# dohyeon-Lee/IsaacgymEnv

Measured on AMD Instinct MI355X. Metric: env-steps/sec AnymalTerrain 4096 envs/GPU, higher is better.
Workload: dtype f32; 1 GPU; AnymalTerrain VecTask.step, terrainType plane (AnymalTerrain.yaml default), 5 physics substeps/step, obs noise on; num_envs_per_gpu=4096, global_num_envs=4096, parallelism=dp1, solver=TGS (physx.solver_type 1, cfg/config.yaml:31)

## Files before the change

include/gymsim.h:

```cpp
#ifndef GYMSIM_H
#define GYMSIM_H

#include <stdint.h>

#include "gymtask.h"

#ifdef __cplusplus
extern "C" {
#endif

#define GS_ABI_VERSION 9

typedef struct gs_sim gs_sim;

typedef struct gs_model_desc {
    int32_t num_bodies, num_dofs, num_candidates, num_shapes, fixed_base;
    const int32_t *parent;
    const int32_t *joint_kind;
    const int32_t *body_dof;
    const double *joint_origin;
    const double *joint_axis;
    const double *mass;
    const double *com;
    const double *inertia;
    const int32_t *cand_body;
    const double *cand_point;
    const double *cand_radius;
    const int32_t *cand_shape;
    const double *dof_effort;
    const double *dof_velocity;
    const double *dof_armature;
    const double *dof_lower;
    const double *dof_upper;
    const int32_t *dof_has_limits;
    int32_t num_links;
    const int32_t *cand_link;
    const int32_t *link_body;
    const double *link_pose;
    const double *link_com;
    const int32_t *cand_dyn;
    const int32_t *shape_kind;
    const int32_t *shape_body;
    const int32_t *shape_link;
    const double *shape_pose;
    const double *shape_size;
    const double *shape_margin;
    const double *shape_sphere;
    int32_t num_hull_verts;
    const double *hull_verts;
    const int32_t *shape_hv0;
    const int32_t *shape_hv1;
    int32_t num_pairs;
    const int32_t *pair_a;
    const int32_t *pair_b;
    const int32_t *pair_kind;
    int32_t pair_pool;
    int32_t num_pair_verts;
    const double *pair_verts;
    const int32_t *shape_pv0;
    const int32_t *shape_pv1;
} gs_model_desc;

typedef struct gs_sim_params {
    double dt;
    int32_t substeps;
    double gravity[3];
    int32_t num_position_iterations;
    int32_t num_velocity_iterations;
    double contact_offset;
    double rest_offset;
    double bounce_threshold_velocity;
    double max_depenetration_velocity;
    int32_t contact_collection;
    int32_t kernel_variant;
    double joint_limit_margin;
    int32_t num_threads;
    int32_t solver_type;
} gs_sim_params;

typedef struct gs_pd_args {
    const float *actions;
    const float *default_pos;
    float kp, kd, action_scale, torque_limit;
    int32_t decimation;
    int32_t extra_simulates;
    float *torques_out;
    float *dof_state_out;
    float *root_state_out;
    float *contact_out;
    float *actions_copy_out;
    const gt_anymal_params *tail_params;
    const gt_anymal_buffers *tail_buffers;
} gs_pd_args;

int gs_abi_version(void);
const char *gs_last_error(void);

int gs_sim_pd_tail_supported(const gs_sim *sim);

int gs_topology_supported(const gs_model_desc *model);

gs_sim *gs_sim_create(int device, const gs_sim_params *params);
void gs_sim_destroy(gs_sim *sim);

int gs_sim_add_ground(gs_sim *sim, double static_friction, double dynamic_friction, double restitution);

int gs_sim_add_triangle_mesh(gs_sim *sim, const float *vertices, int64_t num_vertices, const uint32_t *triangles,
                             int64_t num_triangles, const double *transform_p, double static_friction,
                             double dynamic_friction, double restitution);

int gs_sim_set_model(gs_sim *sim, const gs_model_desc *model);

int gs_sim_prepare(gs_sim *sim, int num_envs, float *state, const float *shape_friction, float *contact);

int gs_sim_simulate(gs_sim *sim, const float *dof_force, void *stream);

int gs_sim_refresh_root(gs_sim *sim, float *root_state, void *stream);
int gs_sim_refresh_dof(gs_sim *sim, float *dof_state, void *stream);
int gs_sim_refresh_contact(gs_sim *sim, float *net_contact, void *stream);

int gs_sim_refresh_rigid_body(gs_sim *sim, float *rigid_body_state, void *stream);
int gs_sim_refresh_jacobian(gs_sim *sim, float *jacobian, void *stream);
int gs_sim_refresh_mass_matrix(gs_sim *sim, float *mass_matrix, void *stream);

int gs_sim_set_root(gs_sim *sim, const float *root_state, const int32_t *idx, int n_idx, void *stream);
int gs_sim_set_dof(gs_sim *sim, const float *dof_state, const int32_t *idx, int n_idx, void *stream);
int gs_sim_set_root_and_dof(gs_sim *sim, const float *root, const float *dof, const int32_t *idx, int n_idx,
                            void *stream);

int gs_sim_pd_step(gs_sim *sim, const gs_pd_args *args, void *stream);

int gs_sim_set_force_sensors(gs_sim *sim, int n, const int32_t *bodies);
int gs_sim_bind_force_sensors(gs_sim *sim, float *sensor_soa);
int gs_sim_refresh_force_sensor(gs_sim *sim, float *out, void *stream);

int gs_sim_set_dof_drives(gs_sim *sim, const int32_t *mode, const double *stiffness, const double *damping);
int gs_sim_bind_dof_targets(gs_sim *sim, const float *pos_targets, const float *vel_targets);
int gs_sim_bind_dof_properties_env(gs_sim *sim, const float *table, int any_drive, int any_limits);

int gs_sim_set_self_collision(gs_sim *sim, int enable);

int gs_sim_kernel_variant(gs_sim *sim);

int gs_sim_enable_timing(gs_sim *sim, int enable);
float gs_sim_last_kernel_ms(gs_sim *sim);

int gs_debug_phase_cycles(unsigned long long *out, int n, int reset);

int gs_debug_terrain_query(gs_sim *sim, const float *centres, const float *radii, int n, float *out, void *stream);

int gs_debug_self_contacts(gs_sim *sim, int mode, float *out, int *count, void *stream);

#ifdef __cplusplus
}
#endif
#endif
```

isaacgymenv_amd/csrc/gs_capi.hip:

```cpp
#include <cmath>
#include <cstdlib>
#include <cstdio>
#include <cstring>
#include <algorithm>
#include <chrono>
#include <string>
#include <vector>

#include "gs_internal.h"
#include "../../include/gymsim.h"

namespace {
thread_local std::string g_err;

int fail(const char* fmt, const char* arg = nullptr) {
  char buf[512];
  std::snprintf(buf, sizeof(buf), fmt, arg ? arg : "");
  g_err = buf;
  return -1;
}
int hip_fail(hipError_t e, const char* where) {
  char buf[512];
  std::snprintf(buf, sizeof(buf), "%s: %s", where, hipGetErrorString(e));
  g_err = buf;
  return -1;
}

std::string signature(const gs_model_desc* m) {
  std::string s = "fb" + std::to_string(m->fixed_base) + "_p";
  for (int i = 0; i < m->num_bodies; ++i) s += (i ? "-" : "") + std::to_string(m->parent[i]);
  s += "_c";
  for (int i = 0; i < m->num_candidates; ++i) s += (i ? "-" : "") + std::to_string(m->cand_body[i]);
  bool links_differ = m->num_links != m->num_bodies;
  for (int i = 0; i < m->num_candidates && !links_differ; ++i) links_differ = m->cand_link[i] != m->cand_body[i];
  if (links_differ) {
    s += "_l" + std::to_string(m->num_links) + "_";
    for (int i = 0; i < m->num_candidates; ++i) s += (i ? "-" : "") + std::to_string(m->cand_link[i]);
  }
  return s;
}

const TopoEntry* find_topology(const gs_model_desc* m) {
  const std::string sig = signature(m);
  for (int i = 0; i < g_num_topologies; ++i)
    if (sig == g_topologies[i].sig) return &g_topologies[i];
  return nullptr;
}
}

struct gs_sim {
  int device = 0;
  gs_sim_params params{};
  DevParams dp{};
  bool has_ground = false;
  float ground_mu = 1.f;
  const TopoEntry* topo = nullptr;
  launch_sim_fn sim_fn = nullptr;
  launch_pd_fn pd_fn = nullptr;
  int variant = 0;
  launch_sim_fn model_sim_fn = nullptr;
  launch_pd_fn model_pd_fn = nullptr;
  int model_variant = 0;
  bool team_pairs = false;
  int uni_any_drive = 0, uni_any_limits = 0;
  TopoEntry gen_entry{};
  GenTopo* d_gen = nullptr;
  int env_any_drive = 0, env_any_limits = 0;
  DevModel* d_model = nullptr;
  DevModel h_model{};
  DevLinks* d_links = nullptr;
  int nr = 0, nv = 0;
  std::vector<int> parent;
  float* sens = nullptr;
  int nb = 0, nd = 0, nc = 0, ns = 0;
  int N = 0;
  float* state = nullptr;
  const float* mu = nullptr;
  float* cf = nullptr;
  bool timing = false;
  hipEvent_t ev0 = nullptr, ev1 = nullptr;
  bool timed = false;
  float4* d_tverts = nullptr;
  uint4* d_tcells = nullptr;
  float* d_tblk = nullptr;
  float* d_tsq4 = nullptr;
  float4* d_trec = nullptr;
  float* d_rows = nullptr;
  size_t rows_cap = 0;
  bool host = false;
  HostPool* pool = nullptr;
  const HostTopoEntry* htopo = nullptr;
  DevLinks h_links{};
  std::vector<float4> h_tverts;
  std::vector<uint4> h_tcells;
  std::vector<float> h_tblk;
  std::vector<float> h_tsq4;
  std::vector<float4> h_trec;
  double host_ms = -1.0;
  const DevModel* model() const { return host ? &h_model : d_model; }
  const DevLinks* links() const { return host ? &h_links : d_links; }
};

extern "C" {

int gs_abi_version(void) { return GS_ABI_VERSION; }
const char* gs_last_error(void) { return g_err.c_str(); }

int gs_topology_supported(const gs_model_desc* model) { return find_topology(model) != nullptr; }

gs_sim* gs_sim_create(int device, const gs_sim_params* p) {
  if (!p) { fail("gs_sim_create: null params"); return nullptr; }
  if (!(p->dt > 0)) { fail("gs_sim_create: dt must be > 0"); return nullptr; }
  gs_sim* s = nullptr;
  if (device < 0) {
    s = new gs_sim();
    s->host = true;
    s->device = -1;
    s->pool = host_pool_create(p->num_threads > 0 ? p->num_threads : 1);
  } else {
    int ndev = 0;
    if (hipGetDeviceCount(&ndev) != hipSuccess || device >= ndev) {
      fail("gs_sim_create: no HIP device %s", std::to_string(device).c_str());
      return nullptr;
    }
    if (hipError_t e = hipSetDevice(device); e != hipSuccess) {
      hip_fail(e, "gs_sim_create hipSetDevice");
      return nullptr;
    }
    s = new gs_sim();
    s->device = device;
  }
  s->params = *p;
  const int sub = p->substeps > 0 ? p->substeps : 1;
  s->dp.h = (float)(p->dt / sub);
  s->dp.substeps = sub;
  for (int k = 0; k < 3; ++k) s->dp.g[k] = (float)p->gravity[k];
  s->dp.pos_iters = p->num_position_iterations;
  s->dp.vel_iters = p->num_velocity_iterations;
  s->dp.contact_offset = (float)p->contact_offset;
  s->dp.rest_offset = (float)p->rest_offset;
  s->dp.max_depen_vel = (float)p->max_depenetration_velocity;
  s->dp.tgs = p->solver_type == 1 && p->num_position_iterations > 0 ? 1 : 0;
  s->dp.collect = p->contact_collection != 0;
  s->dp.limit_margin = (float)(p->joint_limit_margin > 0 ? p->joint_limit_margin : 0.0);
  s->dp.any_limits = 0;
  s->dp.has_ground = 0;
  s->dp.ground_mu = 1.f;
  if (const char* v = std::getenv("GS_TEAM_ENVS_PER_WAVE")) {
    const int w = std::atoi(v);
    s->dp.team_epw = w == 16 || w == 8 || w == 4 ? w : 0;
  }
  return s;
}

void gs_sim_destroy(gs_sim* s) {
  if (!s) return;
  if (s->host) {
    host_pool_destroy(s->pool);
    delete s;
    return;
  }
  (void)hipSetDevice(s->device);
  if (s->d_model) (void)hipFree(s->d_model);
  if (s->d_links) (void)hipFree(s->d_links);
  if (s->d_tverts) (void)hipFree(s->d_tverts);
  if (s->d_tcells) (void)hipFree(s->d_tcells);
  if (s->d_tblk) (void)hipFree(s->d_tblk);
  if (s->d_tsq4) (void)hipFree(s->d_tsq4);
  if (s->d_trec) (void)hipFree(s->d_trec);
  if (s->d_rows) (void)hipFree(s->d_rows);
  if (s->d_gen) (void)hipFree(s->d_gen);
  if (s->ev0) (void)hipEventDestroy(s->ev0);
  if (s->ev1) (void)hipEventDestroy(s->ev1);
  delete s;
}

int gs_sim_add_ground(gs_sim* s, double static_friction, double dynamic_friction, double restitution) {
  if (!s) return fail("gs_sim_add_ground: null sim");
  (void)dynamic_friction;
  (void)restitution;
  s->has_ground = true;
  s->dp.has_ground = 1;
  s->dp.ground_mu = (float)static_friction;
  return 0;
}

int gs_sim_add_triangle_mesh(gs_sim* s, const float* vertices, int64_t num_vertices, const uint32_t* triangles,
                             int64_t num_triangles, const double* transform_p, double static_friction,
                             double dynamic_friction, double restitution) {
  (void)dynamic_friction;
  (void)restitution;
  if (!s || !vertices || !triangles) return fail("gs_sim_add_triangle_mesh: null argument");
  if (s->topo) return fail("gs_sim_add_triangle_mesh: call before the model is set (prepare_sim)");
  if (s->d_tverts) return fail("gs_sim_add_triangle_mesh: one triangle mesh per sim");
  if (num_triangles < 2) return fail("gs_sim_add_triangle_mesh: empty mesh");
  const int64_t cols = (int64_t)triangles[1] - 1;
  if (triangles[0] != 0 || triangles[2] != 1 || cols < 2 || num_vertices % cols != 0)
    return fail("gs_sim_add_triangle_mesh: not a heightfield grid mesh (first triangle)");
  const int64_t rows = num_vertices / cols;
  if (rows < 2 || num_triangles != 2 * (rows - 1) * (cols - 1))
    return fail("gs_sim_add_triangle_mesh: triangle count does not match a %s grid",
                (std::to_string(rows) + "x" + std::to_string(cols)).c_str());
  if (rows > (1 << 24) || cols > (1 << 24)) return fail("gs_sim_add_triangle_mesh: grid too large");
  for (int64_t i = 0; i + 1 < rows; ++i) {
    for (int64_t j = 0; j + 1 < cols; ++j) {
      const int64_t b = i * cols + j, t = 2 * (i * (cols - 1) + j);
      const uint32_t* a = triangles + 3 * t;
      if (a[0] != b || a[1] != b + cols + 1 || a[2] != b + 1 || a[3] != b || a[4] != b + cols || a[5] != b + cols + 1)
        return fail("gs_sim_add_triangle_mesh: triangle %s does not follow the heightfield grid layout",
                    std::to_string(t).c_str());
    }
  }
  std::vector<double> spans;
  for (int64_t j = 0; j < cols && spans.size() < 4096; j += std::max<int64_t>(1, cols / 1024))
    spans.push_back((double)vertices[3 * ((rows - 1) * cols + j)] - (double)vertices[3 * j]);
  std::sort(spans.begin(), spans.end());
  double hs = spans[spans.size() / 2] / (double)(rows - 1);
  if (!(hs > 0)) return fail("gs_sim_add_triangle_mesh: cannot infer the grid spacing");
  const double tx = transform_p ? transform_p[0] : 0.0, ty = transform_p ? transform_p[1] : 0.0,
               tz = transform_p ? transform_p[2] : 0.0;
  double x0 = vertices[0], y0 = vertices[1];
  for (int64_t j = 0; j < cols; ++j) x0 = std::min(x0, (double)vertices[3 * j]);
  for (int64_t i = 0; i < rows; ++i) y0 = std::min(y0, (double)vertices[3 * (i * cols) + 1]);
  std::vector<float4> hv((size_t)(rows * cols));
  for (int64_t i = 0; i < rows; ++i) {
    for (int64_t j = 0; j < cols; ++j) {
      const float* v = vertices + 3 * (i * cols + j);
      const double gx = x0 + i * hs, gy = y0 + j * hs;
      if (std::fabs(v[0] - gx) > 1.001 * hs || std::fabs(v[1] - gy) > 1.001 * hs)
        return fail("gs_sim_add_triangle_mesh: a vertex lies more than one cell from its grid point");
      hv[(size_t)(i * cols + j)] = make_float4((float)(v[0] + tx), (float)(v[1] + ty), (float)(v[2] + tz), 0.f);
    }
  }
  std::vector<uint4> hc((size_t)((rows - 1) * (cols - 1)));
  for (int64_t i = 0; i + 1 < rows; ++i) {
    for (int64_t j = 0; j + 1 < cols; ++j) {
      const float4 q[4] = {hv[i * cols + j], hv[i * cols + j + 1], hv[(i + 1) * cols + j], hv[(i + 1) * cols + j + 1]};
      float zmax = q[0].z, zmin = q[0].z, xmin = q[0].x, xmax = q[0].x, ymin = q[0].y, ymax = q[0].y;
      for (int k = 1; k < 4; ++k) {
        zmax = std::max(zmax, q[k].z);
        zmin = std::min(zmin, q[k].z);
        xmin = std::min(xmin, q[k].x); xmax = std::max(xmax, q[k].x);
        ymin = std::min(ymin, q[k].y); ymax = std::max(ymax, q[k].y);
      }
      const double cx0 = x0 + tx + i * hs, cy0 = y0 + ty + j * hs;
      uint32_t f = 0;
      if (xmin < cx0 - 0.25 * hs) f |= TCELL_XLO;
      if (xmax > cx0 + 1.25 * hs) f |= TCELL_XHI;
      if (ymin < cy0 - 0.25 * hs) f |= TCELL_YLO;
      if (ymax > cy0 + 1.25 * hs) f |= TCELL_YHI;
      auto ext = [&](double d) -> uint32_t {
        return (uint32_t)std::min(255.0, std::ceil(std::max(0.0, d) / hs * TCELL_EXT_UNITS));
      };
      const uint32_t ew = ext(cx0 - xmin) | ext(xmax - (cx0 + hs)) << 8 | ext(cy0 - ymin) << 16 |
                          ext(ymax - (cy0 + hs)) << 24;
      uint32_t zb, zl;
      std::memcpy(&zb, &zmax, 4);
      std::memcpy(&zl, &zmin, 4);
      hc[(size_t)(i * (cols - 1) + j)] = make_uint4(zb, f, zl, ew);
    }
  }
  const int64_t brows = (rows - 1 + TERRAIN_BLK - 1) / TERRAIN_BLK, bcols = (cols - 1 + TERRAIN_BLK - 1) / TERRAIN_BLK;
  std::vector<float> hb((size_t)(brows * bcols), -3.0e38f);
  for (int64_t i = 0; i + 1 < rows; ++i)
    for (int64_t j = 0; j + 1 < cols; ++j) {
      float top;
      std::memcpy(&top, &hc[(size_t)(i * (cols - 1) + j)].x, 4);
      float& b = hb[(size_t)((i / TERRAIN_BLK) * bcols + j / TERRAIN_BLK)];
      b = std::max(b, top);
    }
  const int64_t cr = rows - 1, cc = cols - 1;
  std::vector<float> h4((size_t)(cr * cc)), hq((size_t)(cr * cc));
  for (int64_t i = 0; i < cr; ++i)
    for (int64_t j = 0; j < cc; ++j) {
      float m = -3.0e38f;
      for (int64_t d = 0; d < 4 && j + d < cc; ++d) {
        float top;
        std::memcpy(&top, &hc[(size_t)(i * cc + j + d)].x, 4);
        m = std::max(m, top);
      }
      h4[(size_t)(i * cc + j)] = m;
    }
  for (int64_t i = 0; i < cr; ++i)
    for (int64_t j = 0; j < cc; ++j) {
      float m = -3.0e38f;
      for (int64_t d = 0; d < 4 && i + d < cr; ++d) m = std::max(m, h4[(size_t)((i + d) * cc + j)]);
      hq[(size_t)(i * cc + j)] = m;
    }
  std::vector<float4> hr((size_t)(cr * cc * TERRAIN_REC));
  for (int64_t i = 0; i < cr; ++i)
    for (int64_t j = 0; j < cc; ++j) {
      const float4 q00 = hv[i * cols + j], q01 = hv[i * cols + j + 1], q10 = hv[(i + 1) * cols + j],
                   q11 = hv[(i + 1) * cols + j + 1];
      auto normal = [](const float4& a, const float4& b, const float4& c, float* nf) {
        const double e1[3] = {(double)b.x - a.x, (double)b.y - a.y, (double)b.z - a.z};
        const double e2[3] = {(double)c.x - a.x, (double)c.y - a.y, (double)c.z - a.z};
        const double x[3] = {e1[1] * e2[2] - e1[2] * e2[1], e1[2] * e2[0] - e1[0] * e2[2], e1[0] * e2[1] - e1[1] * e2[0]};
        const double l2 = x[0] * x[0] + x[1] * x[1] + x[2] * x[2];
        nf[0] = 0.f; nf[1] = 0.f; nf[2] = -1.f;
        if (!(l2 > 1e-14)) return;
        const double il = 1.0 / std::sqrt(l2);
        if (x[2] * il < (double)TERRAIN_DOWN_NZ) return;
        for (int k = 0; k < 3; ++k) nf[k] = (float)(x[k] * il);
      };
      float n0[3], n1[3];
      normal(q00, q11, q01, n0);
      normal(q00, q10, q11, n1);
      float4* r = &hr[(size_t)((i * cc + j) * TERRAIN_REC)];
      r[0] = make_float4(q00.x, q00.y, q00.z, n0[0]);
      r[1] = make_float4(q01.x, q01.y, q01.z, n0[1]);
      r[2] = make_float4(q10.x, q10.y, q10.z, n0[2]);
      r[3] = make_float4(q11.x, q11.y, q11.z, n1[0]);
      r[4] = make_float4(n1[1], n1[2], 0.f, 0.f);
    }
  TerrainDev& T = s->dp.terr;
  if (s->host) {
    s->h_tverts = std::move(hv);
    s->h_tcells = std::move(hc);
    s->h_tblk = std::move(hb);
    s->h_tsq4 = std::move(hq);
    s->h_trec = std::move(hr);
    T.rec = s->h_trec.data();
    T.v = s->h_tverts.data();
    T.cell = s->h_tcells.data();
    T.blk = s->h_tblk.data();
    T.sq4 = s->h_tsq4.data();
  } else {
    float4* dv = nullptr;
    uint4* dc = nullptr;
    float* db = nullptr;
    float* dq = nullptr;
    float4* dr = nullptr;
    hipError_t e = hipSetDevice(s->device);
    if (e == hipSuccess) e = hipMalloc(&dv, hv.size() * sizeof(float4));
    if (e == hipSuccess) e = hipMalloc(&dc, hc.size() * sizeof(uint4));
    if (e == hipSuccess) e = hipMalloc(&db, hb.size() * sizeof(float));
    if (e == hipSuccess) e = hipMalloc(&dq, hq.size() * sizeof(float));
    if (e == hipSuccess) e = hipMemcpy(dv, hv.data(), hv.size() * sizeof(float4), hipMemcpyHostToDevice);
    if (e == hipSuccess) e = hipMemcpy(dc, hc.data(), hc.size() * sizeof(uint4), hipMemcpyHostToDevice);
    if (e == hipSuccess) e = hipMemcpy(db, hb.data(), hb.size() * sizeof(float), hipMemcpyHostToDevice);
    if (e == hipSuccess) e = hipMemcpy(dq, hq.data(), hq.size() * sizeof(float), hipMemcpyHostToDevice);
    if (e == hipSuccess) e = hipMalloc(&dr, hr.size() * sizeof(float4));
    if (e == hipSuccess) e = hipMemcpy(dr, hr.data(), hr.size() * sizeof(float4), hipMemcpyHostToDevice);
    if (e != hipSuccess) {
      if (dr) (void)hipFree(dr);
      if (dv) (void)hipFree(dv);
      if (dc) (void)hipFree(dc);
      if (db) (void)hipFree(db);
      if (dq) (void)hipFree(dq);
      return hip_fail(e, "gs_sim_add_triangle_mesh");
    }
    s->d_tverts = dv;
    s->d_tcells = dc;
    s->d_tblk = db;
    s->d_tsq4 = dq;
    s->d_trec = dr;
    T.rec = s->d_trec;
    T.v = s->d_tverts;
    T.cell = s->d_tcells;
    T.blk = s->d_tblk;
    T.sq4 = s->d_tsq4;
  }
  T.bcols = (int)bcols;
  T.rows = (int)rows;
  T.cols = (int)cols;
  T.x0 = (float)(x0 + tx);
  T.y0 = (float)(y0 + ty);
  T.hs = (float)hs;
  T.inv_hs = (float)(1.0 / hs);
  T.mu = (float)static_friction;
  s->dp.has_terrain = 1;
  return 0;
}

int gs_sim_set_model(gs_sim* s, const gs_model_desc* m) {
  if (!s || !m) return fail("gs_sim_set_model: null argument");
  if (m->num_bodies > GS_MAXB || m->num_dofs > GS_MAXD || m->num_candidates > GS_MAXC || m->num_links > GS_MAXL ||
      m->num_shapes > GS_MAXSH)
    return fail("gs_sim_set_model: articulation exceeds compiled maxima (bodies/dofs/candidates/links)");
  if (m->num_links < m->num_bodies || !m->link_body || !m->link_pose || !m->link_com ||
      (m->num_candidates > 0 && !m->cand_link))
    return fail("gs_sim_set_model: link tables missing (gs_model_desc ABI 2: num_links >= num_bodies)");
  for (int l = 0; l < m->num_links; ++l)
    if (m->link_body[l] < 0 || m->link_body[l] >= m->num_bodies) return fail("gs_sim_set_model: link_body out of range");
  for (int c = 0; c < m->num_candidates; ++c)
    if (m->cand_link[c] < 0 || m->cand_link[c] >= m->num_links) return fail("gs_sim_set_model: cand_link out of range");
  const TopoEntry* t = find_topology(m);
  const bool generic = !t || (s->params.kernel_variant == 4 && !s->host);
  if (generic) {
    if (s->host)
      return fail("gs_sim_set_model: the runtime-sized kernel is a GPU kernel and no host solver is compiled for "
                  "this topology (add it with tools/gen_topologies.py): %s", signature(m).c_str());
    if (s->params.kernel_variant == 1 || s->params.kernel_variant == 2)
      return fail("gs_sim_set_model: kernel_variant 1 / 2 requested but topology %s is not compiled (the runtime-"
                  "sized kernel is variant 4)", signature(m).c_str());
    for (int c = 0; c < m->num_candidates; ++c)
      if (m->cand_dyn && m->cand_dyn[c] >= 0)
        return fail("gs_sim_set_model: topology %s has convex-hull candidates: the runtime-sized kernel has no hull "
                    "ground manifold (compile the topology with tools/gen_topologies.py)", signature(m).c_str());
    if (s->dp.has_terrain)
      return fail("gs_sim_set_model: topology %s with a terrain mesh: the runtime-sized kernel has plane contacts only "
                  "(compile the topology with tools/gen_topologies.py)", signature(m).c_str());
    if (m->num_dofs + 6 > GS_MAXD + 6 || (m->num_candidates > 0 && !m->cand_shape))
      return fail("gs_sim_set_model: runtime-sized kernel tables missing for %s", signature(m).c_str());
  }
  if (!generic && m->num_pairs > 0 && m->pair_pool != t->npk)
    return fail("gs_sim_set_model: self-contact pool differs from the compiled topology's %s",
                std::to_string(t->npk).c_str());
  for (int c = 0; c < m->num_candidates && !generic; ++c)
    if (m->cand_dyn && m->cand_dyn[c] != t->cdyn[c])
      return fail("gs_sim_set_model: hull slots differ from the compiled topology (tools/gen_topologies.py)");
  if (!generic && m->num_pairs > 0 && m->num_pairs != t->npair)
    return fail("gs_sim_set_model: self-collision pair count differs from the compiled topology's %s",
                std::to_string(t->npair).c_str());
  for (int q = 0; q < m->num_pairs && !generic; ++q)
    if (m->pair_a[q] != t->pair_a[q] || m->pair_b[q] != t->pair_b[q] || m->pair_kind[q] != t->pair_k[q])
      return fail("gs_sim_set_model: self-collision pairs differ from the compiled topology (tools/gen_topologies.py)");
  for (int sh = 0; sh < m->num_shapes && !generic; ++sh)
    if (m->shape_kind && m->shape_kind[sh] != t->shkind[sh])
      return fail("gs_sim_set_model: shape kinds differ from the compiled topology (tools/gen_topologies.py)");
  DevModel h;
  std::memset(&h, 0, sizeof(h));
  for (int i = 0; i < m->num_bodies; ++i) {
    for (int k = 0; k < 9; ++k) h.jR[i][k] = (float)m->joint_origin[12 * i + k];
    for (int k = 0; k < 3; ++k) h.jt[i][k] = (float)m->joint_origin[12 * i + 9 + k];
    for (int k = 0; k < 3; ++k) h.jaxis[i][k] = (float)m->joint_axis[3 * i + k];
    h.mass[i] = (float)m->mass[i];
    for (int k = 0; k < 3; ++k) h.com[i][k] = (float)m->com[3 * i + k];
    const double* I = m->inertia + 9 * i;
    h.inertia[i][0] = (float)I[0]; h.inertia[i][1] = (float)I[4]; h.inertia[i][2] = (float)I[8];
    h.inertia[i][3] = (float)I[1]; h.inertia[i][4] = (float)I[2]; h.inertia[i][5] = (float)I[5];
  }
  {
    const double* P = m->link_pose;
    const double* c = m->link_com;
    for (int k = 0; k < 3; ++k)
      h.root_com[k] = (float)(P[9 + k] + P[3 * k] * c[0] + P[3 * k + 1] * c[1] + P[3 * k + 2] * c[2]);
  }
  for (int c = 0; c < m->num_candidates; ++c) {
    for (int k = 0; k < 3; ++k) h.cpoint[c][k] = (float)m->cand_point[3 * c + k];
    h.cradius[c] = (float)m->cand_radius[c];
  }
  if (!m->shape_kind || !m->shape_body || !m->shape_link || !m->shape_pose || !m->shape_size || !m->shape_margin ||
      !m->shape_sphere || !m->shape_hv0 || !m->shape_hv1 || (m->num_candidates > 0 && !m->cand_dyn))
    return fail("gs_sim_set_model: shape tables missing (gs_model_desc ABI 5)");
  if (m->num_hull_verts < 0 || m->num_hull_verts > GS_MAXHV || m->num_pairs < 0 || m->num_pairs > GS_MAXP ||
      (m->num_hull_verts > 0 && !m->hull_verts) || (m->num_pairs > 0 && (!m->pair_a || !m->pair_b || !m->pair_kind)))
    return fail("gs_sim_set_model: hull vertices / self-collision pairs exceed compiled maxima");
  for (int sh = 0; sh < m->num_shapes; ++sh) {
    for (int k = 0; k < 3; ++k) h.shc[sh][k] = (float)m->shape_sphere[4 * sh + k];
    double reach = m->shape_sphere[4 * sh + 3];
    for (int c = 0; c < m->num_candidates; ++c) {
      if (m->cand_shape && m->cand_shape[c] == sh && m->cand_dyn[c] < 0) {
        double d2 = 0.0;
        for (int k = 0; k < 3; ++k) {
          const double d = m->cand_point[3 * c + k] - m->shape_sphere[4 * sh + k];
          d2 += d * d;
        }
        reach = std::max(reach, std::sqrt(d2) + m->cand_radius[c]);
      }
    }
    h.shc[sh][3] = (float)(reach * (1.0 + 1e-4) + 1e-5);
    h.shkind[sh] = m->shape_kind[sh];
    h.shbody[sh] = m->shape_body[sh];
    h.shlink[sh] = m->shape_link[sh];
    for (int k = 0; k < 9; ++k) h.shR[sh][k] = (float)m->shape_pose[12 * sh + k];
    for (int k = 0; k < 3; ++k) h.sht[sh][k] = (float)m->shape_pose[12 * sh + 9 + k];
    for (int k = 0; k < 3; ++k) h.shsize[sh][k] = (float)m->shape_size[3 * sh + k];
    h.shm[sh] = (float)m->shape_margin[sh];
    h.hv0[sh] = m->shape_hv0[sh];
    h.hv1[sh] = m->shape_hv1[sh];
    if (h.shbody[sh] < 0 || h.shbody[sh] >= m->num_bodies || h.shlink[sh] < 0 || h.shlink[sh] >= m->num_links ||
        h.hv0[sh] < 0 || h.hv1[sh] < h.hv0[sh] || h.hv1[sh] > m->num_hull_verts ||
        (h.shkind[sh] == 4 && h.hv1[sh] == h.hv0[sh]))
      return fail("gs_sim_set_model: shape %s tables out of range", std::to_string(sh).c_str());
  }
  for (int v = 0; v < m->num_hull_verts; ++v)
    for (int k = 0; k < 4; ++k) h.hv[v][k] = (float)m->hull_verts[4 * v + k];
  if (m->num_pair_verts < 0 || m->num_pair_verts > GS_MAXPV || !m->shape_pv0 || !m->shape_pv1 ||
      (m->num_pair_verts > 0 && !m->pair_verts))
    return fail("gs_sim_set_model: hull self-collision cores missing or beyond GS_MAXPV");
  for (int v = 0; v < m->num_pair_verts; ++v)
    for (int k = 0; k < 4; ++k) h.pv[v][k] = (float)m->pair_verts[4 * v + k];
  for (int sh = 0; sh < m->num_shapes; ++sh) {
    h.pv0[sh] = m->shape_pv0[sh];
    h.pv1[sh] = m->shape_pv1[sh];
    if (h.pv0[sh] < 0 || h.pv1[sh] < h.pv0[sh] || h.pv1[sh] > m->num_pair_verts ||
        (h.shkind[sh] == 4 && h.pv1[sh] == h.pv0[sh]))
      return fail("gs_sim_set_model: shape %s self-collision core out of range", std::to_string(sh).c_str());
  }
  for (int c = 0; c < m->num_candidates; ++c)
    if (m->cand_dyn[c] >= 0 && m->shape_kind[m->cand_shape[c]] != 4)
      return fail("gs_sim_set_model: dynamic candidate %s on a shape that is not a hull", std::to_string(c).c_str());
  h.np = m->num_pairs;
  for (int q = 0; q < m->num_pairs; ++q) {
    h.pa[q] = m->pair_a[q];
    h.pb[q] = m->pair_b[q];
    h.pk[q] = m->pair_kind[q];
    if (h.pa[q] < 0 || h.pb[q] <= h.pa[q] || h.pb[q] >= m->num_shapes || h.pk[q] < 0 || h.pk[q] > 3)
      return fail("gs_sim_set_model: self-collision pair %s out of range", std::to_string(q).c_str());
  }
  for (int b = 0; b < m->num_bodies; ++b) {
    unsigned mask = 0;
    for (int a = b; a >= 0; a = m->parent[a]) mask |= 1u << a;
    h.banc[b] = mask;
  }
  int any_lim = 0;
  for (int j = 0; j < m->num_dofs; ++j) {
    h.effort[j] = (float)m->dof_effort[j];
    h.vmax[j] = (float)m->dof_velocity[j];
    h.armature[j] = (float)m->dof_armature[j];
    h.has_lim[j] = m->dof_has_limits && m->dof_has_limits[j] && m->dof_upper[j] > m->dof_lower[j];
    h.lower[j] = h.has_lim[j] ? (float)m->dof_lower[j] : 0.f;
    h.upper[j] = h.has_lim[j] ? (float)m->dof_upper[j] : 0.f;
    any_lim |= h.has_lim[j];
  }
  h.nsens = 0;
  for (int b = 0; b < GS_MAXB; ++b) h.sens_of_body[b] = -1;

  DevLinks hl;
  std::memset(&hl, 0, sizeof(hl));
  hl.nb = m->num_bodies;
  hl.nd = m->num_dofs;
  hl.nr = m->num_links;
  hl.fixed_base = m->fixed_base;
  for (int b = 0; b < m->num_bodies; ++b) {
    hl.parent[b] = m->parent[b];
    hl.jkind[b] = m->joint_kind[b];
    hl.bdof[b] = m->body_dof[b];
    unsigned mask = 0;
    for (int a = b; a >= 0; a = m->parent[a]) mask |= 1u << a;
    hl.anc_mask[b] = mask;
    if (m->body_dof[b] >= 0) hl.dbody[m->body_dof[b]] = b;
  }
  for (int l = 0; l < m->num_links; ++l) {
    hl.lbody[l] = m->link_body[l];
    for (int k = 0; k < 9; ++k) hl.lR[l][k] = (float)m->link_pose[12 * l + k];
    for (int k = 0; k < 3; ++k) hl.lt[l][k] = (float)m->link_pose[12 * l + 9 + k];
    for (int k = 0; k < 3; ++k) hl.lcom[l][k] = (float)m->link_com[3 * l + k];
  }

  const int want = s->params.kernel_variant;
  launch_sim_fn sim_fn = nullptr;
  launch_pd_fn pd_fn = nullptr;
  const HostTopoEntry* htopo = nullptr;
  int variant = 0;
  GenTopo hg;
  std::memset(&hg, 0, sizeof(hg));
  if (generic) {
    hg.nc = m->num_candidates;
    for (int c = 0; c < m->num_candidates; ++c) {
      hg.cbody[c] = m->cand_body[c];
      hg.cshape[c] = m->cand_shape[c];
      hg.clink[c] = m->cand_link[c];
      if (hg.cbody[c] < 0 || hg.cbody[c] >= m->num_bodies || hg.cshape[c] < 0 || hg.cshape[c] >= m->num_shapes)
        return fail("gs_sim_set_model: candidate %s tables out of range", std::to_string(c).c_str());
    }
    TopoEntry& g = s->gen_entry;
    g = TopoEntry{};
    g.sig = "runtime";
    g.name = "runtime-sized (gs_generic.hip)";
    g.sim = launch_sim_generic;
    g.pd = launch_pd_generic;
    g.dbg_pool = nullptr;
    g.nb = m->num_bodies; g.nd = m->num_dofs; g.nc = m->num_candidates; g.ns = m->num_shapes;
    g.sens = 0;
    g.row_floats = (int)generic_ws_floats(m->num_candidates, m->num_dofs, m->fixed_base);
    g.row_lanes = 1;
    g.npk = 0;
    g.npair = 0;
    t = &g;
  }
  if (s->host) {
    for (int i = 0; i < g_num_host_topologies; ++i)
      if (std::strcmp(g_host_topologies[i].sig, t->sig) == 0) htopo = &g_host_topologies[i];
    if (!htopo) return fail("gs_sim_set_model: no host solver for topology %s", t->sig);
    if (want == 2) return fail("gs_sim_set_model: the lane-team kernel is a GPU kernel (host sim)");
    variant = 3;
  } else {
    const TeamEntry* te = nullptr;
    for (int i = 0; i < g_num_team_kernels; ++i)
      if (std::strcmp(g_team_kernels[i].sig, t->sig) == 0 && g_team_kernels[i].sim) te = &g_team_kernels[i];
    if (te && any_lim) te = nullptr;
    if (want == 2 && !te)
      return fail("gs_sim_set_model: no lane-team kernel for this topology / joint limits");
    if (generic) {
      sim_fn = launch_sim_generic;
      pd_fn = launch_pd_generic;
      variant = 4;
    } else if (te && want != 1) {
      sim_fn = te->sim;
      pd_fn = te->pd;
      variant = 2;
    } else {
      sim_fn = t->sim;
      pd_fn = t->pd;
      variant = 1;
    }
    if (hipError_t e = hipSetDevice(s->device); e != hipSuccess) return hip_fail(e, "gs_sim_set_model hipSetDevice");
    DevModel* dm = s->d_model;
    DevLinks* dl = s->d_links;
    hipError_t e = hipSuccess;
    if (!dm) e = hipMalloc(&dm, sizeof(DevModel));
    if (e == hipSuccess && !dl) e = hipMalloc(&dl, sizeof(DevLinks));
    s->d_model = dm;
    s->d_links = dl;
    if (e == hipSuccess) e = hipMemcpy(dm, &h, sizeof(DevModel), hipMemcpyHostToDevice);
    if (e == hipSuccess) e = hipMemcpy(dl, &hl, sizeof(DevLinks), hipMemcpyHostToDevice);
    if (e == hipSuccess && generic && !s->d_gen) e = hipMalloc(&s->d_gen, sizeof(GenTopo));
    if (e == hipSuccess && generic) e = hipMemcpy(s->d_gen, &hg, sizeof(GenTopo), hipMemcpyHostToDevice);
    if (e != hipSuccess) return hip_fail(e, "gs_sim_set_model upload");
  }
  s->h_model = h;
  s->h_links = hl;
  s->dp.any_limits = any_lim;
  s->uni_any_limits = any_lim;
  s->parent.assign(m->parent, m->parent + m->num_bodies);
  s->sim_fn = sim_fn;
  s->pd_fn = pd_fn;
  s->htopo = htopo;
  s->variant = variant;
  s->model_sim_fn = sim_fn;
  s->model_pd_fn = pd_fn;
  s->model_variant = variant;
  s->team_pairs = variant == 2;
  s->nr = m->num_links;
  s->nv = (m->fixed_base ? 0 : 6) + m->num_dofs;
  s->nb = m->num_bodies;
  s->nd = m->num_dofs;
  s->nc = m->num_candidates;
  s->ns = m->num_shapes;
  s->topo = t;
  s->dp.gen = generic ? s->d_gen : nullptr;
  s->dp.gen_links = generic ? s->d_links : nullptr;
  s->dp.gen_nd = m->num_dofs;
  s->dp.gen_nr = m->num_links;
  return 0;
}

int gs_sim_prepare(gs_sim* s, int num_envs, float* state, const float* shape_friction, float* contact) {
  if (!s || !s->topo) return fail("gs_sim_prepare: model not set");
  if (num_envs <= 0 || !state || !shape_friction || !contact) return fail("gs_sim_prepare: bad buffers");
  s->N = num_envs;
  s->state = state;
  s->mu = shape_friction;
  s->cf = contact;
  return 0;
}

static SimBuffers buffers(gs_sim* s) { return SimBuffers{s->state, s->mu, s->cf, s->N, s->sens, s->d_rows}; }

static size_t rows_needed(const gs_sim* s) {
  if (s->host || !s->topo || (s->variant != 1 && s->variant != 4) || (s->variant == 1 && s->dp.has_terrain) ||
      s->topo->row_floats <= 0 || s->N <= 0)
    return 0;
  const size_t lanes = (size_t)s->topo->row_lanes;
  return ((size_t)s->N + lanes - 1) / lanes * lanes * (size_t)s->topo->row_floats;
}

static int ready(gs_sim* s, const char* where) {
  if (!s || !s->topo || !s->state) return fail("%s: sim not prepared", where);
  if (s->host ? !s->htopo : (!s->sim_fn || !s->pd_fn || !s->d_model || !s->d_links))
    return fail("%s: sim model incomplete", where);
  if (const size_t need = rows_needed(s); need > s->rows_cap) {
    if (hipError_t e = hipSetDevice(s->device); e != hipSuccess) return hip_fail(e, where);
    if (s->d_rows) (void)hipFree(s->d_rows);
    s->d_rows = nullptr;
    s->rows_cap = 0;
    if (hipError_t e = hipMalloc(&s->d_rows, need * sizeof(float)); e != hipSuccess) {
      s->d_rows = nullptr;
      return hip_fail(e, where);
    }
    s->rows_cap = need;
  }
  return 0;
}

static void timing_begin(gs_sim* s, hipStream_t st) {
  if (!s->timing || s->host) return;
  if (!s->ev0) {
    if (hipEventCreate(&s->ev0) != hipSuccess || hipEventCreate(&s->ev1) != hipSuccess) {
      s->timing = false;
      return;
    }
  }
  (void)hipEventRecord(s->ev0, st);
}
static void timing_end(gs_sim* s, hipStream_t st) {
  if (!s->timing || s->host) return;
  s->timed = hipEventRecord(s->ev1, st) == hipSuccess;
}

namespace {
using host_clock = std::chrono::steady_clock;
double ms_since(host_clock::time_point t0) {
  return std::chrono::duration<double, std::milli>(host_clock::now() - t0).count();
}
}

int gs_sim_simulate(gs_sim* s, const float* dof_force, void* stream) {
  if (ready(s, "gs_sim_simulate")) return -1;
  if (s->host) {
    const auto t0 = host_clock::now();
    s->htopo->sim(&s->h_model, s->dp, buffers(s), dof_force, s->pool);
    s->host_ms = ms_since(t0);
    return 0;
  }
  hipStream_t st = (hipStream_t)stream;
  timing_begin(s, st);
  hipError_t e = s->sim_fn(s->d_model, s->dp, buffers(s), dof_force, st);
  timing_end(s, st);
  return e == hipSuccess ? 0 : hip_fail(e, "gs_sim_simulate");
}

int gs_sim_pd_step(gs_sim* s, const gs_pd_args* a, void* stream) {
  if (ready(s, "gs_sim_pd_step")) return -1;
  if (!a || !a->actions || !a->default_pos || !a->torques_out || !a->dof_state_out)
    return fail("gs_sim_pd_step: actions/default_pos/torques_out/dof_state_out required");
  PdDev d;
  d.actions = a->actions;
  d.dof_state_in = a->dof_state_out;
  d.default_pos = a->default_pos;
  d.kp = a->kp; d.kd = a->kd; d.scale = a->action_scale; d.tlim = a->torque_limit;
  d.decimation = a->decimation;
  d.extra = a->extra_simulates;
  d.torques_out = a->torques_out;
  d.dof_out = a->dof_state_out;
  d.root_out = a->root_state_out;
  d.cf_out = a->contact_out;
  d.actions_copy = a->actions_copy_out;
  d.tail_on = 0;
  if (a->tail_params || a->tail_buffers) {
    const gt_anymal_params* tp = a->tail_params;
    const gt_anymal_buffers* tb = a->tail_buffers;
    auto aligned = [](const void* q) { return ((uintptr_t)q & 15u) == 0; };
    if (!gs_sim_pd_tail_supported(s)) return fail("gs_sim_pd_step: this sim's kernel has no fused tail");
    if (!tp || !tb || tb->hound || tp->num_envs != s->N || tp->num_dofs != s->nd || tp->num_dofs % 4 != 0 ||
        tp->num_bodies != s->nr || tp->num_feet > 4 || tp->num_knees > 4 || tp->num_feet < 0 || tp->num_knees < 0 ||
        tp->base_index < 0 || tp->base_index >= s->nr || !tb->reset_count || !tb->reset_masks || !tb->reset_buf ||
        !tb->timeout_buf || !tb->rew_buf || !tb->episode_sums || !tb->base_lin_vel || !tb->base_ang_vel ||
        !tb->projected_gravity || !tb->progress_buf || !tb->randomize_buf || !tb->commands || !tb->feet_air_time ||
        !tb->last_actions || !tb->last_dof_vel)
      return fail("gs_sim_pd_step: invalid tail parameters / buffers");
    for (int k = 0; k < tp->num_feet; ++k)
      if (tp->feet_idx[k] < 0 || tp->feet_idx[k] >= s->nr) return fail("gs_sim_pd_step: tail foot index");
    for (int k = 0; k < tp->num_knees; ++k)
      if (tp->knee_idx[k] < 0 || tp->knee_idx[k] >= s->nr) return fail("gs_sim_pd_step: tail knee index");
    if (tb->torques != a->torques_out || tb->actions != a->actions_copy_out || tb->root_states != a->root_state_out ||
        tb->contact_forces != a->contact_out || tb->dof_state != a->dof_state_out)
      return fail("gs_sim_pd_step: the tail must read this call's outputs");
    if (!aligned(tb->torques) || !aligned(tb->actions) || !aligned(tb->last_actions) || !aligned(tb->last_dof_vel) ||
        !aligned(tb->dof_state))
      return fail("gs_sim_pd_step: the tail's dof rows must be 16-byte aligned");
    d.tail_on = 1;
    d.tail_p = *tp;
    d.tail_b = *tb;
  }
  if (s->host) {
    const auto t0 = host_clock::now();
    s->htopo->pd(&s->h_model, s->dp, buffers(s), d, s->pool);
    s->host_ms = ms_since(t0);
    return 0;
  }
  hipStream_t st = (hipStream_t)stream;
  timing_begin(s, st);
  hipError_t e = s->pd_fn(s->d_model, s->dp, buffers(s), d, st);
  timing_end(s, st);
  return e == hipSuccess ? 0 : hip_fail(e, "gs_sim_pd_step");
}

int gs_sim_refresh_root(gs_sim* s, float* out, void* stream) {
  if (ready(s, "gs_sim_refresh_root")) return -1;
  if (s->host) {
    host_refresh_root(s->state, s->N, &s->h_model.root_com[0], out, s->pool);
    return 0;
  }
  hipError_t e = launch_refresh_root(s->state, s->N, s->nd, &s->d_model->root_com[0], out, (hipStream_t)stream);
  return e == hipSuccess ? 0 : hip_fail(e, "gs_sim_refresh_root");
}
int gs_sim_refresh_dof(gs_sim* s, float* out, void* stream) {
  if (ready(s, "gs_sim_refresh_dof")) return -1;
  if (s->host) {
    host_refresh_dof(s->state, s->N, s->nd, out, s->pool);
    return 0;
  }
  hipError_t e = launch_refresh_dof(s->state, s->N, s->nd, out, (hipStream_t)stream);
  return e == hipSuccess ? 0 : hip_fail(e, "gs_sim_refresh_dof");
}
int gs_sim_refresh_contact(gs_sim* s, float* out, void* stream) {
  if (ready(s, "gs_sim_refresh_contact")) return -1;
  if (s->host) {
    host_soa_to_aos(s->cf, s->N, s->nr, 3, out, s->pool);
    return 0;
  }
  hipError_t e = launch_refresh_contact(s->cf, s->N, s->nr, out, (hipStream_t)stream);
  return e == hipSuccess ? 0 : hip_fail(e, "gs_sim_refresh_contact");
}
static int kinematics(gs_sim* s, int mode, float* rb, float* jac, float* mm, void* stream, const char* where) {
  if (ready(s, where)) return -1;
  if (!rb && !jac && !mm) return fail("%s: null output", where);
  if (s->host) {
    host_kinematics(&s->h_model, &s->h_links, s->state, s->N, s->nv, mode, rb, jac, mm, s->pool);
    return 0;
  }
  hipError_t e = launch_kinematics(s->d_model, s->d_links, s->state, s->N, s->nv, mode, rb, jac, mm,
                                   (hipStream_t)stream);
  return e == hipSuccess ? 0 : hip_fail(e, where);
}
int gs_sim_refresh_rigid_body(gs_sim* s, float* out, void* stream) {
  return kinematics(s, 1, out, nullptr, nullptr, stream, "gs_sim_refresh_rigid_body");
}
int gs_sim_refresh_jacobian(gs_sim* s, float* out, void* stream) {
  return kinematics(s, 2, nullptr, out, nullptr, stream, "gs_sim_refresh_jacobian");
}
int gs_sim_refresh_mass_matrix(gs_sim* s, float* out, void* stream) {
  return kinematics(s, 4, nullptr, nullptr, out, stream, "gs_sim_refresh_mass_matrix");
}
int gs_sim_set_root(gs_sim* s, const float* src, const int32_t* idx, int n_idx, void* stream) {
  if (ready(s, "gs_sim_set_root")) return -1;
  if (s->host) {
    host_set_root(s->state, s->N, &s->h_model.root_com[0], src, idx, idx ? n_idx : s->N);
    return 0;
  }
  hipError_t e = launch_set_root(s->state, s->N, s->nd, &s->d_model->root_com[0], src, idx, n_idx,
                                 (hipStream_t)stream);
  return e == hipSuccess ? 0 : hip_fail(e, "gs_sim_set_root");
}
int gs_sim_set_dof(gs_sim* s, const float* src, const int32_t* idx, int n_idx, void* stream) {
  if (ready(s, "gs_sim_set_dof")) return -1;
  if (s->host) {
    host_set_dof(s->state, s->N, s->nd, src, idx, idx ? n_idx : s->N);
    return 0;
  }
  hipError_t e = launch_set_dof(s->state, s->N, s->nd, src, idx, n_idx, (hipStream_t)stream);
  return e == hipSuccess ? 0 : hip_fail(e, "gs_sim_set_dof");
}

int gs_sim_set_root_and_dof(gs_sim* s, const float* root, const float* dof, const int32_t* idx, int n_idx,
                            void* stream) {
  if (ready(s, "gs_sim_set_root_and_dof")) return -1;
  if (!root || !dof || !idx || n_idx < 0) return fail("gs_sim_set_root_and_dof: root, dof and idx required");
  if (s->host) {
    host_set_root(s->state, s->N, &s->h_model.root_com[0], root, idx, n_idx);
    host_set_dof(s->state, s->N, s->nd, dof, idx, n_idx);
    return 0;
  }
  hipError_t e = launch_set_root_dof(s->state, s->N, s->nd, &s->d_model->root_com[0], root, dof, idx, n_idx,
                                     (hipStream_t)stream);
  return e == hipSuccess ? 0 : hip_fail(e, "gs_sim_set_root_and_dof");
}

int gs_sim_set_force_sensors(gs_sim* s, int n, const int32_t* bodies) {
  if (!s || !s->topo) return fail("gs_sim_set_force_sensors: model not set");
  if (s->state) return fail("gs_sim_set_force_sensors: call before gs_sim_prepare");
  if (n < 0 || n > GS_MAXS || (n > 0 && !bodies)) return fail("gs_sim_set_force_sensors: at most 8 sensors");
  if (n > 0 && s->variant == 2)
    return fail("gs_sim_set_force_sensors: the lane-team kernel has no force sensors (use kernel_variant 1)");
  if (n > 0 && s->variant == 4)
    return fail("gs_sim_set_force_sensors: the runtime-sized kernel has no force sensors (compile the topology)");
  if (n > 0 && !s->topo->sens)
    return fail("gs_sim_set_force_sensors: topology %s is compiled without force sensors (sensors flag in "
                "tools/gen_topologies.py MODELS)", s->topo->name);
  DevModel& h = s->h_model;
  for (int b = 0; b < GS_MAXB; ++b) h.sens_of_body[b] = -1;
  for (int i = 0; i < n; ++i) {
    const int b = bodies[i];
    if (b <= 0 || b >= s->nb) return fail("gs_sim_set_force_sensors: sensor body out of range (or the root)");
    for (int c = 0; c < s->nb; ++c)
      if (s->parent[c] == b) return fail("gs_sim_set_force_sensors: sensors on non-leaf bodies are not supported");
    if (h.sens_of_body[b] >= 0) return fail("gs_sim_set_force_sensors: two sensors on one body");
    h.sens_of_body[b] = i;
  }
  h.nsens = n;
  if (s->host) return 0;
  hipError_t e = hipSetDevice(s->device);
  if (e == hipSuccess) e = hipMemcpy(s->d_model, &h, sizeof(DevModel), hipMemcpyHostToDevice);
  return e == hipSuccess ? 0 : hip_fail(e, "gs_sim_set_force_sensors hipMemcpy");
}

static int kernel_select(gs_sim* s, const char* who) {
  launch_sim_fn sim_fn = s->model_sim_fn;
  launch_pd_fn pd_fn = s->model_pd_fn;
  int variant = s->model_variant;
  const bool lane = s->dp.any_drive || s->dp.dof_env || (s->dp.self_collide && !s->team_pairs);
  if (lane && variant == 2) {
    if (s->params.kernel_variant == 2)
      return fail("%s: the lane-team kernel (kernel_variant 2) has no joint drives or per-actor dof properties", who);
    sim_fn = s->topo->sim;
    pd_fn = s->topo->pd;
    variant = 1;
  }
  s->sim_fn = sim_fn;
  s->pd_fn = pd_fn;
  s->variant = variant;
  return 0;
}

int gs_sim_set_dof_drives(gs_sim* s, const int32_t* mode, const double* stiffness, const double* damping) {
  if (!s || !s->topo) return fail("gs_sim_set_dof_drives: model not set");
  if (s->nd > 0 && (!mode || !stiffness || !damping)) return fail("gs_sim_set_dof_drives: null argument");
  DevModel h = s->h_model;
  int any = 0;
  for (int j = 0; j < s->nd; ++j) {
    const double kp = mode[j] == 1 ? stiffness[j] : 0.0;
    const double kd = (mode[j] == 1 || mode[j] == 2) ? damping[j] : 0.0;
    if (!(kp >= 0.0) || !(kd >= 0.0)) return fail("gs_sim_set_dof_drives: negative or NaN drive gain");
    h.dkp[j] = (float)kp;
    h.dkd[j] = (float)kd;
    any |= (kp > 0.0 || kd > 0.0);
  }
  if (any && s->model_variant == 2 && s->params.kernel_variant == 2)
    return fail("gs_sim_set_dof_drives: the lane-team kernel (kernel_variant 2) has no joint drives");
  if (!s->host) {
    hipError_t e = hipSetDevice(s->device);
    if (e == hipSuccess) e = hipDeviceSynchronize();
    if (e == hipSuccess) e = hipMemcpy(s->d_model, &h, sizeof(DevModel), hipMemcpyHostToDevice);
    if (e != hipSuccess) return hip_fail(e, "gs_sim_set_dof_drives hipMemcpy");
  }
  s->h_model = h;
  s->uni_any_drive = any;
  s->dp.any_drive = s->dp.dof_env ? s->env_any_drive : any;
  return kernel_select(s, "gs_sim_set_dof_drives");
}

int gs_sim_set_self_collision(gs_sim* s, int enable) {
  if (!s || !s->topo) return fail("gs_sim_set_self_collision: model not set");
  if (enable && s->h_model.np > 0 && s->topo->npk <= 0)
    return fail("gs_sim_set_self_collision: the compiled topology has no self-contact pool");
  if (enable && s->h_model.np > 0 && s->variant == 4)
    return fail("gs_sim_set_self_collision: the runtime-sized kernel has no self-collision (compile the topology "
                "with tools/gen_topologies.py, or create the actors with collision filter 1)");
  s->dp.self_collide = enable && s->h_model.np > 0;
  if (s->dp.self_collide && s->variant == 2 && !s->team_pairs) {
    if (s->params.kernel_variant == 2)
      return fail("gs_sim_set_self_collision: the lane-team kernel (kernel_variant 2) has no self-collision");
    s->sim_fn = s->topo->sim;
    s->pd_fn = s->topo->pd;
    s->variant = 1;
  }
  return 0;
}

int gs_sim_bind_dof_targets(gs_sim* s, const float* pos_targets, const float* vel_targets) {
  if (!s || !s->topo) return fail("gs_sim_bind_dof_targets: model not set");
  s->dp.ptgt = pos_targets;
  s->dp.vtgt = vel_targets;
  return 0;
}

int gs_sim_bind_dof_properties_env(gs_sim* s, const float* table, int any_drive, int any_limits) {
  if (ready(s, "gs_sim_bind_dof_properties_env")) return -1;
  if (table) {
    s->dp.dof_env = table;
    s->dp.dof_env_n = s->N;
    s->env_any_drive = any_drive != 0;
    s->env_any_limits = any_limits != 0;
    s->dp.any_drive = s->env_any_drive;
    s->dp.any_limits = s->env_any_limits;
  } else {
    s->dp.dof_env = nullptr;
    s->dp.dof_env_n = 0;
    s->dp.any_drive = s->uni_any_drive;
    s->dp.any_limits = s->uni_any_limits;
  }
  return kernel_select(s, "gs_sim_bind_dof_properties_env");
}

int gs_sim_bind_force_sensors(gs_sim* s, float* soa) {
  if (ready(s, "gs_sim_bind_force_sensors")) return -1;
  if (s->h_model.nsens > 0 && !soa) return fail("gs_sim_bind_force_sensors: buffer required");
  s->sens = soa;
  return 0;
}

int gs_sim_refresh_force_sensor(gs_sim* s, float* out, void* stream) {
  if (ready(s, "gs_sim_refresh_force_sensor")) return -1;
  if (s->h_model.nsens == 0) return 0;
  if (!s->sens) return fail("gs_sim_refresh_force_sensor: sensors not bound");
  if (s->host) {
    host_soa_to_aos(s->sens, s->N, s->h_model.nsens, 6, out, s->pool);
    return 0;
  }
  hipError_t e = launch_refresh_sensor(s->sens, s->N, s->h_model.nsens, out, (hipStream_t)stream);
  return e == hipSuccess ? 0 : hip_fail(e, "gs_sim_refresh_force_sensor");
}

int gs_debug_terrain_query(gs_sim* s, const float* centres, const float* radii, int n, float* out, void* stream) {
  if (!s || !s->dp.has_terrain) return fail("gs_debug_terrain_query: no terrain mesh");
  if (n < 0 || (n > 0 && (!centres || !radii || !out))) return fail("gs_debug_terrain_query: bad buffers");
  if (s->host) {
    host_terrain_query(s->dp, centres, radii, n, out);
    return 0;
  }
  hipError_t e = launch_terrain_query(s->dp, centres, radii, n, out, (hipStream_t)stream);
  return e == hipSuccess ? 0 : hip_fail(e, "gs_debug_terrain_query");
}

int gs_debug_self_contacts(gs_sim* s, int mode, float* out, int* count, void* stream) {
  if (ready(s, "gs_debug_self_contacts")) return -1;
  if (!out || !count) return fail("gs_debug_self_contacts: bad buffers");
  if (s->host) {
    if (mode != 0) return fail("gs_debug_self_contacts: the host backend has the inline form only (mode 0)");
    s->htopo->dbg_pool(&s->h_model, s->dp, buffers(s), out, count, s->pool);
    return 0;
  }
  const hipError_t e = s->topo->dbg_pool(s->d_model, s->dp, buffers(s), mode, out, count, (hipStream_t)stream);
  return e == hipSuccess ? 0 : hip_fail(e, "gs_debug_self_contacts (mode 1 needs a split-form topology)");
}

int gs_sim_kernel_variant(gs_sim* s) { return s ? s->variant : -1; }

int gs_sim_pd_tail_supported(const gs_sim* s) {
  return s && !s->host && s->topo && s->variant == 2 && !s->dp.has_terrain && team_fused_tail_available() ? 1 : 0;
}

int gs_sim_enable_timing(gs_sim* s, int enable) {
  if (!s) return fail("gs_sim_enable_timing: null sim");
  s->timing = enable != 0;
  return 0;
}
float gs_sim_last_kernel_ms(gs_sim* s) {
  if (s && s->host) return s->timing ? (float)s->host_ms : -1.f;
  if (!s || !s->timed) return -1.f;
  float ms = -1.f;
  if (hipEventSynchronize(s->ev1) != hipSuccess) return -1.f;
  if (hipEventElapsedTime(&ms, s->ev0, s->ev1) != hipSuccess) return -1.f;
  return ms;
}

}
```

isaacgymenv_amd/csrc/gs_internal.h:

```cpp
#pragma once
#include <hip/hip_runtime.h>

#include "gs_terrain.h"
#include "../../include/gymtask.h"

#define GS_MAXB 32
#define GS_MAXD 32
#define GS_MAXC 192
#define GS_MAXL 40
#define GS_MAXS 8
#define GS_MAXSH 32
#define GS_MAXHV 2048
#define GS_MAXP 512
#define GS_MAXPV 512
#define GS_MAXPOOL 8
#define GS_WAVE 64
#ifndef GS_MIN_RESPONSE
#define GS_MIN_RESPONSE 1e-3f
#endif

struct DevModel {
  float jR[GS_MAXB][9];
  float jt[GS_MAXB][3];
  float jaxis[GS_MAXB][3];
  float mass[GS_MAXB];
  float com[GS_MAXB][3];
  float root_com[3];
  float inertia[GS_MAXB][6];
  float cpoint[GS_MAXC][3];
  float cradius[GS_MAXC];
  float shc[GS_MAXSH][4];
  float effort[GS_MAXD];
  float vmax[GS_MAXD];
  float armature[GS_MAXD];
  float dkp[GS_MAXD], dkd[GS_MAXD];
  float lower[GS_MAXD], upper[GS_MAXD];
  int has_lim[GS_MAXD];
  int nsens;
  int sens_of_body[GS_MAXB];
  unsigned banc[GS_MAXB];
  int shkind[GS_MAXSH];
  int shbody[GS_MAXSH], shlink[GS_MAXSH];
  float shR[GS_MAXSH][9], sht[GS_MAXSH][3];
  float shsize[GS_MAXSH][3];
  float shm[GS_MAXSH];
  int hv0[GS_MAXSH], hv1[GS_MAXSH];
  int np;
  int pa[GS_MAXP], pb[GS_MAXP], pk[GS_MAXP];
  alignas(16) float hv[GS_MAXHV][4];
  int pv0[GS_MAXSH], pv1[GS_MAXSH];
  alignas(16) float pv[GS_MAXPV][4];
};

struct DevParams {
  float h;
  int substeps;
  float g[3];
  int pos_iters, vel_iters;
  int tgs;
  float contact_offset, rest_offset, max_depen_vel;
  float ground_mu;
  int has_ground;
  int collect;
  float limit_margin;
  int any_limits;
  int has_terrain;
  TerrainDev terr;
  int any_drive;
  int self_collide;
  const float* ptgt;
  const float* vtgt;
  const float* dof_env;
  int dof_env_n;
  const struct GenTopo* gen;
  const struct DevLinks* gen_links;
  int gen_nd, gen_nr;
  int team_epw;
};
#define GS_DOFP_FIELDS 6

struct SimBuffers {
  float* state;
  const float* mu;
  float* cf;
  int N;
  float* sens;
  float* rows;
};

struct GenTopo {
  int nc;
  int cbody[GS_MAXC], cshape[GS_MAXC], clink[GS_MAXC];
};

struct PdDev {
  const float* actions;
  const float* dof_state_in;
  const float* default_pos;
  float kp, kd, scale, tlim;
  int decimation, extra;
  float* torques_out;
  float* dof_out;
  float* root_out;
  float* cf_out;
  float* actions_copy;
  int tail_on;
  gt_anymal_params tail_p;
  gt_anymal_buffers tail_b;
};

bool team_fused_tail_available();

typedef hipError_t (*launch_sim_fn)(const DevModel*, const DevParams&, const SimBuffers&, const float* tau,
                                    hipStream_t);
typedef hipError_t (*launch_pd_fn)(const DevModel*, const DevParams&, const SimBuffers&, const PdDev&,
                                   hipStream_t);

typedef hipError_t (*launch_dbg_pool_fn)(const DevModel*, const DevParams&, const SimBuffers&, int mode, float* out,
                                        int* count, hipStream_t);
struct TopoEntry {
  const char* sig;
  const char* name;
  launch_sim_fn sim;
  launch_pd_fn pd;
  launch_dbg_pool_fn dbg_pool;
  int nb, nd, nc, ns;
  int sens;
  int row_floats, row_lanes;
  int npk;
  const int* cdyn;
  int npair;
  const int *pair_a, *pair_b, *pair_k, *shkind;
};

struct DevLinks {
  int nb, nd, nr, fixed_base;
  int parent[GS_MAXB];
  int jkind[GS_MAXB];
  int bdof[GS_MAXB];
  unsigned anc_mask[GS_MAXB];
  int dbody[GS_MAXD];
  int lbody[GS_MAXL];
  float lR[GS_MAXL][9];
  float lt[GS_MAXL][3];
  float lcom[GS_MAXL][3];
};

extern TopoEntry g_topologies[];
extern const int g_num_topologies;

struct TeamEntry {
  const char* sig;
  launch_sim_fn sim;
  launch_pd_fn pd;
};
extern TeamEntry g_team_kernels[];
extern const int g_num_team_kernels;

hipError_t launch_terrain_query(const DevParams& P, const float* c, const float* r, int n, float* out, hipStream_t s);
hipError_t launch_refresh_root(const float* state, int N, int nd, const float* com0, float* out, hipStream_t s);
hipError_t launch_refresh_dof(const float* state, int N, int nd, float* out, hipStream_t s);
hipError_t launch_refresh_contact(const float* cf, int N, int nb, float* out, hipStream_t s);
hipError_t launch_kinematics(const DevModel* M, const DevLinks* L, const float* state, int N, int nv, int mode,
                             float* rb, float* jac, float* mm, hipStream_t s);
hipError_t launch_refresh_sensor(const float* soa, int N, int ns, float* out, hipStream_t s);
hipError_t launch_set_root(float* state, int N, int nd, const float* com0, const float* src, const int* idx,
                           int n_idx, hipStream_t s);
hipError_t launch_set_root_dof(float* state, int N, int nd, const float* com0, const float* root, const float* dof,
                               const int* idx, int n, hipStream_t s);
hipError_t launch_set_dof(float* state, int N, int nd, const float* src, const int* idx, int n_idx,
                          hipStream_t s);
hipError_t launch_sim_generic(const DevModel* M, const DevParams& P, const SimBuffers& B, const float* tau,
                              hipStream_t st);
hipError_t launch_pd_generic(const DevModel* M, const DevParams& P, const SimBuffers& B, const PdDev& A,
                             hipStream_t st);
inline size_t generic_ws_floats(int nc, int nd, int fixed_base) {
  return (size_t)2 * (3 * nc + nd) * ((fixed_base ? 0 : 6) + nd);
}

struct HostPool;
HostPool* host_pool_create(int threads);
void host_pool_destroy(HostPool* p);
int host_pool_threads(const HostPool* p);
typedef void (*host_sim_fn)(const DevModel*, const DevParams&, const SimBuffers&, const float* tau, HostPool*);
typedef void (*host_pd_fn)(const DevModel*, const DevParams&, const SimBuffers&, const PdDev&, HostPool*);
typedef void (*host_dbg_pool_fn)(const DevModel*, const DevParams&, const SimBuffers&, float* out, int* count, HostPool*);
struct HostTopoEntry {
  const char* sig;
  host_sim_fn sim;
  host_pd_fn pd;
  host_dbg_pool_fn dbg_pool;
};
extern HostTopoEntry g_host_topologies[];
extern const int g_num_host_topologies;
void host_refresh_root(const float* st, int N, const float* com0, float* out, HostPool* pool);
void host_refresh_dof(const float* st, int N, int nd, float* out, HostPool* pool);
void host_soa_to_aos(const float* soa, int N, int n, int comp, float* out, HostPool* pool);
void host_set_root(float* st, int N, const float* com0, const float* src, const int* idx, int n);
void host_set_dof(float* st, int N, int nd, const float* src, const int* idx, int n);
void host_kinematics(const DevModel* M, const DevLinks* L, const float* st, int N, int nv, int mode, float* rb,
                     float* jac, float* mm, HostPool* pool);
void host_terrain_query(const DevParams& P, const float* c, const float* r, int n, float* out);
```

isaacgymenv_amd/csrc/gs_team.hip:

```cpp
#include <type_traits>

#include "gs_internal.h"
#include "gs_topologies.h"
#include "gs_math.h"
#include "gs_pairs.h"
#include "gt_anymal_tail.h"

#ifdef GS_PHASE_PROFILE
__device__ unsigned long long gs_phase_cycles[64];
#define GS_PROF_DECL long long gs_t_ = clock64(); long long gs_acc_[16] = {0};
#define GS_PROF(i) { const long long t_ = clock64(); gs_acc_[i] += t_ - gs_t_; gs_t_ = t_; }
#define GS_PROF_COUNT(i, n) { gs_acc_[i] += (n); }
#define GS_PROF_PARAM , long long &gs_t_, long long *gs_acc_
#define GS_PROF_ARGS , gs_t_, gs_acc_
#define GS_PROF_FLUSH                                                   \
  if ((threadIdx.x & 63) == 0) {                                        \
    long long tot_ = 0;                                                 \
    for (int i_ = 0; i_ < 16; ++i_) {                                   \
      atomicAdd(&gs_phase_cycles[i_], (unsigned long long)gs_acc_[i_]); \
      if (i_ < 8 || i_ == 11) tot_ += gs_acc_[i_];                      \
    }                                                                   \
    atomicAdd(&gs_phase_cycles[16 + (int)min(tot_ / 25000, 15ll)], 1ull); \
    if (tot_ > 250000) {                                                \
      for (int i_ = 0; i_ < 16; ++i_) atomicAdd(&gs_phase_cycles[32 + i_], (unsigned long long)gs_acc_[i_]); \
      atomicAdd(&gs_phase_cycles[48], 1ull);                            \
    }                                                                   \
  }
#else
#define GS_PROF_DECL
#define GS_PROF_PARAM
#define GS_PROF_ARGS
#define GS_PROF(i)
#define GS_PROF_COUNT(i, n)
#define GS_PROF_FLUSH
#endif

namespace {

template <int CTRL>
__device__ __forceinline__ float qperm(float x) {
  return __builtin_bit_cast(float, __builtin_amdgcn_update_dpp(0, __builtin_bit_cast(int, x), CTRL, 0xF, 0xF, true));
}
template <int CTRL>
__device__ __forceinline__ int qperm_i(int x) {
  return __builtin_amdgcn_mov_dpp(x, CTRL, 0xF, 0xF, false);
}
__device__ __forceinline__ float quad_sum(float x) {
  x = x + qperm<0xB1>(x);
  return x + qperm<0x4E>(x);
}
typedef float f2 __attribute__((ext_vector_type(2)));
#ifndef GS_TEAM_PK
#define GS_TEAM_PK 0
#endif
__device__ __forceinline__ f2 pk_fma(f2 a, f2 b, f2 c) {
#if GS_TEAM_PK
  return __builtin_elementwise_fma(a, b, c);
#else
  return f2{fmaf(a.x, b.x, c.x), fmaf(a.y, b.y, c.y)};
#endif
}

__device__ __forceinline__ void quad_sum3(float* u) {
  const float a0 = qperm<0xB1>(u[0]), a1 = qperm<0xB1>(u[1]), a2 = qperm<0xB1>(u[2]);
  const float t0 = u[0] + a0, t1 = u[1] + a1, t2 = u[2] + a2;
  const float b0 = qperm<0x4E>(t0), b1 = qperm<0x4E>(t1), b2 = qperm<0x4E>(t2);
  u[0] = t0 + b0;
  u[1] = t1 + b1;
  u[2] = t2 + b2;
}
__device__ __forceinline__ void quad_sum4(float* u) {
  const float a0 = qperm<0xB1>(u[0]), a1 = qperm<0xB1>(u[1]), a2 = qperm<0xB1>(u[2]), a3 = qperm<0xB1>(u[3]);
  const float t0 = u[0] + a0, t1 = u[1] + a1, t2 = u[2] + a2, t3 = u[3] + a3;
  const float b0 = qperm<0x4E>(t0), b1 = qperm<0x4E>(t1), b2 = qperm<0x4E>(t2), b3 = qperm<0x4E>(t3);
  u[0] = t0 + b0;
  u[1] = t1 + b1;
  u[2] = t2 + b2;
  u[3] = t3 + b3;
}
__device__ __forceinline__ float bcast(float x, int L) {
  switch (L) {
    case 0: return qperm<0x00>(x);
    case 1: return qperm<0x55>(x);
    case 2: return qperm<0xAA>(x);
    default: return qperm<0xFF>(x);
  }
}
__device__ __forceinline__ int bcast_i(int x, int L) {
  switch (L) {
    case 0: return qperm_i<0x00>(x);
    case 1: return qperm_i<0x55>(x);
    case 2: return qperm_i<0xAA>(x);
    default: return qperm_i<0xFF>(x);
  }
}

template <class T>
struct CM {
  static constexpr int CL = T::T_CL, CC = T::T_CC;
  static constexpr int BODY = 25;
  static constexpr int CAND = BODY * CL;
  static constexpr int DOF = CAND + 4 * CC;
  static constexpr int SHP = DOF + 3 * CL;
  static constexpr int NP = SHP + (T::NPK > 0 ? 8 * T::T_SPC : 0);
  static constexpr int LANES = T::T_LANES;
};

#ifndef GS_TEAM_BLOCK
#define GS_TEAM_BLOCK 64
#endif
constexpr int kTeamBlock = GS_TEAM_BLOCK;
static_assert(kTeamBlock % 4 == 0 && kTeamBlock <= GS_WAVE, "a workgroup holds whole teams within one wave");

constexpr int RW = kTeamBlock + 1;

template <int EPW>
struct WaveForm {
  static_assert(EPW == 16 || EPW == 8 || EPW == 4, "envs per wave");
  static constexpr bool kWhole = EPW * 4 >= kTeamBlock;
  static constexpr int TEAMS = kWhole ? kTeamBlock / 4 : EPW;
  static constexpr int LANES = 4 * TEAMS;
  static constexpr int WAVES = kTeamBlock / LANES;
  static constexpr int THREADS = kWhole ? kTeamBlock : GS_WAVE * WAVES;
};
template <int EPW>
__device__ __forceinline__ int team_column() {
  if constexpr (WaveForm<EPW>::kWhole) return threadIdx.x;
  else return (threadIdx.x / GS_WAVE) * WaveForm<EPW>::LANES + (threadIdx.x & (GS_WAVE - 1));
}
template <int EPW>
__device__ __forceinline__ void team_sync() {
  if constexpr (WaveForm<EPW>::kWhole) {
    __syncthreads();
  } else {
    __builtin_amdgcn_fence(__ATOMIC_RELEASE, "workgroup");
    __builtin_amdgcn_wave_barrier();
    __builtin_amdgcn_fence(__ATOMIC_ACQUIRE, "workgroup");
  }
}

template <class T>
struct RowSlots {
  static constexpr int CL = T::T_CL;
  static constexpr int ZROW = 16;
  static constexpr int RZROW = 16;
  static constexpr int CSLOT = 15;
  __device__ static constexpr int zslot(int comp) { return comp < 6 ? 4 * (comp >> 1) + (comp & 1) : 4 * (comp - 6) + 2; }
  __device__ static constexpr int zs(int rr, int s) { return rr < 2 ? 2 * s + rr : 2 * ZROW + s; }
  static constexpr int C_DI = 3 * ZROW, C_G = C_DI + 3, C_TP = C_G + 3, C_TV = C_TP + 1,
                       C_MU = C_TV + 1, C_ACT = C_MU + 1, C_SEP = C_ACT + 1, PER_CONTACT = C_SEP + 1;
  static constexpr int R_DI = 3 * RZROW, R_G = R_DI + 3, R_TP = R_G + 3, R_TV = R_TP + 1,
                       R_MU = R_TV + 1, R_SEP = R_MU + 1, PER_ROOT = R_SEP + 1;
  static constexpr int CHAIN = PER_CONTACT * T::T_CC;
  static constexpr int ROOT = PER_ROOT * (T::T_RC > 0 ? T::T_RC : 1);
  static constexpr int P_Z = kPoolLam + 3, P_DI = P_Z + 15, P_G = P_DI + 3, P_TP = P_G + 3, P_TV = P_TP + 1,
                       P_CA = P_TV + 1, P_CB = P_CA + 1, PER_POOL = P_CB + 1;
  static constexpr int POOL = CHAIN + ROOT;
  static constexpr int TOTAL = POOL + PER_POOL * T::NPK;
  __device__ static constexpr int chain(int j) { return j * PER_CONTACT; }
  __device__ static constexpr int root(int j) { return CHAIN + j * PER_ROOT; }
};

template <int NCH, int K>
__device__ __forceinline__ float sel_chain(const float (&x)[NCH][K], int lc, int k) {
  float v = x[0][k];
#pragma unroll
  for (int c = 1; c < NCH; ++c) v = lc == c ? x[c][k] : v;
  return v;
}

template <class T>
__device__ __forceinline__ void gather_w(int lc, float wA, float wA2, const float (&wC)[T::T_NCH], float* wb,
                                         float* wc) {
  wb[0] = bcast(wA, 0); wb[1] = bcast(wA2, 0); wb[2] = bcast(wA, 1); wb[3] = bcast(wA2, 1);
  wb[4] = bcast(wA, 2); wb[5] = bcast(wA2, 2);
  wc[0] = wc[1] = wc[2] = 0.f;
#pragma unroll
  for (int c = 0; c < T::T_NCH; ++c) {
    const float c0 = bcast(wC[c], 0), c1 = bcast(wC[c], 1), c2 = bcast(wC[c], 2);
    wc[0] = lc == c ? c0 : wc[0];
    wc[1] = lc == c ? c1 : wc[1];
    wc[2] = lc == c ? c2 : wc[2];
  }
}

__device__ __forceinline__ void contact_block(float u0, float u1, float u2, float di0, float di1, float di2,
                                              float s10, float s20, float s21, float tdi, float mu,
                                              float* lam, float& dl0, float& dl1, float& dl2) {
  const float n0 = fmaxf(fmaf(-u0, di0, lam[0] + tdi), 0.f);
  const float a1 = fmaf(-u1, di1, lam[1]);
  const float a2 = fmaf(-u2, di2, lam[2]);
  dl0 = n0 - lam[0];
  lam[0] = n0;
  const float lim = mu * n0;
  const float n1 = __builtin_amdgcn_fmed3f(fmaf(-s10, dl0, a1), -lim, lim);
  const float b2 = fmaf(-s20, dl0, a2);
  dl1 = n1 - lam[1];
  lam[1] = n1;
  const float n2 = __builtin_amdgcn_fmed3f(fmaf(-s21, dl1, b2), -lim, lim);
  dl2 = n2 - lam[2];
  lam[2] = n2;
}

template <class T>
struct TeamState {
  float p[3], quat[4], vo[3], w[3];
  float q[T::T_CL], qd[T::T_CL];
};

template <class T>
__device__ __forceinline__ void stage_chain_model(const DevModel* __restrict__ M, float* mdl) {
  using C = CM<T>;
  for (int i = threadIdx.x; i < C::NP * T::T_NCH; i += blockDim.x) {
    const int p = i / T::T_NCH, c = i - p * T::T_NCH;
    float v;
    if (p < C::CAND) {
      const int k = p / C::BODY, f = p - k * C::BODY;
      const int b = 1 + c * C::CL + k;
      if (f < 9) v = M->jR[b][f];
      else if (f < 12) v = M->jt[b][f - 9];
      else if (f < 15) v = M->jaxis[b][f - 12];
      else if (f < 16) v = M->mass[b];
      else if (f < 19) v = M->com[b][f - 16];
      else v = M->inertia[b][f - 19];
    } else if (p < C::DOF) {
      const int j = (p - C::CAND) / 4, f = (p - C::CAND) - 4 * j;
      const int cand = T::T_RC + c * C::CC + j;
      v = f < 3 ? M->cpoint[cand][f] : M->cradius[cand];
    } else if (p < C::SHP) {
      const int k = (p - C::DOF) / 3, f = (p - C::DOF) - 3 * k;
      const int d = c * C::CL + k;
      v = f == 0 ? M->effort[d] : (f == 1 ? M->vmax[d] : M->armature[d]);
    } else {
      const int j = (p - C::SHP) / 8, f = (p - C::SHP) - 8 * j;
      const int sh = T::T_RS + c * T::T_SPC + j;
      const int kind = M->shkind[sh];
      const float hl = kind == 1 ? M->shsize[sh][1] : 0.f;
      if (f < 6) {
        const float sg = f < 3 ? -hl : hl;
        const int a = f % 3;
        v = kind == 0 || kind == 1 ? M->sht[sh][a] + sg * M->shR[sh][3 * a + 2] : M->shc[sh][a];
      } else if (f == 6) {
        v = kind == 0 || kind == 1 ? M->shm[sh] : M->shc[sh][3];
      } else {
        v = hl;
      }
    }
    mdl[p * C::LANES + c] = v;
  }
}

template <class T>
struct ShapeTab {
  static constexpr int RS = T::HAS_TEAM ? T::T_RS : 0;
  static constexpr int ROOT = kShC * T::NS;
  static constexpr int POSE = ROOT + 8 * RS;
  static constexpr int SIZE = T::NPK > 0 ? POSE + 15 * T::NS : 1;
};
template <class T>
__device__ __forceinline__ void stage_shape_consts(const DevModel* __restrict__ M, float* sct) {
  if constexpr (T::NPK > 0) {
    using S = ShapeTab<T>;
    for (int i = threadIdx.x; i < S::SIZE; i += blockDim.x) {
      float v = 0.f;
      if (i < S::ROOT) {
        const int sh = i / kShC, f = i - kShC * sh;
        v = f == 0 ? M->shc[sh][3]
                   : (f == 1 ? M->shm[sh] : (f == 2 ? M->shsize[sh][1] : (float)(256 * M->shbody[sh] + M->shlink[sh])));
      } else if (i >= S::POSE) {
        const int sh = (i - S::POSE) / 15, f = (i - S::POSE) - 15 * sh;
        v = f < 9 ? M->shR[sh][f] : (f < 12 ? M->sht[sh][f - 9] : M->shc[sh][f - 12]);
      } else {
        const int sr = (i - S::ROOT) / 8, f = (i - S::ROOT) - 8 * sr;
        const int kind = T::shkind[sr];
        const bool seg = kind == 0 || kind == 1;
        const float hl = kind == 1 ? M->shsize[sr][1] : 0.f;
        if (f < 6) {
          const int a = f % 3;
          const float sg = f < 3 ? -hl : hl;
          v = seg ? M->sht[sr][a] + sg * M->shR[sr][3 * a + 2] : M->shc[sr][a];
        } else {
          v = f == 6 ? (seg ? M->shm[sr] : M->shc[sr][3]) : hl;
        }
      }
      sct[i] = v;
    }
  }
}

template <class T>
__device__ __forceinline__ void team_load(const float* __restrict__ st, int N, int e, int lc, TeamState<T>& s) {
  constexpr int ND = T::ND, CL = T::T_CL;
#pragma unroll
  for (int k = 0; k < 3; ++k) s.p[k] = st[k * N + e];
#pragma unroll
  for (int k = 0; k < 4; ++k) s.quat[k] = st[(3 + k) * N + e];
#pragma unroll
  for (int k = 0; k < 3; ++k) s.vo[k] = st[(7 + k) * N + e];
#pragma unroll
  for (int k = 0; k < 3; ++k) s.w[k] = st[(10 + k) * N + e];
#pragma unroll
  for (int k = 0; k < CL; ++k) {
    s.q[k] = st[(13 + lc * CL + k) * N + e];
    s.qd[k] = st[(13 + ND + lc * CL + k) * N + e];
  }
}
template <class T>
__device__ __forceinline__ void team_store(float* __restrict__ st, int N, int e, int lc, const TeamState<T>& s) {
  constexpr int ND = T::ND, CL = T::T_CL;
  if (lc == 0) {
#pragma unroll
    for (int k = 0; k < 3; ++k) st[k * N + e] = s.p[k];
#pragma unroll
    for (int k = 0; k < 4; ++k) st[(3 + k) * N + e] = s.quat[k];
#pragma unroll
    for (int k = 0; k < 3; ++k) st[(7 + k) * N + e] = s.vo[k];
#pragma unroll
    for (int k = 0; k < 3; ++k) st[(10 + k) * N + e] = s.w[k];
  }
#pragma unroll
  for (int k = 0; k < CL; ++k) {
    st[(13 + lc * CL + k) * N + e] = s.q[k];
    st[(13 + ND + lc * CL + k) * N + e] = s.qd[k];
  }
}

__device__ __forceinline__ void body_inertia(const float* R, const float* X, float m, const float* com,
                                             const float* Il, SpI& I) {
  float c[3];
  mat3vec(R, com, c);
  c[0] += X[0]; c[1] += X[1]; c[2] += X[2];
  float Am[9];
#pragma unroll
  for (int r = 0; r < 3; ++r) {
    Am[3 * r + 0] = R[3 * r] * Il[0] + R[3 * r + 1] * Il[3] + R[3 * r + 2] * Il[4];
    Am[3 * r + 1] = R[3 * r] * Il[3] + R[3 * r + 1] * Il[1] + R[3 * r + 2] * Il[5];
    Am[3 * r + 2] = R[3 * r] * Il[4] + R[3 * r + 1] * Il[5] + R[3 * r + 2] * Il[2];
  }
  const float cc = c[0] * c[0] + c[1] * c[1] + c[2] * c[2];
  I.m = m;
  I.h[0] = m * c[0]; I.h[1] = m * c[1]; I.h[2] = m * c[2];
  I.I[0] = Am[0] * R[0] + Am[1] * R[1] + Am[2] * R[2] + m * (cc - c[0] * c[0]);
  I.I[1] = Am[3] * R[3] + Am[4] * R[4] + Am[5] * R[5] + m * (cc - c[1] * c[1]);
  I.I[2] = Am[6] * R[6] + Am[7] * R[7] + Am[8] * R[8] + m * (cc - c[2] * c[2]);
  I.I[3] = Am[0] * R[3] + Am[1] * R[4] + Am[2] * R[5] - m * c[0] * c[1];
  I.I[4] = Am[0] * R[6] + Am[1] * R[7] + Am[2] * R[8] - m * c[0] * c[2];
  I.I[5] = Am[3] * R[6] + Am[4] * R[7] + Am[5] * R[8] - m * c[1] * c[2];
}

__device__ __forceinline__ float base_jac(const float* xc, int ax, int k) {
  if (k < 3) {
    const float m3[3][3] = {{0.f, xc[2], -xc[1]}, {-xc[2], 0.f, xc[0]}, {xc[1], -xc[0], 0.f}};
    return m3[ax][k];
  }
  return (ax == k - 3) ? 1.f : 0.f;
}

__device__ __forceinline__ int opaque_index(int x) {
  asm volatile("" : "+v"(x));
  return x;
}

template <class T>
__host__ __device__ constexpr int team_stash_size() {
  return 15 + 6 + 6 + T::T_CL * (6 + 2) + T::T_CL * (T::T_CL - 1) / 2;
}

constexpr int kTeamsPerBlock = kTeamBlock / 4;

template <class T>
__host__ __device__ constexpr bool team_closed_form() {
  for (int q = 0; q < T::NPAIR; ++q)
    if (T::pair_k[q] > 2) return false;
  return true;
}
constexpr int kTeamSt = 9;
template <class T>
__host__ __device__ constexpr int team_lc() { return T::NPK > 0 ? T::NPK : 1; }
template <class T>
__host__ __device__ constexpr int shw_size() {
  const int pose = kShW * T::NS * kTeamsPerBlock;
  const int stage = team_lc<T>() * kTeamSt * 64 + T::NPK * kTeamSt * kTeamsPerBlock;
  return T::NPK == 0 ? 1 : (team_closed_form<T>() ? (stage > pose ? stage : pose) : pose);
}

__device__ __forceinline__ float seg_seg_d2(const float* p1, const float* q1, const float* p2, const float* q2) {
  float d1[3], d2[3], r[3];
#pragma unroll
  for (int k = 0; k < 3; ++k) { d1[k] = q1[k] - p1[k]; d2[k] = q2[k] - p2[k]; r[k] = p1[k] - p2[k]; }
  const float a = dot3f(d1, d1), e = dot3f(d2, d2), b = dot3f(d1, d2), c = dot3f(d1, r), f = dot3f(d2, r);
  const float ia = a > 1e-12f ? __builtin_amdgcn_rcpf(a) : 0.f;
  const float ie = e > 1e-12f ? __builtin_amdgcn_rcpf(e) : 0.f;
  const float den = a * e - b * b;
  float s = den > 1e-12f * a * e ? __builtin_amdgcn_fmed3f((b * f - c * e) * __builtin_amdgcn_rcpf(den), 0.f, 1.f) : 0.f;
  const float t = __builtin_amdgcn_fmed3f((b * s + f) * ie, 0.f, 1.f);
  s = __builtin_amdgcn_fmed3f((b * t - c) * ia, 0.f, 1.f);
  float dd = 0.f;
#pragma unroll
  for (int k = 0; k < 3; ++k) {
    const float x = r[k] + s * d1[k] - t * d2[k];
    dd += x * x;
  }
  return dd;
}

__device__ __forceinline__ float seg_pt_d2(const float* s0, const float* s1, const float* p) {
  float d[3], r[3];
#pragma unroll
  for (int k = 0; k < 3; ++k) { d[k] = s1[k] - s0[k]; r[k] = p[k] - s0[k]; }
  const float dd = dot3f(d, d);
  const float t = dd > 1e-12f ? __builtin_amdgcn_fmed3f(dot3f(r, d) * __builtin_amdgcn_rcpf(dd), 0.f, 1.f) : 0.f;
  float out = 0.f;
#pragma unroll
  for (int k = 0; k < 3; ++k) {
    const float x = r[k] - t * d[k];
    out += x * x;
  }
  return out;
}

__device__ __forceinline__ void seg_seg_rcp(const float* p1, const float* q1, const float* p2, const float* q2, float& s,
                                            float& t, float& den, float& a, float& e) {
  float d1[3], d2[3], r[3];
#pragma unroll
  for (int k = 0; k < 3; ++k) { d1[k] = q1[k] - p1[k]; d2[k] = q2[k] - p2[k]; r[k] = p1[k] - p2[k]; }
  a = dot3f(d1, d1);
  e = dot3f(d2, d2);
  const float f = dot3f(d2, r);
  s = 0.f; t = 0.f; den = 0.f;
  const float ia = __builtin_amdgcn_rcpf(a), ie = __builtin_amdgcn_rcpf(e);
  auto cl = [](float x) { return __builtin_amdgcn_fmed3f(x, 0.f, 1.f); };
  if (a <= 1e-12f && e <= 1e-12f) {
  } else if (a <= 1e-12f) {
    t = cl(f * ie);
  } else {
    const float c = dot3f(d1, r);
    if (e <= 1e-12f) {
      s = cl(-c * ia);
    } else {
      const float b = dot3f(d1, d2);
      den = a * e - b * b;
      s = den > 0.f ? cl((b * f - c * e) * __builtin_amdgcn_rcpf(den)) : 0.f;
      t = (b * s + f) * ie;
      if (t < 0.f) { t = 0.f; s = cl(-c * ia); }
      else if (t > 1.f) { t = 1.f; s = cl((b - c) * ia); }
    }
  }
}
__device__ __forceinline__ void seg_closest_pt_rcp(const float* p, const float* a, const float* b, float* q) {
  const float ab[3] = {b[0] - a[0], b[1] - a[1], b[2] - a[2]}, ap[3] = {p[0] - a[0], p[1] - a[1], p[2] - a[2]};
  const float l2 = dot3f(ab, ab);
  const float t = l2 > 0.f ? __builtin_amdgcn_fmed3f(dot3f(ap, ab) * __builtin_amdgcn_rcpf(l2), 0.f, 1.f) : 0.f;
#pragma unroll
  for (int k = 0; k < 3; ++k) q[k] = a[k] + t * ab[k];
}

template <class T>
__host__ __device__ constexpr bool team_pair(int a, int b) {
  for (int q = 0; q < T::NPAIR; ++q)
    if (T::pair_a[q] == a && T::pair_b[q] == b) return true;
  return false;
}
template <class T>
__host__ __device__ constexpr int team_pair_index(int a, int b) {
  for (int q = 0; q < T::NPAIR; ++q)
    if ((T::pair_a[q] == a && T::pair_b[q] == b) || (T::pair_a[q] == b && T::pair_b[q] == a)) return q;
  return -1;
}
template <class T>
__device__ __forceinline__ unsigned long long team_pair_bit(int lc, int ra, int ja, int dl, int jb) {
  unsigned long long bit = 0ull;
#pragma unroll
  for (int c = 0; c < 4; ++c) {
    const int a = ja < 0 ? ra : T::T_RS + c * T::T_SPC + ja;
    const int b = T::T_RS + ((c + dl) & 3) * T::T_SPC + jb;
    const int q = team_pair_index<T>(a, b);
    bit = lc == c ? (q >= 0 ? 1ull << q : 0ull) : bit;
  }
  return bit;
}
__device__ __forceinline__ unsigned long long quad_or64(unsigned long long m) {
  int lo = (int)(unsigned)m, hi = (int)(unsigned)(m >> 32);
  lo |= qperm_i<0xB1>(lo);
  hi |= qperm_i<0xB1>(hi);
  lo |= qperm_i<0x4E>(lo);
  hi |= qperm_i<0x4E>(hi);
  return ((unsigned long long)(unsigned)hi << 32) | (unsigned)lo;
}

template <class T, int EPW>
__device__ __forceinline__ int team_narrow_replicated(const DevModel* __restrict__ M, const DevParams& P,
                                                   const float* __restrict__ mu_g, int N, int e, int lc,
                                                   const float (&R0)[9], const float (&R)[T::T_CL][9],
                                                   const float (&X)[T::T_CL][3], unsigned long long near,
                                                   float* __restrict__ shw_tab, const float* __restrict__ sct,
                                                   float* __restrict__ pool) {
  constexpr int TPW = WaveForm<EPW>::TEAMS;
  const int team = (threadIdx.x & (GS_WAVE - 1)) >> 2;
  float* tab = shw_tab + team;
  team_sync<EPW>();
#pragma unroll
  for (int j = 0; j < T::T_SPC; ++j) {
    const int sh = T::T_RS + lc * T::T_SPC + j;
    const int k = T::sh_body[T::T_RS + j] - 1;
    const float* ps = sct + ShapeTab<T>::POSE + 15 * sh;
    float Rs[9], t[3], c[3];
    mat3mul(R[k], ps, Rs);
    mat3vec(R[k], ps + 9, t);
    mat3vec(R[k], ps + 12, c);
#pragma unroll
    for (int f = 0; f < 9; ++f) tab[(kShW * sh + f) * TPW] = Rs[f];
#pragma unroll
    for (int f = 0; f < 3; ++f) {
      tab[(kShW * sh + 9 + f) * TPW] = X[k][f] + t[f];
      tab[(kShW * sh + 12 + f) * TPW] = X[k][f] + c[f];
    }
  }
  if (lc == 0) {
#pragma unroll
    for (int sh = 0; sh < T::T_RS; ++sh) {
      const float* ps = sct + ShapeTab<T>::POSE + 15 * sh;
      float Rs[9], t[3], c[3];
      mat3mul(R0, ps, Rs);
      mat3vec(R0, ps + 9, t);
      mat3vec(R0, ps + 12, c);
#pragma unroll
      for (int f = 0; f < 9; ++f) tab[(kShW * sh + f) * TPW] = Rs[f];
#pragma unroll
      for (int f = 0; f < 3; ++f) {
        tab[(kShW * sh + 9 + f) * TPW] = t[f];
        tab[(kShW * sh + 12 + f) * TPW] = c[f];
      }
    }
  }
  team_sync<EPW>();
  const unsigned long long tmask = quad_or64(near);
  int cnt = 0;
  if (tmask) cnt = self_contacts<T, TPW, RW, RowSlots<T>::PER_POOL>(M, P, mu_g, N, e, tab, pool, ShapeConstsTab{sct},
                                                                    tmask);
  return cnt;
}

template <class T, int EPW>
__device__ __forceinline__ int team_self_contacts(const DevModel* __restrict__ M, const float* __restrict__ cm,
                                                  const DevParams& P, const float* __restrict__ mu_g, int N, int e,
                                                  int lc, const float (&R0)[9], const float (&R)[T::T_CL][9],
                                                  const float (&X)[T::T_CL][3], float* __restrict__ shw_tab,
                                                  const float* __restrict__ sct, float* __restrict__ pool) {
  constexpr int TPW = WaveForm<EPW>::TEAMS, WL = WaveForm<EPW>::kWhole ? 64 : WaveForm<EPW>::LANES;
  constexpr int LN = T::T_LANES, SPC = T::T_SPC, RSH = T::T_RS;
  using C = CM<T>;
  const float off = P.contact_offset * 1.001f + 1e-5f;
  float p0[SPC][3], p1[SPC][3], rad[SPC], hl[SPC];
#pragma unroll
  for (int j = 0; j < SPC; ++j) {
    const int k = T::sh_body[RSH + j] - 1;
    const float* sp = cm + (C::SHP + 8 * j) * LN;
    const float l0[3] = {sp[0], sp[LN], sp[2 * LN]}, l1[3] = {sp[3 * LN], sp[4 * LN], sp[5 * LN]};
    mat3vec(R[k], l0, p0[j]);
    mat3vec(R[k], l1, p1[j]);
#pragma unroll
    for (int f = 0; f < 3; ++f) { p0[j][f] += X[k][f]; p1[j][f] += X[k][f]; }
    rad[j] = sp[6 * LN];
    hl[j] = sp[7 * LN];
  }
  static_assert(T::NPAIR <= 64, "the team's near-pair mask is 64 bits");
  unsigned long long near = 0ull;
  auto test = [&](const float* a0, const float* a1, float ra, float ha, bool sa, int, const float* b0, const float* b1,
                  float rb, float hb, bool sb, int, unsigned long long bit) {
    const float rr = ra + rb + off;
    float dc = 0.f;
#pragma unroll
    for (int k = 0; k < 3; ++k) {
      const float x = 0.5f * ((a0[k] + a1[k]) - (b0[k] + b1[k]));
      dc += x * x;
    }
    if (!sa && !sb) {
      if (dc < rr * rr) near |= bit;
      return;
    }
    const float rs = rr + (sa ? ha : 0.f) + (sb ? hb : 0.f);
    if (!(dc < rs * rs)) return;
    float d2;
    if (sa && sb) {
      d2 = seg_seg_d2(a0, a1, b0, b1);
    } else {
      const float* s0 = sa ? a0 : b0;
      const float* s1 = sa ? a1 : b1;
      const float* pt = sa ? b0 : a0;
      d2 = seg_pt_d2(s0, s1, pt);
    }
    if (d2 < rr * rr) near |= bit;
  };
  auto visit = [&](int lcv, auto&& f) {
#pragma unroll
    for (int sr = 0; sr < RSH; ++sr) {
      const float* rt = sct + ShapeTab<T>::ROOT + 8 * sr;
      const float l0[3] = {rt[0], rt[1], rt[2]}, l1[3] = {rt[3], rt[4], rt[5]};
      const float rr = rt[6], rhl = rt[7];
      float r0[3], r1[3];
      mat3vec(R0, l0, r0);
      mat3vec(R0, l1, r1);
#pragma unroll
      for (int j = 0; j < SPC; ++j)
        if (team_pair<T>(sr, RSH + j))
          f(r0, r1, rr, rhl, T::shkind[sr] == 1, sr, p0[j], p1[j], rad[j], hl[j], T::shkind[RSH + j] == 1,
            RSH + lcv * SPC + j, team_pair_bit<T>(lcv, sr, -1, 0, j));
    }
#pragma unroll
    for (int j = 0; j < SPC; ++j)
#pragma unroll
      for (int j2 = j + 1; j2 < SPC; ++j2)
        if (team_pair<T>(RSH + j, RSH + j2))
          f(p0[j], p1[j], rad[j], hl[j], T::shkind[RSH + j] == 1, RSH + lcv * SPC + j, p0[j2], p1[j2], rad[j2], hl[j2],
            T::shkind[RSH + j2] == 1, RSH + lcv * SPC + j2, team_pair_bit<T>(lcv, 0, j, 0, j2));
#pragma unroll
    for (int dl = 1; dl <= 2; ++dl) {
      float q0[SPC][3], q1[SPC][3];
#pragma unroll
      for (int j = 0; j < SPC; ++j) {
#pragma unroll
        for (int g = 0; g < 3; ++g) {
          q0[j][g] = dl == 1 ? qperm<0x39>(p0[j][g]) : qperm<0x4E>(p0[j][g]);
          q1[j][g] = dl == 1 ? qperm<0x39>(p1[j][g]) : qperm<0x4E>(p1[j][g]);
        }
      }
      if (dl == 1 || lcv < 2) {
        const int lo = (lcv + dl) & 3;
#pragma unroll
        for (int j = 0; j < SPC; ++j)
#pragma unroll
          for (int j2 = 0; j2 < SPC; ++j2)
            if (team_pair<T>(RSH + j, RSH + SPC + j2))
              f(p0[j], p1[j], rad[j], hl[j], T::shkind[RSH + j] == 1, RSH + lcv * SPC + j, q0[j2], q1[j2], rad[j2],
                hl[j2], T::shkind[RSH + j2] == 1, RSH + lo * SPC + j2, team_pair_bit<T>(lcv, 0, j, dl, j2));
      }
    }
  };
  visit(lc, test);
  if (__ballot(near != 0ull) == 0ull) return 0;
#ifdef GS_PHASE_PROFILE
  if ((threadIdx.x & 63) == 0) atomicAdd(&gs_phase_cycles[12], 1ull);
  const long long np_t0 = clock64();
#endif
  if constexpr (!team_closed_form<T>()) {
    return team_narrow_replicated<T, EPW>(M, P, mu_g, N, e, lc, R0, R, X, near, shw_tab, sct, pool);
  } else {
  constexpr int kLC = team_lc<T>(), kSt = kTeamSt;
  constexpr int kNone = 0x7fffffff;
  const int wl = threadIdx.x & 63;
  const int team = wl >> 2;
  float* lslot = shw_tab + wl;
  float* tstg = shw_tab + kLC * kSt * WL + team;
  static_assert(kLC * kSt * WL + T::NPK * kSt * TPW <= shw_size<T>() / WaveForm<EPW>::WAVES,
                "contact staging fits the wave's slice of the table");
  team_sync<EPW>();
  const float coff = P.contact_offset;
  int cnt = 0;
  int key[kLC];
#pragma unroll
  for (int i = 0; i < kLC; ++i) key[i] = kNone;
  auto narrow = [&](const float* a0_, const float* a1_, float ra_, float, bool sa, int ia, const float* b0_,
                    const float* b1_, float rb_, float, bool sb, int ib, unsigned long long bit) {
    if (!(near & bit)) return;
    const int q = __builtin_ctzll(bit);
    const bool sw = ia > ib;
    float a0[3], a1[3], b0[3], b1[3];
#pragma unroll
    for (int k = 0; k < 3; ++k) {
      a0[k] = sw ? b0_[k] : a0_[k]; a1[k] = sw ? b1_[k] : a1_[k];
      b0[k] = sw ? a0_[k] : b0_[k]; b1[k] = sw ? a1_[k] : b1_[k];
    }
    const float ra = sw ? rb_ : ra_, rb = sw ? ra_ : rb_;
    const int sha = sw ? ib : ia, shb = sw ? ia : ib;
    float pa[2][3], pb[2][3];
    int nct = 1;
    if (!sa && !sb) {
#pragma unroll
      for (int k = 0; k < 3; ++k) { pa[0][k] = a0[k]; pb[0][k] = b0[k]; }
    } else if (sa && sb) {
      float s, t, den, aa, ee;
      seg_seg_rcp(a0, a1, b0, b1, s, t, den, aa, ee);
      bool two = false;
      float lo = 0.f, hi = 0.f;
      if (aa > 1e-12f && ee > 1e-12f && den <= 1e-4f * aa * ee) {
        float d1[3], w0[3], w1[3];
#pragma unroll
        for (int k = 0; k < 3; ++k) { d1[k] = a1[k] - a0[k]; w0[k] = b0[k] - a0[k]; w1[k] = b1[k] - a0[k]; }
        const float ia = __builtin_amdgcn_rcpf(aa);
        const float s0 = dot3f(w0, d1) * ia, s1 = dot3f(w1, d1) * ia;
        lo = fminf(s0, s1);
        hi = fmaxf(s0, s1);
        lo = lo < 0.f ? 0.f : lo;
        hi = hi > 1.f ? 1.f : hi;
        two = hi - lo > 1e-3f;
      }
      if (two) {
        nct = 2;
#pragma unroll
        for (int c = 0; c < 2; ++c) {
          const float sc2 = c == 0 ? lo : hi;
#pragma unroll
          for (int k = 0; k < 3; ++k) pa[c][k] = a0[k] + sc2 * (a1[k] - a0[k]);
          seg_closest_pt_rcp(pa[c], b0, b1, pb[c]);
        }
      } else {
#pragma unroll
        for (int k = 0; k < 3; ++k) { pa[0][k] = a0[k] + s * (a1[k] - a0[k]); pb[0][k] = b0[k] + t * (b1[k] - b0[k]); }
      }
    } else {
      const bool capa = sw ? sb : sa;
      float e0[3], e1[3], pt[3], q3[3];
#pragma unroll
      for (int k = 0; k < 3; ++k) {
        e0[k] = capa ? a0[k] : b0[k]; e1[k] = capa ? a1[k] : b1[k]; pt[k] = capa ? b0[k] : a0[k];
      }
      seg_closest_pt_rcp(pt, e0, e1, q3);
#pragma unroll
      for (int k = 0; k < 3; ++k) { pa[0][k] = capa ? q3[k] : a0[k]; pb[0][k] = capa ? b0[k] : q3[k]; }
    }
#pragma unroll
    for (int c = 0; c < 2; ++c) {
      if (c >= nct) break;
      float nn[3] = {pa[c][0] - pb[c][0], pa[c][1] - pb[c][1], pa[c][2] - pb[c][2]};
      const float d2 = dot3f(nn, nn);
      float dist = sqrtf(d2);
      if (!(dist > 1e-9f)) {
        float f[3];
#pragma unroll
        for (int k = 0; k < 3; ++k) f[k] = 0.5f * ((a0[k] + a1[k]) - (b0[k] + b1[k]));
        float l = sqrtf(dot3f(f, f));
        if (!(l > 1e-9f)) { f[0] = 0.f; f[1] = 0.f; f[2] = 1.f; l = 1.f; }
#pragma unroll
        for (int k = 0; k < 3; ++k) nn[k] = f[k] / l;
        dist = 0.f;
      } else {
        const float idist = __builtin_amdgcn_rsqf(d2);
#pragma unroll
        for (int k = 0; k < 3; ++k) nn[k] *= idist;
      }
      const float sep = dist - ra - rb;
      if (!(sep < coff)) continue;
      const int kn = 2 * q + c;
      int slot = cnt < kLC ? cnt : -1;
      if (cnt >= kLC) {
        int m = 0, km = key[0];
#pragma unroll
        for (int i = 1; i < kLC; ++i) {
          m = key[i] > km ? i : m;
          km = key[i] > km ? key[i] : km;
        }
        slot = kn < km ? m : -1;
      }
      if (slot >= 0) {
        float* o = lslot + kSt * slot * WL;
#pragma unroll
        for (int k = 0; k < 3; ++k) {
          o[k * WL] = 0.5f * ((pa[c][k] - ra * nn[k]) + (pb[c][k] + rb * nn[k]));
          o[(3 + k) * WL] = nn[k];
        }
        o[6 * WL] = sep;
        o[7 * WL] = __int_as_float(sha);
        o[8 * WL] = __int_as_float(shb);
#pragma unroll
        for (int i = 0; i < kLC; ++i) key[i] = i == slot ? kn : key[i];
      }
      ++cnt;
    }
  };
  visit(opaque_index(lc), narrow);
#ifdef GS_PHASE_PROFILE
  if ((threadIdx.x & 63) == 0) atomicAdd(&gs_phase_cycles[14], (unsigned long long)(clock64() - np_t0));
#endif
  int cnt_team = 0;
  {
    int rk[kLC];
#pragma unroll
    for (int i = 0; i < kLC; ++i) rk[i] = 0;
    auto tally = [&](const int (&ks)[kLC]) {
#pragma unroll
      for (int j = 0; j < kLC; ++j)
#pragma unroll
        for (int i = 0; i < kLC; ++i) rk[i] += ks[j] < key[i];
    };
    tally(key);
    {
      int ks[kLC];
#pragma unroll
      for (int j = 0; j < kLC; ++j) ks[j] = qperm_i<0x39>(key[j]);
      tally(ks);
#pragma unroll
      for (int j = 0; j < kLC; ++j) ks[j] = qperm_i<0x4E>(key[j]);
      tally(ks);
#pragma unroll
      for (int j = 0; j < kLC; ++j) ks[j] = qperm_i<0x93>(key[j]);
      tally(ks);
    }
    cnt_team = cnt + qperm_i<0xB1>(cnt);
    cnt_team += qperm_i<0x4E>(cnt_team);
#pragma unroll
    for (int i = 0; i < kLC; ++i) {
      if (i < cnt && rk[i] < T::NPK) {
        const float* src = lslot + kSt * i * WL;
        float* dst = tstg + kSt * rk[i] * TPW;
#pragma unroll
        for (int f = 0; f < kSt; ++f) dst[f * TPW] = src[f * WL];
      }
    }
    team_sync<EPW>();
    cnt_team = cnt_team < T::NPK ? cnt_team : T::NPK;
#pragma unroll
    for (int r = 0; r < T::NPK; ++r) {
      if (r < cnt_team) {
        const float* src = tstg + kSt * r * TPW;
        float* o = pool + RowSlots<T>::PER_POOL * r * RW;
#pragma unroll
        for (int k = 0; k < 3; ++k) {
          o[(kPoolX + k) * RW] = src[k * TPW];
          o[(kPoolN + k) * RW] = src[(3 + k) * TPW];
        }
        o[kPoolSep * RW] = src[6 * TPW];
        const int a = __float_as_int(src[7 * TPW]), b = __float_as_int(src[8 * TPW]);
        const float nn[3] = {src[3 * TPW], src[4 * TPW], src[5 * TPW]};
        float t1[3], t2[3];
        gs_terrain::tangents(nn, t1, t2);
#pragma unroll
        for (int k = 0; k < 3; ++k) {
          o[(kPoolT1 + k) * RW] = t1[k];
          o[(kPoolT2 + k) * RW] = t2[k];
        }
        o[kPoolMu * RW] = 0.5f * (mu_g[a * N + e] + mu_g[b * N + e]);
        const int bla = (int)sct[kShC * a + 3], blb = (int)sct[kShC * b + 3];
        o[kPoolBA * RW] = (float)(bla >> 8);
        o[kPoolBB * RW] = (float)(blb >> 8);
        o[kPoolLA * RW] = (float)(bla & 255);
        o[kPoolLB * RW] = (float)(blb & 255);
      }
    }
  }
#ifdef GS_PHASE_PROFILE
  {
    const unsigned long long tm = quad_or64(near);
    const unsigned long long lanes = __ballot(tm != 0ull);
    if ((threadIdx.x & 63) == 0) {
      atomicAdd(&gs_phase_cycles[13], (unsigned long long)(clock64() - np_t0));
      atomicAdd(&gs_phase_cycles[15], (unsigned long long)__popcll(lanes));
      atomicAdd(&gs_phase_cycles[10], (unsigned long long)__popcll(tm));
    }
  }
#endif
  return cnt_team;
  }
}

__device__ __forceinline__ float terrain_candidate(const DevParams& P, const float* p, const float* x, float r,
                                                   float* nrm, float& smu) {
  const float cw[3] = {p[0] + x[0], p[1] + x[1], p[2] + x[2]};
  float dist = P.has_ground ? cw[2] - r : 3.0e38f;
  nrm[0] = 0.f; nrm[1] = 0.f; nrm[2] = 1.f;
  smu = P.ground_mu;
  float st, nt[3];
  if (gs_terrain::sphere_contact(P.terr, cw, r, r + P.contact_offset, st, nt) && st < dist) {
    dist = st;
    nrm[0] = nt[0]; nrm[1] = nt[1]; nrm[2] = nt[2];
    smu = P.terr.mu;
  }
  return dist;
}

template <class T, bool TERR, bool TGS, int EPW>
__device__ __forceinline__ void substep_team(const DevModel* __restrict__ Min, const float* __restrict__ mdl,
                                             const DevParams& P, TeamState<T>& s, const float* tau,
                                             const float* __restrict__ mu_t, int N, int e, int lc,
                                             float* __restrict__ rows_own, const float* __restrict__ rows_team,
                                             float* __restrict__ cf_soa, bool collect,
                                             float* __restrict__ cf_aos, float* __restrict__ shw_tab,
                                             const float* __restrict__ sct, float* __restrict__ stash GS_PROF_PARAM) {
  constexpr int CL = T::T_CL, CC = T::T_CC, RC = T::T_RC, NCH = T::T_NCH, LN = T::T_LANES;
  static_assert(NCH == LN && LN == 4, "lane teams are DPP quads with one chain per lane");
  using C = CM<T>;
  using RS = RowSlots<T>;
  uintptr_t mp = reinterpret_cast<uintptr_t>(Min);
  asm volatile("" : "+s"(mp));
  const DevModel* __restrict__ M = reinterpret_cast<const DevModel*>(mp);
  const float* cm = mdl + lc;
  const float h = P.h;

  float R0[9];
  {
    const float inv = rsqrtf(s.quat[0] * s.quat[0] + s.quat[1] * s.quat[1] + s.quat[2] * s.quat[2] +
                             s.quat[3] * s.quat[3]);
    const float qn[4] = {s.quat[0] * inv, s.quat[1] * inv, s.quat[2] * inv, s.quat[3] * inv};
    quat_to_mat(qn, R0);
  }
  const float X0[3] = {0.f, 0.f, 0.f};
  float nub[6] = {s.w[0], s.w[1], s.w[2], s.vo[0], s.vo[1], s.vo[2]};
  const float A0[6] = {0.f, 0.f, 0.f, -P.g[0], -P.g[1], -P.g[2]};
  SpI I0;
  body_inertia(R0, X0, M->mass[0], M->com[0], M->inertia[0], I0);
  float F0[6];
  {
    float ia[6], iv[6], x6[6];
    spi_mul(I0, A0, ia);
    spi_mul(I0, nub, iv);
    crf(nub, iv, x6);
#pragma unroll
    for (int k = 0; k < 6; ++k) F0[k] = ia[k] + x6[k];
  }

  struct TerrQ {
    float d[CC], n[CC][3], m[CC];
    float rd[RC > 0 ? RC : 1], rn[RC > 0 ? RC : 1][3], rm[RC > 0 ? RC : 1];
  };
  struct NoTerrQ {};
  [[maybe_unused]] std::conditional_t<TERR, TerrQ, NoTerrQ> tq;
  if constexpr (TERR) {
    constexpr int NQ = CC + 1;
    static_assert(RC <= LN, "one root candidate per lane of the team");
    float qc[NQ][3], qr[NQ];
    bool qv[NQ];
    float Rk[9], Xk[3] = {0.f, 0.f, 0.f};
#pragma unroll
    for (int f = 0; f < 9; ++f) Rk[f] = R0[f];
#pragma unroll
    for (int k = 0; k < CL; ++k) {
      const float* bp = cm + (k * C::BODY) * LN;
      float jR[9], jt[3], ax[3];
#pragma unroll
      for (int f = 0; f < 9; ++f) jR[f] = bp[f * LN];
#pragma unroll
      for (int f = 0; f < 3; ++f) { jt[f] = bp[(9 + f) * LN]; ax[f] = bp[(12 + f) * LN]; }
      float RJ[9], t[3], aw[3];
      mat3mul(Rk, jR, RJ);
      mat3vec(Rk, jt, t);
      Xk[0] += t[0]; Xk[1] += t[1]; Xk[2] += t[2];
      mat3vec(RJ, ax, aw);
      const float qj = s.q[k];
      if (T::jkind[1 + k] == 1) {
        float sn, cs;
        sincosf(qj, &sn, &cs);
        const float Cc = 1.f - cs;
        float Rq[9];
        Rq[0] = cs + ax[0] * ax[0] * Cc;         Rq[1] = ax[0] * ax[1] * Cc - ax[2] * sn; Rq[2] = ax[0] * ax[2] * Cc + ax[1] * sn;
        Rq[3] = ax[1] * ax[0] * Cc + ax[2] * sn; Rq[4] = cs + ax[1] * ax[1] * Cc;         Rq[5] = ax[1] * ax[2] * Cc - ax[0] * sn;
        Rq[6] = ax[2] * ax[0] * Cc - ax[1] * sn; Rq[7] = ax[2] * ax[1] * Cc + ax[0] * sn; Rq[8] = cs + ax[2] * ax[2] * Cc;
        mat3mul(RJ, Rq, Rk);
      } else {
#pragma unroll
        for (int f = 0; f < 9; ++f) Rk[f] = RJ[f];
        Xk[0] += aw[0] * qj; Xk[1] += aw[1] * qj; Xk[2] += aw[2] * qj;
      }
#pragma unroll
      for (int j = 0; j < CC; ++j) {
        if (T::T_ccb[j] == k) {
          const float* cp = cm + (C::CAND + 4 * j) * LN;
          const float pl[3] = {cp[0], cp[LN], cp[2 * LN]};
          float x[3];
          mat3vec(Rk, pl, x);
          x[0] += Xk[0]; x[1] += Xk[1]; x[2] += Xk[2];
#pragma unroll
          for (int f = 0; f < 3; ++f) qc[j][f] = s.p[f] + x[f];
          qr[j] = cp[3 * LN];
          qv[j] = true;
        }
      }
    }
    qv[CC] = lc < RC;
    qr[CC] = 0.f;
    qc[CC][0] = qc[CC][1] = qc[CC][2] = 0.f;
    if (lc < RC) {
      float x[3];
      mat3vec(R0, M->cpoint[lc], x);
#pragma unroll
      for (int f = 0; f < 3; ++f) qc[CC][f] = s.p[f] + x[f];
      qr[CC] = M->cradius[lc];
    }
    constexpr int kQItem = 9;
    static_assert(T::NPK > 0 && kShW * T::NS >= kQItem * (CC * LN + RC), "query list fits the pose table");
    float* ql = shw_tab;
    const int wl = threadIdx.x & 63;
    const unsigned long long below = (1ull << wl) - 1ull;
    int slot[NQ];
    int cnt = 0;
#ifdef GS_PHASE_PROFILE
    const long long tq0 = clock64();
#endif
#pragma unroll
    for (int q = 0; q < NQ; ++q) {
      const bool need = qv[q] && gs_terrain::may_contact(P.terr, qc[q], qr[q], qr[q] + P.contact_offset);
      const unsigned long long bal = __ballot(need);
      slot[q] = need ? cnt + __popcll(bal & below) : -1;
      if (need) {
        float* it = ql + slot[q] * kQItem;
        it[0] = qc[q][0]; it[1] = qc[q][1]; it[2] = qc[q][2]; it[3] = qr[q];
      }
      cnt += __popcll(bal);
    }
    team_sync<EPW>();
#ifdef GS_PHASE_PROFILE
    const long long tq1 = clock64();
#endif
    const unsigned long long live = __ballot(true);
    const int nlive = __popcll(live);
    for (int i = __popcll(live & below); i < cnt; i += nlive) {
      float* it = ql + i * kQItem;
      const float cw[3] = {it[0], it[1], it[2]};
      const float r = it[3];
      float st = 0.f, nt[3] = {0.f, 0.f, 1.f};
      const bool found = gs_terrain::sphere_contact_scan(P.terr, cw, r, r + P.contact_offset, st, nt);
      it[4] = found ? 1.f : 0.f;
      it[5] = st;
      it[6] = nt[0]; it[7] = nt[1]; it[8] = nt[2];
    }
    team_sync<EPW>();
#ifdef GS_PHASE_PROFILE
    if ((threadIdx.x & 63) == 0) {
      const long long tq2 = clock64();
      atomicAdd(&gs_phase_cycles[50], (unsigned long long)(tq1 - tq0));
      atomicAdd(&gs_phase_cycles[51], (unsigned long long)(tq2 - tq1));
      atomicAdd(&gs_phase_cycles[52], (unsigned long long)cnt);
    }
#endif
    float rd = 3.0e38f, rn[3] = {0.f, 0.f, 1.f}, rm = P.ground_mu;
#pragma unroll
    for (int q = 0; q < NQ; ++q) {
      float dist = P.has_ground ? qc[q][2] - qr[q] : 3.0e38f;
      float nrm[3] = {0.f, 0.f, 1.f};
      float smu = P.ground_mu;
      if (slot[q] >= 0) {
        const float* it = ql + slot[q] * kQItem;
        if (it[4] != 0.f && it[5] < dist) {
          dist = it[5];
          nrm[0] = it[6]; nrm[1] = it[7]; nrm[2] = it[8];
          smu = P.terr.mu;
        }
      }
      if (q < CC) {
        tq.d[q] = dist; tq.m[q] = smu;
        tq.n[q][0] = nrm[0]; tq.n[q][1] = nrm[1]; tq.n[q][2] = nrm[2];
      } else {
        rd = dist; rm = smu;
        rn[0] = nrm[0]; rn[1] = nrm[1]; rn[2] = nrm[2];
      }
    }
#pragma unroll
    for (int j = 0; j < RC; ++j) {
      tq.rd[j] = bcast(rd, j);
      tq.rm[j] = bcast(rm, j);
#pragma unroll
      for (int f = 0; f < 3; ++f) tq.rn[j][f] = bcast(rn[f], j);
    }
  }

  float R[CL][9], X[CL][3], S[CL][6], V[CL][6], A[CL][6], Fc[CL][6];
  SpI Ic[CL];
  bool act[CC];
  float sep[CC], cmu[CC];
  float cnrm[TERR ? CC : 1][3];
#pragma unroll
  for (int k = 0; k < CL; ++k) {
    const float* Rp = k == 0 ? R0 : R[k - 1];
    const float* Xp = k == 0 ? X0 : X[k - 1];
    const float* bp = cm + (k * C::BODY) * LN;
    float jR[9], jt[3], ax[3];
#pragma unroll
    for (int f = 0; f < 9; ++f) jR[f] = bp[f * LN];
#pragma unroll
    for (int f = 0; f < 3; ++f) { jt[f] = bp[(9 + f) * LN]; ax[f] = bp[(12 + f) * LN]; }
    float RJ[9], t[3], aw[3];
    mat3mul(Rp, jR, RJ);
    mat3vec(Rp, jt, t);
    X[k][0] = Xp[0] + t[0]; X[k][1] = Xp[1] + t[1]; X[k][2] = Xp[2] + t[2];
    mat3vec(RJ, ax, aw);
    const float qj = s.q[k];
    if (T::jkind[1 + k] == 1) {
      float sn, cs;
      sincosf(qj, &sn, &cs);
      const float Cc = 1.f - cs;
      float Rq[9];
      Rq[0] = cs + ax[0] * ax[0] * Cc;         Rq[1] = ax[0] * ax[1] * Cc - ax[2] * sn; Rq[2] = ax[0] * ax[2] * Cc + ax[1] * sn;
      Rq[3] = ax[1] * ax[0] * Cc + ax[2] * sn; Rq[4] = cs + ax[1] * ax[1] * Cc;         Rq[5] = ax[1] * ax[2] * Cc - ax[0] * sn;
      Rq[6] = ax[2] * ax[0] * Cc - ax[1] * sn; Rq[7] = ax[2] * ax[1] * Cc + ax[0] * sn; Rq[8] = cs + ax[2] * ax[2] * Cc;
      mat3mul(RJ, Rq, R[k]);
      S[k][0] = aw[0]; S[k][1] = aw[1]; S[k][2] = aw[2];
      cross3(X[k], aw, &S[k][3]);
    } else {
#pragma unroll
      for (int f = 0; f < 9; ++f) R[k][f] = RJ[f];
      X[k][0] += aw[0] * qj; X[k][1] += aw[1] * qj; X[k][2] += aw[2] * qj;
      S[k][0] = S[k][1] = S[k][2] = 0.f;
      S[k][3] = aw[0]; S[k][4] = aw[1]; S[k][5] = aw[2];
    }
  }
  GS_PROF(0)
  int npc = 0;
  float* pool = rows_own + RS::POOL * RW;
  if constexpr (T::NPK > 0) {
    if (P.self_collide) npc = team_self_contacts<T, EPW>(M, cm, P, mu_t, kTeamsPerBlock, 0, lc, R0, R, X, shw_tab, sct, pool);
  }
  GS_PROF(11)
#pragma unroll
  for (int k = 0; k < CL; ++k) {
    const float* Vp = k == 0 ? nub : V[k - 1];
    const float* Ap = k == 0 ? A0 : A[k - 1];
    const float* bp = cm + (k * C::BODY) * LN;
    const float qd = s.qd[k];
    float c6[6];
#pragma unroll
    for (int f = 0; f < 6; ++f) V[k][f] = Vp[f] + S[k][f] * qd;
    crm(V[k], S[k], c6);
#pragma unroll
    for (int f = 0; f < 6; ++f) A[k][f] = Ap[f] + c6[f] * qd;
    float com[3], Il[6];
#pragma unroll
    for (int f = 0; f < 3; ++f) com[f] = bp[(16 + f) * LN];
#pragma unroll
    for (int f = 0; f < 6; ++f) Il[f] = bp[(19 + f) * LN];
    body_inertia(R[k], X[k], bp[15 * LN], com, Il, Ic[k]);
    {
      float ia[6], iv[6], x6[6];
      spi_mul(Ic[k], A[k], ia);
      spi_mul(Ic[k], V[k], iv);
      crf(V[k], iv, x6);
#pragma unroll
      for (int f = 0; f < 6; ++f) Fc[k][f] = ia[f] + x6[f];
    }
#pragma unroll
    for (int j = 0; j < CC; ++j) {
      if (T::T_ccb[j] == k) {
        const float* cp = cm + (C::CAND + 4 * j) * LN;
        const float pl[3] = {cp[0], cp[LN], cp[2 * LN]};
        const float r = cp[3 * LN];
        float x[3];
        mat3vec(R[k], pl, x);
        x[0] += X[k][0]; x[1] += X[k][1]; x[2] += X[k][2];
        const int shape = T::T_RS + lc * T::T_SPC + T::T_ccs[j];
        if constexpr (TERR) {
          const float* nrm = tq.n[j];
          const float dist = tq.d[j], smu = tq.m[j];
          act[j] = dist < P.contact_offset;
          sep[j] = dist - P.rest_offset;
          cmu[j] = 0.5f * (mu_t[shape * kTeamsPerBlock] + smu);
          cnrm[j][0] = nrm[0]; cnrm[j][1] = nrm[1]; cnrm[j][2] = nrm[2];
          if (act[j]) {
            float dir[3][3];
            dir[0][0] = nrm[0]; dir[0][1] = nrm[1]; dir[0][2] = nrm[2];
            gs_terrain::tangents(nrm, dir[1], dir[2]);
            const float xc[3] = {x[0] - r * nrm[0], x[1] - r * nrm[1], x[2] - r * nrm[2]};
#pragma unroll
            for (int rr = 0; rr < 3; ++rr) {
              const float* d = dir[rr];
              float xd[3];
              cross3(xc, d, xd);
              float* row = rows_own + RS::chain(j) * RW;
#pragma unroll
              for (int b = 0; b < 6; ++b) row[RS::zs(rr, RS::zslot(b)) * RW] = b < 3 ? xd[b] : d[b - 3];
#pragma unroll
              for (int kk = 0; kk < CL; ++kk) {
                float v = 0.f;
                if (kk <= k)
                  v = S[kk][3] * d[0] + S[kk][4] * d[1] + S[kk][5] * d[2] + S[kk][0] * xd[0] + S[kk][1] * xd[1] +
                      S[kk][2] * xd[2];
                row[RS::zs(rr, RS::zslot(6 + kk)) * RW] = v;
              }
            }
          }
        } else {
        const float dist = s.p[2] + x[2] - r;
        act[j] = P.has_ground && (dist < P.contact_offset);
        sep[j] = dist - P.rest_offset;
        cmu[j] = 0.5f * (mu_t[shape * kTeamsPerBlock] + P.ground_mu);
        if (act[j]) {
          const float xc[3] = {x[0], x[1], x[2] - r};
#pragma unroll
          for (int rr = 0; rr < 3; ++rr) {
            const int ax3 = (rr == 0) ? 2 : (rr == 1 ? 0 : 1);
            float* row = rows_own + RS::chain(j) * RW;
#pragma unroll
            for (int b = 0; b < 6; ++b) row[RS::zs(rr, RS::zslot(b)) * RW] = base_jac(xc, ax3, b);
#pragma unroll
            for (int kk = 0; kk < CL; ++kk) {
              float v = 0.f;
              if (kk <= k) {
                float tt[3];
                cross3(S[kk], xc, tt);
                v = S[kk][3 + ax3] + tt[ax3];
              }
              row[RS::zs(rr, RS::zslot(6 + kk)) * RW] = v;
            }
          }
        }
        }
      }
    }
  }

  GS_PROF(0)
  float Mcc[CL][CL], Mcb[CL][6], biasc[CL];
#pragma unroll
  for (int kk = 0; kk < CL; ++kk) {
    const int k = CL - 1 - kk;
    if (k < CL - 1) {
      Ic[k].m += Ic[k + 1].m;
#pragma unroll
      for (int f = 0; f < 3; ++f) Ic[k].h[f] += Ic[k + 1].h[f];
#pragma unroll
      for (int f = 0; f < 6; ++f) Ic[k].I[f] += Ic[k + 1].I[f];
#pragma unroll
      for (int f = 0; f < 6; ++f) Fc[k][f] += Fc[k + 1][f];
    }
    biasc[k] = dot6(S[k], Fc[k]);
    float Fk[6];
    spi_mul(Ic[k], S[k], Fk);
    Mcc[k][k] = dot6(S[k], Fk) + cm[(C::DOF + 3 * k + 2) * LN];
#pragma unroll
    for (int j = 0; j < k; ++j) Mcc[k][j] = dot6(S[j], Fk);
#pragma unroll
    for (int b = 0; b < 6; ++b) Mcb[k][b] = Fk[b];
  }
  float Fb[6], Mbb[6][6];
  SpI Ir;
  {
#pragma unroll
    for (int f = 0; f < 6; ++f) Fb[f] = F0[f] + quad_sum(Fc[0][f]);
    Ir.m = I0.m + quad_sum(Ic[0].m);
#pragma unroll
    for (int f = 0; f < 3; ++f) Ir.h[f] = I0.h[f] + quad_sum(Ic[0].h[f]);
#pragma unroll
    for (int f = 0; f < 6; ++f) Ir.I[f] = I0.I[f] + quad_sum(Ic[0].I[f]);
    Mbb[0][0] = Ir.I[0]; Mbb[1][1] = Ir.I[1]; Mbb[2][2] = Ir.I[2];
    Mbb[1][0] = Ir.I[3]; Mbb[2][0] = Ir.I[4]; Mbb[2][1] = Ir.I[5];
    Mbb[3][0] = 0.f;       Mbb[3][1] = Ir.h[2];  Mbb[3][2] = -Ir.h[1];
    Mbb[4][0] = -Ir.h[2];  Mbb[4][1] = 0.f;      Mbb[4][2] = Ir.h[0];
    Mbb[5][0] = Ir.h[1];   Mbb[5][1] = -Ir.h[0]; Mbb[5][2] = 0.f;
    Mbb[3][3] = Ir.m; Mbb[4][4] = Ir.m; Mbb[5][5] = Ir.m;
    Mbb[4][3] = 0.f; Mbb[5][3] = 0.f; Mbb[5][4] = 0.f;
  }

  {
    float corr[6][6];
#pragma unroll
    for (int a = 0; a < 6; ++a)
#pragma unroll
      for (int b = 0; b <= a; ++b) corr[a][b] = 0.f;
#pragma unroll
    for (int kk = 0; kk < CL; ++kk) {
      const int k = CL - 1 - kk;
      const float dinv = __builtin_amdgcn_rcpf(Mcc[k][k]);
#pragma unroll
      for (int jj = 0; jj < CL; ++jj) {
        const int j = k - 1 - jj;
        if (j >= 0) {
          const float a = Mcc[k][j] * dinv;
#pragma unroll
          for (int i = 0; i <= j; ++i) Mcc[j][i] -= a * Mcc[k][i];
#pragma unroll
          for (int b = 0; b < 6; ++b) Mcb[j][b] -= a * Mcb[k][b];
          Mcc[k][j] = a;
        }
      }
#pragma unroll
      for (int bb = 0; bb < 6; ++bb) {
        const int b = 5 - bb;
        const float a = Mcb[k][b] * dinv;
#pragma unroll
        for (int i = 0; i <= b; ++i) corr[b][i] -= a * Mcb[k][i];
        Mcb[k][b] = a;
      }
    }
#pragma unroll
    for (int a = 0; a < 6; ++a)
#pragma unroll
      for (int b = 0; b <= a; ++b) Mbb[a][b] += quad_sum(corr[a][b]);
  }
#pragma unroll
  for (int kk = 0; kk < 6; ++kk) {
    const int k = 5 - kk;
    const float dinv = __builtin_amdgcn_rcpf(Mbb[k][k]);
#pragma unroll
    for (int ii = 0; ii < 6; ++ii) {
      const int i = k - 1 - ii;
      if (i >= 0) {
        const float a = Mbb[k][i] * dinv;
#pragma unroll
        for (int j = 0; j <= i; ++j) Mbb[i][j] -= a * Mbb[k][j];
        Mbb[k][i] = a;
      }
    }
  }
  float sDc[CL], sDb[6];
#pragma unroll
  for (int k = 0; k < CL; ++k) sDc[k] = rsqrtf(Mcc[k][k]);
#pragma unroll
  for (int k = 0; k < 6; ++k) sDb[k] = rsqrtf(Mbb[k][k]);

  GS_PROF(1)
  float nufc[CL], nufb[6];
  {
    float rc[CL], rb[6], rcorr[6];
#pragma unroll
    for (int k = 0; k < CL; ++k) {
      float t = tau[k];
      const float ef = cm[(C::DOF + 3 * k + 0) * LN];
      if (ef > 0.f) t = clampf(t, -ef, ef);
      rc[k] = t - biasc[k];
    }
#pragma unroll
    for (int b = 0; b < 6; ++b) { rb[b] = -Fb[b]; rcorr[b] = 0.f; }
#pragma unroll
    for (int kk = 0; kk < CL; ++kk) {
      const int k = CL - 1 - kk;
#pragma unroll
      for (int j = 0; j < k; ++j) rc[j] -= Mcc[k][j] * rc[k];
#pragma unroll
      for (int b = 0; b < 6; ++b) rcorr[b] -= Mcb[k][b] * rc[k];
    }
#pragma unroll
    for (int b = 0; b < 6; ++b) rb[b] += quad_sum(rcorr[b]);
#pragma unroll
    for (int kk = 0; kk < 6; ++kk) {
      const int k = 5 - kk;
#pragma unroll
      for (int b = 0; b < k; ++b) rb[b] -= Mbb[k][b] * rb[k];
    }
#pragma unroll
    for (int b = 0; b < 6; ++b) rb[b] *= sDb[b] * sDb[b];
#pragma unroll
    for (int k = 0; k < CL; ++k) rc[k] *= sDc[k] * sDc[k];
#pragma unroll
    for (int k = 0; k < 6; ++k)
#pragma unroll
      for (int b = 0; b < k; ++b) rb[k] -= Mbb[k][b] * rb[b];
#pragma unroll
    for (int k = 0; k < CL; ++k) {
#pragma unroll
      for (int b = 0; b < 6; ++b) rc[k] -= Mcb[k][b] * rb[b];
#pragma unroll
      for (int j = 0; j < k; ++j) rc[k] -= Mcc[k][j] * rc[j];
    }
#pragma unroll
    for (int b = 0; b < 6; ++b) nufb[b] = nub[b] + h * rb[b];
#pragma unroll
    for (int k = 0; k < CL; ++k) nufc[k] = s.qd[k] + h * rc[k];
    float wxp[3];
    cross3(&nub[0], &nub[3], wxp);
    nufb[3] += h * wxp[0]; nufb[4] += h * wxp[1]; nufb[5] += h * wxp[2];
  }

  GS_PROF(2)
  const float inv_h = 1.f / h;
#pragma unroll
  for (int j = 0; j < CC; ++j) {
    float* rec = rows_own + RS::chain(j) * RW;
    rec[RS::C_ACT * RW] = act[j] ? 1.f : 0.f;
    if (act[j]) {
      const int kb = T::T_ccb[j];
      float zr[3][6 + CL], dir[3];
#pragma unroll
      for (int rr = 0; rr < 3; ++rr) {
        float* row = rows_own + RS::chain(j) * RW;
        auto Z = [&](int sl) -> float& { return row[RS::zs(rr, sl) * RW]; };
        float zb[6], zc[CL];
        float cj = 0.f;
#pragma unroll
        for (int b = 0; b < 6; ++b) { zb[b] = Z(RS::zslot(b)); cj += zb[b] * nufb[b]; }
#pragma unroll
        for (int k = 0; k < CL; ++k) { zc[k] = Z(RS::zslot(6 + k)); if (k <= kb) cj += zc[k] * nufc[k]; }
#pragma unroll
        for (int kk = 0; kk < CL; ++kk) {
          const int k = kb - kk;
          if (k >= 0) {
#pragma unroll
            for (int i = 0; i < k; ++i) zc[i] -= Mcc[k][i] * zc[k];
#pragma unroll
            for (int b = 0; b < 6; ++b) zb[b] -= Mcb[k][b] * zc[k];
          }
        }
#pragma unroll
        for (int kk = 0; kk < 6; ++kk) {
          const int k = 5 - kk;
#pragma unroll
          for (int b = 0; b < k; ++b) zb[b] -= Mbb[k][b] * zb[k];
        }
        float d = 0.f;
#pragma unroll
        for (int b = 0; b < 6; ++b) {
          zb[b] *= sDb[b];
          d += zb[b] * zb[b];
          Z(RS::zslot(b)) = zb[b];
          zr[rr][b] = zb[b];
        }
#pragma unroll
        for (int k = 0; k < CL; ++k) {
          const float z = k <= kb ? zc[k] * sDc[k] : 0.f;
          d += z * z;
          Z(RS::zslot(6 + k)) = z;
          zr[rr][6 + k] = z;
        }
        Z(3) = 0.f;
        Z(7) = 0.f;
        Z(11) = 0.f;
        Z(12) = 0.f;
        Z(13) = 0.f;
        Z(14) = 0.f;
        Z(RS::CSLOT) = cj;
        dir[rr] = d > 0.f ? __builtin_amdgcn_rcpf(d) : 0.f;
        rec[(RS::C_DI + rr) * RW] = dir[rr];
      }
      float g10 = 0.f, g20 = 0.f, g21 = 0.f;
#pragma unroll
      for (int f = 0; f < 6 + CL; ++f) {
        g10 += zr[1][f] * zr[0][f];
        g20 += zr[2][f] * zr[0][f];
        g21 += zr[2][f] * zr[1][f];
      }
      rec[(RS::C_G + 0) * RW] = g10 * dir[1];
      rec[(RS::C_G + 1) * RW] = g20 * dir[2];
      rec[(RS::C_G + 2) * RW] = g21 * dir[2];
      const float sc = sep[j];
      const float tgt = -sc * inv_h;
      rec[RS::C_TP * RW] = (sc < 0.f ? fminf(tgt, P.max_depen_vel) : tgt) * dir[0];
      rec[RS::C_TV * RW] = (sc < 0.f ? 0.f : tgt) * dir[0];
      rec[RS::C_MU * RW] = cmu[j];
      rec[RS::C_SEP * RW] = sc;
    }
  }
  bool ract[RC > 0 ? RC : 1];
  float rnrm[TERR && RC > 0 ? RC : 1][3];
#pragma unroll
  for (int j = 0; j < RC; ++j) {
    float x[3];
    mat3vec(R0, M->cpoint[j], x);
    const float r = M->cradius[j];
    float dist, rmu_s = P.ground_mu;
    float rdir[3][3];
    if constexpr (TERR) {
      dist = tq.rd[j];
      rmu_s = tq.rm[j];
#pragma unroll
      for (int f = 0; f < 3; ++f) rnrm[j][f] = tq.rn[j][f];
      ract[j] = dist < P.contact_offset;
      rdir[0][0] = rnrm[j][0]; rdir[0][1] = rnrm[j][1]; rdir[0][2] = rnrm[j][2];
      gs_terrain::tangents(rnrm[j], rdir[1], rdir[2]);
    } else {
      dist = s.p[2] + x[2] - r;
      ract[j] = P.has_ground && (dist < P.contact_offset);
    }
    if (ract[j]) {
      float* rec = rows_own + RS::root(j) * RW;
      const float xc[3] = {TERR ? x[0] - r * rdir[0][0] : x[0], TERR ? x[1] - r * rdir[0][1] : x[1],
                           TERR ? x[2] - r * rdir[0][2] : x[2] - r};
      float zr[3][6], dir[3];
#pragma unroll
      for (int rr = 0; rr < 3; ++rr) {
        const int ax3 = (rr == 0) ? 2 : (rr == 1 ? 0 : 1);
        float zb[6], cj = 0.f;
        float xd[3] = {0.f, 0.f, 0.f};
        if constexpr (TERR) cross3(xc, rdir[rr], xd);
#pragma unroll
        for (int b = 0; b < 6; ++b) {
          zb[b] = TERR ? (b < 3 ? xd[b] : rdir[rr][b - 3]) : base_jac(xc, ax3, b);
          cj += zb[b] * nufb[b];
        }
#pragma unroll
        for (int kk = 0; kk < 6; ++kk) {
          const int k = 5 - kk;
#pragma unroll
          for (int b = 0; b < k; ++b) zb[b] -= Mbb[k][b] * zb[k];
        }
        float d = 0.f;
#pragma unroll
        for (int b = 0; b < 6; ++b) {
          zb[b] *= sDb[b];
          d += zb[b] * zb[b];
          rec[RS::zs(rr, RS::zslot(b)) * RW] = zb[b];
          zr[rr][b] = zb[b];
        }
        auto Z = [&](int sl) -> float& { return rec[RS::zs(rr, sl) * RW]; };
#pragma unroll
        for (int k = 0; k < 3; ++k) {
          Z(4 * k + 2) = 0.f;
          Z(4 * k + 3) = 0.f;
        }
        Z(12) = 0.f;
        Z(13) = 0.f;
        Z(14) = 0.f;
        Z(RS::CSLOT) = cj;
        dir[rr] = d > 0.f ? __builtin_amdgcn_rcpf(d) : 0.f;
        rec[(RS::R_DI + rr) * RW] = dir[rr];
      }
      float g10 = 0.f, g20 = 0.f, g21 = 0.f;
#pragma unroll
      for (int f = 0; f < 6; ++f) {
        g10 += zr[1][f] * zr[0][f];
        g20 += zr[2][f] * zr[0][f];
        g21 += zr[2][f] * zr[1][f];
      }
      rec[(RS::R_G + 0) * RW] = g10 * dir[1];
      rec[(RS::R_G + 1) * RW] = g20 * dir[2];
      rec[(RS::R_G + 2) * RW] = g21 * dir[2];
      const float sc = dist - P.rest_offset;
      const float tgt = -sc * inv_h;
      rec[RS::R_TP * RW] = (sc < 0.f ? fminf(tgt, P.max_depen_vel) : tgt) * dir[0];
      rec[RS::R_TV * RW] = (sc < 0.f ? 0.f : tgt) * dir[0];
      rec[RS::R_MU * RW] = 0.5f * (mu_t[T::T_rcs[j] * kTeamsPerBlock] + rmu_s);
      rec[RS::R_SEP * RW] = sc;
    }
  }
  if constexpr (T::NPK > 0) {
    for (int p = 0; p < npc; ++p) {
      float* o = pool + RS::PER_POOL * p * RW;
      const int ba = (int)o[kPoolBA * RW], bb = (int)o[kPoolBB * RW];
      const int ca = ba > 0 ? (ba - 1) / CL : -1, ka = ba > 0 ? (ba - 1) - ca * CL : -1;
      const int cb = bb > 0 ? (bb - 1) / CL : -1, kb = bb > 0 ? (bb - 1) - cb * CL : -1;
      const float x[3] = {o[kPoolX * RW], o[(kPoolX + 1) * RW], o[(kPoolX + 2) * RW]};
      float zr[3][6], zc3[3][CL], dd[3];
#pragma unroll
      for (int rr = 0; rr < 3; ++rr) {
        const int dofs = rr == 0 ? kPoolN : (rr == 1 ? kPoolT1 : kPoolT2);
        const float d[3] = {o[dofs * RW], o[(dofs + 1) * RW], o[(dofs + 2) * RW]};
        float zc[CL], zbc[6];
        float cpart = 0.f;
#pragma unroll
        for (int k = 0; k < CL; ++k) {
          const float coef = (lc == ca && k <= ka ? 1.f : 0.f) - (lc == cb && k <= kb ? 1.f : 0.f);
          float vx[3];
          cross3(S[k], x, vx);
          zc[k] = coef * (d[0] * (S[k][3] + vx[0]) + d[1] * (S[k][4] + vx[1]) + d[2] * (S[k][5] + vx[2]));
          cpart += zc[k] * nufc[k];
        }
#pragma unroll
        for (int b = 0; b < 6; ++b) zbc[b] = 0.f;
#pragma unroll
        for (int kk = 0; kk < CL; ++kk) {
          const int k = CL - 1 - kk;
#pragma unroll
          for (int i = 0; i < k; ++i) zc[i] -= Mcc[k][i] * zc[k];
#pragma unroll
          for (int b = 0; b < 6; ++b) zbc[b] -= Mcb[k][b] * zc[k];
        }
        float zb[6];
#pragma unroll
        for (int b = 0; b < 6; ++b) zb[b] = quad_sum(zbc[b]);
#pragma unroll
        for (int kk = 0; kk < 6; ++kk) {
          const int k = 5 - kk;
#pragma unroll
          for (int b = 0; b < k; ++b) zb[b] -= Mbb[k][b] * zb[k];
        }
        float own = 0.f, db = 0.f;
#pragma unroll
        for (int b = 0; b < 6; ++b) { zb[b] *= sDb[b]; db += zb[b] * zb[b]; zr[rr][b] = zb[b]; }
#pragma unroll
        for (int k = 0; k < CL; ++k) { zc[k] *= sDc[k]; own += zc[k] * zc[k]; zc3[rr][k] = zc[k]; }
        dd[rr] = db + quad_sum(own);
        const float cj = quad_sum(cpart);
        float za = 0.f, zbb = 0.f;
#pragma unroll
        for (int l = 0; l < CL; ++l) {
          float va = 0.f, vb = 0.f;
#pragma unroll
          for (int L = 0; L < 4; ++L) {
            const float t = bcast(zc[l], L);
            va = L == ca ? t : va;
            vb = L == cb ? t : vb;
          }
          za = lc == l ? va : za;
          zbb = lc == l ? vb : zbb;
        }
        if (cb == ca) zbb = 0.f;
        const float b0 = lc == 0 ? zb[0] : (lc == 1 ? zb[2] : (lc == 2 ? zb[4] : 0.f));
        const float b1 = lc == 0 ? zb[1] : (lc == 1 ? zb[3] : (lc == 2 ? zb[5] : 0.f));
        float* zo = o + (RS::P_Z + 5 * rr) * RW;
        zo[0] = b0;
        zo[RW] = b1;
        zo[2 * RW] = za;
        zo[3 * RW] = zbb;
        zo[4 * RW] = lc == 3 ? cj : 0.f;
      }
      float g10 = 0.f, g20 = 0.f, g21 = 0.f, c10 = 0.f, c20 = 0.f, c21 = 0.f;
#pragma unroll
      for (int b = 0; b < 6; ++b) {
        g10 += zr[1][b] * zr[0][b];
        g20 += zr[2][b] * zr[0][b];
        g21 += zr[2][b] * zr[1][b];
      }
#pragma unroll
      for (int k = 0; k < CL; ++k) {
        c10 += zc3[1][k] * zc3[0][k];
        c20 += zc3[2][k] * zc3[0][k];
        c21 += zc3[2][k] * zc3[1][k];
      }
      g10 += quad_sum(c10);
      g20 += quad_sum(c20);
      g21 += quad_sum(c21);
      float di[3];
#pragma unroll
      for (int rr = 0; rr < 3; ++rr) {
        di[rr] = dd[rr] > GS_MIN_RESPONSE ? __builtin_amdgcn_rcpf(dd[rr]) : 0.f;
        o[(RS::P_DI + rr) * RW] = di[rr];
        o[(kPoolLam + rr) * RW] = 0.f;
      }
      o[(RS::P_G + 0) * RW] = g10 * di[1];
      o[(RS::P_G + 1) * RW] = g20 * di[2];
      o[(RS::P_G + 2) * RW] = g21 * di[2];
      const float sc = o[kPoolSep * RW];
      const float tgt = -sc * inv_h;
      o[RS::P_TP * RW] = (sc < 0.f ? fminf(tgt, P.max_depen_vel) : tgt) * di[0];
      o[RS::P_TV * RW] = (sc < 0.f ? 0.f : tgt) * di[0];
      o[RS::P_CA * RW] = (float)ca;
      o[RS::P_CB * RW] = (float)(cb == ca ? -1 : cb);
    }
  }
  team_sync<EPW>();

  GS_PROF(3)
  auto stash_io = [&](bool save) {
    int q = 0;
    auto io = [&](float& v) {
      if (save) stash[q * kTeamBlock] = v; else v = stash[q * kTeamBlock];
      ++q;
    };
#pragma unroll
    for (int k = 0; k < 6; ++k) {
#pragma unroll
      for (int b = 0; b < k; ++b) io(Mbb[k][b]);
      io(sDb[k]);
      io(nufb[k]);
    }
#pragma unroll
    for (int k = 0; k < CL; ++k) {
#pragma unroll
      for (int b = 0; b < 6; ++b) io(Mcb[k][b]);
#pragma unroll
      for (int j = 0; j < k; ++j) io(Mcc[k][j]);
      io(sDc[k]);
      io(nufc[k]);
    }
  };
  stash_io(true);
  static_assert(CL == 3, "component distribution assumes 3-dof chains");
  float wA = 0.f, wA2 = 0.f, wC[NCH];
#pragma unroll
  for (int c = 0; c < NCH; ++c) wC[c] = 0.f;
  float lamc[NCH][CC][3], lamr[RC > 0 ? RC : 1][3];
#pragma unroll
  for (int c = 0; c < NCH; ++c)
#pragma unroll
    for (int j = 0; j < CC; ++j) lamc[c][j][0] = lamc[c][j][1] = lamc[c][j][2] = 0.f;
#pragma unroll
  for (int j = 0; j < RC; ++j) lamr[j][0] = lamr[j][1] = lamr[j][2] = 0.f;
  float wbp[6], wcp[CL];
  const int iters = P.pos_iters + P.vel_iters;
  constexpr bool tgs = TGS;
  const float hs = tgs ? h / (float)P.pos_iters : h, inv_hs = 1.f / hs;
  [[maybe_unused]] float aA = 0.f, aA2 = 0.f, aC[NCH];
#pragma unroll
  for (int c = 0; c < NCH; ++c) aC[c] = 0.f;
  for (int it = 0; it < iters; ++it) {
    const int tsel = it < P.pos_iters ? RS::C_TP : RS::C_TV;
    const int rsel = it < P.pos_iters ? RS::R_TP : RS::R_TV;
    const bool pos = it < P.pos_iters;
    const float na = (float)(it < P.pos_iters ? it : P.pos_iters);
    const float kgap = pos ? inv_hs : inv_h, cap = pos ? P.max_depen_vel : 0.f;
    auto tgs_tdi = [&](float sc, float su, float di0) {
      const float sep = fmaf(hs, su, sc);
      const float t = sep >= 0.f ? -sep * kgap : fminf(-sep * inv_h, cap);
      return t * di0;
    };
#pragma unroll
    for (int j = 0; j < RC; ++j) {
      if (ract[j]) {
        const float* rec = rows_own + RS::root(j) * RW;
        float z[12], u[4];
#pragma unroll
        for (int i = 0; i < 12; ++i) z[i] = rec[RS::zs(i >> 2, 4 * lc + (i & 3)) * RW];
        {
          const f2 u01 = pk_fma(f2{z[0], z[4]}, f2{wA, wA}, pk_fma(f2{z[1], z[5]}, f2{wA2, wA2}, f2{z[3], z[7]}));
          u[0] = u01.x;
          u[1] = u01.y;
        }
        u[2] = fmaf(z[8], wA, fmaf(z[9], wA2, z[11]));
        float tdi;
        if constexpr (tgs) {
          u[3] = fmaf(z[0], aA, fmaf(z[1], aA2, na * z[3]));
          quad_sum4(u);
          tdi = tgs_tdi(rec[RS::R_SEP * RW], u[3], rec[RS::R_DI * RW]);
        } else {
          quad_sum3(u);
          tdi = rec[rsel * RW];
        }
        float dl0, dl1, dl2;
        contact_block(u[0], u[1], u[2], rec[RS::R_DI * RW], rec[(RS::R_DI + 1) * RW], rec[(RS::R_DI + 2) * RW],
                      rec[RS::R_G * RW], rec[(RS::R_G + 1) * RW], rec[(RS::R_G + 2) * RW], tdi,
                      rec[RS::R_MU * RW], lamr[j], dl0, dl1, dl2);
        wA = fmaf(z[8], dl2, fmaf(z[4], dl1, fmaf(z[0], dl0, wA)));
        wA2 = fmaf(z[9], dl2, fmaf(z[5], dl1, fmaf(z[1], dl0, wA2)));
      }
    }
    float nact, nz[12], nk[8];
    auto fetch = [&](int n) {
      const int cc = n / CC, j = n - (n / CC) * CC;
      const float* rec = rows_team + cc + RS::chain(j) * RW;
      nact = rec[RS::C_ACT * RW];
#pragma unroll
      for (int i = 0; i < 12; ++i) nz[i] = rec[RS::zs(i >> 2, 4 * lc + (i & 3)) * RW];
#pragma unroll
      for (int i = 0; i < 6; ++i) nk[i] = rec[(RS::C_DI + i) * RW];
      nk[6] = rec[(tgs ? RS::C_SEP : tsel) * RW];
      nk[7] = rec[RS::C_MU * RW];
    };
    fetch(0);
#pragma unroll
    for (int n = 0; n < NCH * CC; ++n) {
      const int cc = n / CC, j = n - (n / CC) * CC;
      float z[12], k8[8];
      const float act_n = nact;
#pragma unroll
      for (int i = 0; i < 12; ++i) z[i] = nz[i];
#pragma unroll
      for (int i = 0; i < 8; ++i) k8[i] = nk[i];
#ifdef GS_PGS_FENCE
      __builtin_amdgcn_sched_barrier(0);
#endif
      if (n + 1 < NCH * CC) fetch(n + 1);
      const bool a_o = act_n != 0.f;
#ifdef GS_PHASE_PROFILE
      if (__ballot(a_o) != 0ull) GS_PROF_COUNT(8, 1)
#endif
      if (a_o) {
        float u[4];
        {
          const f2 u01 = pk_fma(f2{z[0], z[4]}, f2{wA, wA},
                                pk_fma(f2{z[1], z[5]}, f2{wA2, wA2}, pk_fma(f2{z[2], z[6]}, f2{wC[cc], wC[cc]},
                                                                         f2{z[3], z[7]})));
          u[0] = u01.x;
          u[1] = u01.y;
        }
        u[2] = fmaf(z[8], wA, fmaf(z[9], wA2, fmaf(z[10], wC[cc], z[11])));
        float tdi = k8[6];
        if constexpr (tgs) {
          u[3] = fmaf(z[0], aA, fmaf(z[1], aA2, fmaf(z[2], aC[cc], na * z[3])));
          quad_sum4(u);
          tdi = tgs_tdi(k8[6], u[3], k8[0]);
        } else {
          quad_sum3(u);
        }
        float dl0, dl1, dl2;
        contact_block(u[0], u[1], u[2], k8[0], k8[1], k8[2], k8[3], k8[4], k8[5], tdi, k8[7], lamc[cc][j], dl0,
                      dl1, dl2);
        wA = fmaf(z[8], dl2, fmaf(z[4], dl1, fmaf(z[0], dl0, wA)));
        wA2 = fmaf(z[9], dl2, fmaf(z[5], dl1, fmaf(z[1], dl0, wA2)));
        wC[cc] = fmaf(z[10], dl2, fmaf(z[6], dl1, fmaf(z[2], dl0, wC[cc])));
      }
    }
    if constexpr (T::NPK > 0) {
      const int psel = it < P.pos_iters ? RS::P_TP : RS::P_TV;
      float pz[15], pk[11];
      int pca = 0, pcb = 0;
      auto pfetch = [&](int p) {
        const float* o = pool + RS::PER_POOL * p * RW;
#pragma unroll
        for (int i = 0; i < 15; ++i) pz[i] = o[(RS::P_Z + i) * RW];
#pragma unroll
        for (int i = 0; i < 3; ++i) {
          pk[i] = o[(kPoolLam + i) * RW];
          pk[3 + i] = o[(RS::P_DI + i) * RW];
          pk[6 + i] = o[(RS::P_G + i) * RW];
        }
        pk[9] = o[(tgs ? (int)kPoolSep : psel) * RW];
        pk[10] = o[kPoolMu * RW];
        pca = (int)o[RS::P_CA * RW];
        pcb = (int)o[RS::P_CB * RW];
      };
      const unsigned long long any_pool = __ballot(npc > 0);
      if (any_pool) pfetch(0);
#pragma unroll
      for (int p = 0; p < T::NPK; ++p) {
        if (__ballot(p < npc) == 0ull) break;
        float z[15], k11[11];
#pragma unroll
        for (int i = 0; i < 15; ++i) z[i] = pz[i];
#pragma unroll
        for (int i = 0; i < 11; ++i) k11[i] = pk[i];
        const int ca = pca, cb = pcb;
        if (p + 1 < T::NPK) pfetch(p + 1);
        if (p < npc) {
          float wa = 0.f, wb = 0.f, ana = 0.f, anb = 0.f;
#pragma unroll
          for (int c = 0; c < NCH; ++c) {
            wa = c == ca ? wC[c] : wa;
            wb = c == cb ? wC[c] : wb;
            ana = c == ca ? aC[c] : ana;
            anb = c == cb ? aC[c] : anb;
          }
          float u[4];
#pragma unroll
          for (int rr = 0; rr < 3; ++rr)
            u[rr] = fmaf(z[5 * rr], wA, fmaf(z[5 * rr + 1], wA2, fmaf(z[5 * rr + 2], wa, fmaf(z[5 * rr + 3], wb, z[5 * rr + 4]))));
          float lam[3] = {k11[0], k11[1], k11[2]};
          float tdi = k11[9];
          if constexpr (tgs) {
            u[3] = fmaf(z[0], aA, fmaf(z[1], aA2, fmaf(z[2], ana, fmaf(z[3], anb, na * z[4]))));
            quad_sum4(u);
            tdi = tgs_tdi(k11[9], u[3], k11[3]);
          } else {
            quad_sum3(u);
          }
          float dl0, dl1, dl2;
          contact_block(u[0], u[1], u[2], k11[3], k11[4], k11[5], k11[6], k11[7], k11[8], tdi, k11[10], lam, dl0, dl1,
                        dl2);
          float* o = pool + RS::PER_POOL * p * RW;
          o[kPoolLam * RW] = lam[0];
          o[(kPoolLam + 1) * RW] = lam[1];
          o[(kPoolLam + 2) * RW] = lam[2];
          wA = fmaf(z[10], dl2, fmaf(z[5], dl1, fmaf(z[0], dl0, wA)));
          wA2 = fmaf(z[11], dl2, fmaf(z[6], dl1, fmaf(z[1], dl0, wA2)));
          const float da = fmaf(z[12], dl2, fmaf(z[7], dl1, z[2] * dl0));
          const float db = fmaf(z[13], dl2, fmaf(z[8], dl1, z[3] * dl0));
#pragma unroll
          for (int c = 0; c < NCH; ++c) wC[c] += (c == ca ? da : 0.f) + (c == cb ? db : 0.f);
        }
      }
    }
#ifdef GS_PHASE_PROFILE
    for (int j = 0; j < RC; ++j)
      if (__ballot(ract[j]) != 0ull) GS_PROF_COUNT(9, 1)
#endif
    if (tgs && pos) {
      aA += wA;
      aA2 += wA2;
#pragma unroll
      for (int c = 0; c < NCH; ++c) aC[c] += wC[c];
    }
    if (it == P.pos_iters - 1) {
      if constexpr (tgs) {
        const float inv_n = 1.f / (float)P.pos_iters;
        float mC[NCH];
#pragma unroll
        for (int c = 0; c < NCH; ++c) mC[c] = aC[c] * inv_n;
        gather_w<T>(lc, aA * inv_n, aA2 * inv_n, mC, wbp, wcp);
      } else {
        gather_w<T>(lc, wA, wA2, wC, wbp, wcp);
      }
    }
  }
  float wb[6], wc[CL];
  gather_w<T>(lc, wA, wA2, wC, wb, wc);
  if (P.pos_iters <= 0) {
#pragma unroll
    for (int b = 0; b < 6; ++b) wbp[b] = wb[b];
#pragma unroll
    for (int k = 0; k < CL; ++k) wcp[k] = wc[k];
  }
  team_sync<EPW>();
  stash_io(false);

  GS_PROF(4)
  float nunb[6], nupb[6], nunc[CL], nupc[CL];
#pragma unroll
  for (int k = 0; k < 6; ++k) {
    float v = wb[k] * sDb[k], vp = wbp[k] * sDb[k];
#pragma unroll
    for (int b = 0; b < k; ++b) { v -= Mbb[k][b] * nunb[b]; vp -= Mbb[k][b] * nupb[b]; }
    nunb[k] = v;
    nupb[k] = vp;
  }
#pragma unroll
  for (int k = 0; k < CL; ++k) {
    float v = wc[k] * sDc[k], vp = wcp[k] * sDc[k];
#pragma unroll
    for (int b = 0; b < 6; ++b) { v -= Mcb[k][b] * nunb[b]; vp -= Mcb[k][b] * nupb[b]; }
#pragma unroll
    for (int j = 0; j < k; ++j) { v -= Mcc[k][j] * nunc[j]; vp -= Mcc[k][j] * nupc[j]; }
    nunc[k] = v;
    nupc[k] = vp;
  }
#pragma unroll
  for (int b = 0; b < 6; ++b) { nunb[b] += nufb[b]; nupb[b] += nufb[b]; }
#pragma unroll
  for (int k = 0; k < CL; ++k) {
    float vn = nunc[k] + nufc[k], vp = nupc[k] + nufc[k];
    const float vm = cm[(C::DOF + 3 * k + 1) * LN];
    if (vm > 0.f) { vn = clampf(vn, -vm, vm); vp = clampf(vp, -vm, vm); }
    nunc[k] = vn;
    nupc[k] = vp;
  }

  s.p[0] += h * nupb[3]; s.p[1] += h * nupb[4]; s.p[2] += h * nupb[5];
  {
    const float wx = nupb[0], wy = nupb[1], wz = nupb[2];
    float x = s.quat[0], y = s.quat[1], z = s.quat[2], w = s.quat[3];
    const float hh = 0.5f * h;
    const float dx = hh * (w * wx + wy * z - wz * y);
    const float dy = hh * (w * wy + wz * x - wx * z);
    const float dz = hh * (w * wz + wx * y - wy * x);
    const float dw = -hh * (wx * x + wy * y + wz * z);
    x += dx; y += dy; z += dz; w += dw;
    const float n = rsqrtf(x * x + y * y + z * z + w * w);
    s.quat[0] = x * n; s.quat[1] = y * n; s.quat[2] = z * n; s.quat[3] = w * n;
  }
  s.w[0] = nunb[0]; s.w[1] = nunb[1]; s.w[2] = nunb[2];
  s.vo[0] = nunb[3]; s.vo[1] = nunb[4]; s.vo[2] = nunb[5];
#pragma unroll
  for (int k = 0; k < CL; ++k) {
    s.q[k] += h * nupc[k];
    s.qd[k] = nunc[k];
  }
  if (collect) {
    e = opaque_index(e);
#pragma unroll
    for (int k = 0; k < CL; ++k) {
      float f0 = 0.f, f1 = 0.f, f2 = 0.f;
#pragma unroll
      for (int j = 0; j < CC; ++j) {
        if (T::T_ccb[j] == k) {
          float l0 = lamc[0][j][0], l1 = lamc[0][j][1], l2 = lamc[0][j][2];
#pragma unroll
          for (int c = 1; c < NCH; ++c) {
            l0 = lc == c ? lamc[c][j][0] : l0;
            l1 = lc == c ? lamc[c][j][1] : l1;
            l2 = lc == c ? lamc[c][j][2] : l2;
          }
          if constexpr (TERR) {
            float t1[3], t2[3];
            gs_terrain::tangents(cnrm[j], t1, t2);
            f0 += (l0 * cnrm[j][0] + l1 * t1[0] + l2 * t2[0]) * inv_h;
            f1 += (l0 * cnrm[j][1] + l1 * t1[1] + l2 * t2[1]) * inv_h;
            f2 += (l0 * cnrm[j][2] + l1 * t1[2] + l2 * t2[2]) * inv_h;
          } else {
            f0 += l1 * inv_h;
            f1 += l2 * inv_h;
            f2 += l0 * inv_h;
          }
        }
      }
      if constexpr (T::NPK > 0) {
        for (int p = 0; p < npc; ++p) {
          const float* o = pool + RS::PER_POOL * p * RW;
          const int bk = 1 + lc * CL + k;
          const float sg = ((int)o[kPoolBA * RW] == bk ? inv_h : 0.f) - ((int)o[kPoolBB * RW] == bk ? inv_h : 0.f);
          if (sg != 0.f) {
            const float l0 = o[kPoolLam * RW], l1 = o[(kPoolLam + 1) * RW], l2 = o[(kPoolLam + 2) * RW];
            f0 += sg * (l0 * o[kPoolN * RW] + l1 * o[kPoolT1 * RW] + l2 * o[kPoolT2 * RW]);
            f1 += sg * (l0 * o[(kPoolN + 1) * RW] + l1 * o[(kPoolT1 + 1) * RW] + l2 * o[(kPoolT2 + 1) * RW]);
            f2 += sg * (l0 * o[(kPoolN + 2) * RW] + l1 * o[(kPoolT1 + 2) * RW] + l2 * o[(kPoolT2 + 2) * RW]);
          }
        }
      }
      const int b = 1 + lc * CL + k;
      cf_soa[(3 * b + 0) * N + e] = f0;
      cf_soa[(3 * b + 1) * N + e] = f1;
      cf_soa[(3 * b + 2) * N + e] = f2;
      if (cf_aos) {
        float* o = cf_aos + ((size_t)e * T::NB + b) * 3;
        o[0] = f0; o[1] = f1; o[2] = f2;
      }
    }
    if (lc == 0) {
      float f0 = 0.f, f1 = 0.f, f2 = 0.f;
#pragma unroll
      for (int j = 0; j < RC; ++j) {
        if constexpr (TERR) {
          float t1[3], t2[3];
          gs_terrain::tangents(rnrm[j], t1, t2);
          const float g = ract[j] ? inv_h : 0.f;
          f0 += (lamr[j][0] * rnrm[j][0] + lamr[j][1] * t1[0] + lamr[j][2] * t2[0]) * g;
          f1 += (lamr[j][0] * rnrm[j][1] + lamr[j][1] * t1[1] + lamr[j][2] * t2[1]) * g;
          f2 += (lamr[j][0] * rnrm[j][2] + lamr[j][1] * t1[2] + lamr[j][2] * t2[2]) * g;
        } else {
          f0 += lamr[j][1] * inv_h;
          f1 += lamr[j][2] * inv_h;
          f2 += lamr[j][0] * inv_h;
        }
      }
      if constexpr (T::NPK > 0) {
        for (int p = 0; p < npc; ++p) {
          const float* o = pool + RS::PER_POOL * p * RW;
          const float sg = ((int)o[kPoolBA * RW] == 0 ? inv_h : 0.f) - ((int)o[kPoolBB * RW] == 0 ? inv_h : 0.f);
          if (sg != 0.f) {
            const float l0 = o[kPoolLam * RW], l1 = o[(kPoolLam + 1) * RW], l2 = o[(kPoolLam + 2) * RW];
            f0 += sg * (l0 * o[kPoolN * RW] + l1 * o[kPoolT1 * RW] + l2 * o[kPoolT2 * RW]);
            f1 += sg * (l0 * o[(kPoolN + 1) * RW] + l1 * o[(kPoolT1 + 1) * RW] + l2 * o[(kPoolT2 + 1) * RW]);
            f2 += sg * (l0 * o[(kPoolN + 2) * RW] + l1 * o[(kPoolT1 + 2) * RW] + l2 * o[(kPoolT2 + 2) * RW]);
          }
        }
      }
      cf_soa[0 * N + e] = f0;
      cf_soa[1 * N + e] = f1;
      cf_soa[2 * N + e] = f2;
      if (cf_aos) {
        float* o = cf_aos + (size_t)e * T::NB * 3;
        o[0] = f0; o[1] = f1; o[2] = f2;
      }
    }
  }
  GS_PROF(5)
}

template <class T>
__device__ __forceinline__ void team_com_velocity(const DevModel* __restrict__ M, const TeamState<T>& s, float* v) {
  float R[9], c[3], wc[3];
  quat_to_mat(s.quat, R);
  mat3vec(R, M->root_com, c);
  cross3(s.w, c, wc);
  v[0] = s.vo[0] + wc[0]; v[1] = s.vo[1] + wc[1]; v[2] = s.vo[2] + wc[2];
}

__device__ __forceinline__ int xcd_block(int b, int G) {
  constexpr int kXcd = 8;
  const int per = G / kXcd, rem = G % kXcd, x = b % kXcd, q = b / kXcd;
  return x * per + (x < rem ? x : rem) + q;
}

struct TeamLane {
  int wave, col, lc, e;
  bool on;
};
template <class T, int EPW>
__device__ __forceinline__ TeamLane team_lane(int N) {
  constexpr int LN = T::T_LANES;
  static_assert(WaveForm<EPW>::WAVES == 1 || shw_size<T>() % WaveForm<EPW>::WAVES == 0, "every wave its own slice");
  TeamLane t;
  t.wave = WaveForm<EPW>::kWhole ? 0 : (int)(threadIdx.x / GS_WAVE);
  t.col = team_column<EPW>();
  t.lc = threadIdx.x & (LN - 1);
  t.on = WaveForm<EPW>::kWhole || (int)(threadIdx.x & (GS_WAVE - 1)) < WaveForm<EPW>::LANES;
  t.e = t.on ? (xcd_block(blockIdx.x, gridDim.x) * kTeamBlock + t.col) / LN : N;
  return t;
}

template <class T, bool TERR, bool TGS, int EPW>
__global__ __launch_bounds__(WaveForm<EPW>::THREADS, 1) void k_simulate_team(const DevModel* __restrict__ M, DevParams P,
                                                                 SimBuffers B, const float* __restrict__ tau_aos) {
  constexpr int LN = T::T_LANES, CL = T::T_CL, ND = T::ND;
  __shared__ float mdl[CM<T>::NP * LN];
  __shared__ float rows[RowSlots<T>::TOTAL * RW];
  __shared__ float shw_tab[shw_size<T>()];
  __shared__ float sct[ShapeTab<T>::SIZE];
  __shared__ float mu_tab[T::NS * kTeamsPerBlock];
  __shared__ float stash_tab[team_stash_size<T>() * kTeamBlock];
  stage_chain_model<T>(M, mdl);
  stage_shape_consts<T>(M, sct);
  const TeamLane tl = team_lane<T, EPW>(B.N);
  const int lc = tl.lc, e = tl.e, col = tl.col;
  if (tl.on)
    for (int sh = lc; sh < T::NS; sh += LN)
      mu_tab[sh * kTeamsPerBlock + (col >> 2)] = e < B.N ? B.mu[(size_t)sh * B.N + e] : 1.f;
  __syncthreads();
  if (e >= B.N) return;
  const float* mu_t = mu_tab + (col >> 2);
  float* shw_wave = shw_tab + tl.wave * (shw_size<T>() / WaveForm<EPW>::WAVES);
  const int N = B.N;
  TeamState<T> s;
  team_load<T>(B.state, N, e, lc, s);
  float tau[CL];
#pragma unroll
  for (int k = 0; k < CL; ++k) tau[k] = tau_aos ? tau_aos[(size_t)e * ND + lc * CL + k] : 0.f;
  float* own = rows + col;
  const float* team = rows + (col & ~(LN - 1));
  GS_PROF_DECL
  for (int sstep = 0; sstep < P.substeps; ++sstep) {
    const bool last = (sstep == P.substeps - 1) && P.collect;
    substep_team<T, TERR, TGS, EPW>(M, mdl, P, s, tau, mu_t, N, e, lc, own, team, B.cf, last, nullptr, shw_wave, sct, stash_tab + col GS_PROF_ARGS);
  }
  team_store<T>(B.state, N, opaque_index(e), opaque_index(lc), s);
  GS_PROF_FLUSH
}

template <class T, bool TERR, bool TGS, int EPW>
__global__ __launch_bounds__(WaveForm<EPW>::THREADS, 1) void k_pd_step_team(const DevModel* __restrict__ M, DevParams P,
                                                                SimBuffers B, PdDev A) {
  constexpr int LN = T::T_LANES, CL = T::T_CL, ND = T::ND, NB = T::NB;
  __shared__ float mdl[CM<T>::NP * LN];
  __shared__ float rows[RowSlots<T>::TOTAL * RW];
  __shared__ float shw_tab[shw_size<T>()];
  __shared__ float sct[ShapeTab<T>::SIZE];
  __shared__ float mu_tab[T::NS * kTeamsPerBlock];
  __shared__ float stash_tab[team_stash_size<T>() * kTeamBlock];
  stage_chain_model<T>(M, mdl);
  stage_shape_consts<T>(M, sct);
  const TeamLane tl = team_lane<T, EPW>(B.N);
  const int lc = tl.lc, e = tl.e, col = tl.col;
  if (tl.on)
    for (int sh = lc; sh < T::NS; sh += LN)
      mu_tab[sh * kTeamsPerBlock + (col >> 2)] = e < B.N ? B.mu[(size_t)sh * B.N + e] : 1.f;
  __syncthreads();
  if (e >= B.N) return;
  const float* mu_t = mu_tab + (col >> 2);
  float* shw_wave = shw_tab + tl.wave * (shw_size<T>() / WaveForm<EPW>::WAVES);
  const int N = B.N;
  TeamState<T> s;
  team_load<T>(B.state, N, e, lc, s);
  float tau[CL];
  float* own = rows + col;
  const float* team = rows + (col & ~(LN - 1));
  const int sub = P.substeps;
  const int n_pd = A.decimation * sub;
  const int total = (A.decimation + A.extra) * sub;
  auto dof0 = [&]() { return (size_t)opaque_index(e) * ND + lc * CL; };
  GS_PROF_DECL
  for (int it = 0; it < total; ++it) {
    if (it < n_pd && (it % sub) == 0) {
      const bool first = it == 0;
      const size_t d0 = dof0();
#pragma unroll
      for (int k = 0; k < CL; ++k) {
        const float qj = first ? A.dof_state_in[(d0 + k) * 2 + 0] : s.q[k];
        const float qdj = first ? A.dof_state_in[(d0 + k) * 2 + 1] : s.qd[k];
        const float aj = A.actions[d0 + k];
        tau[k] = clampf(A.kp * (A.scale * aj + A.default_pos[lc * CL + k] - qj) - A.kd * qdj, -A.tlim, A.tlim);
      }
    }
    const bool last = ((it % sub) == sub - 1) && P.collect;
    GS_PROF(6)
    float* cf_aos = (it == total - 1) ? A.cf_out : nullptr;
    substep_team<T, TERR, TGS, EPW>(M, mdl, P, s, tau, mu_t, N, e, lc, own, team, B.cf, last, cf_aos, shw_wave, sct, stash_tab + col GS_PROF_ARGS);
    if (it == n_pd - 1 && A.dof_out) {
      const size_t d0 = dof0();
#pragma unroll
      for (int k = 0; k < CL; ++k) {
        A.dof_out[(d0 + k) * 2 + 0] = s.q[k];
        A.dof_out[(d0 + k) * 2 + 1] = s.qd[k];
      }
    }
  }
  team_store<T>(B.state, N, opaque_index(e), opaque_index(lc), s);
  const size_t d0 = dof0();
#pragma unroll
  for (int k = 0; k < CL; ++k) A.torques_out[d0 + k] = tau[k];
  if (A.actions_copy) {
#pragma unroll
    for (int k = 0; k < CL; ++k) A.actions_copy[d0 + k] = A.actions[d0 + k];
  }
  if (A.root_out && lc == 0) {
    float* o = A.root_out + (size_t)e * 13;
    o[0] = s.p[0]; o[1] = s.p[1]; o[2] = s.p[2];
    o[3] = s.quat[0]; o[4] = s.quat[1]; o[5] = s.quat[2]; o[6] = s.quat[3];
    float v[3];
    team_com_velocity<T>(M, s, v);
    o[7] = v[0]; o[8] = v[1]; o[9] = v[2];
    o[10] = s.w[0]; o[11] = s.w[1]; o[12] = s.w[2];
  }
  if constexpr (!TERR && EPW == 16) if (kTeamsPerBlock == 16 && A.tail_on) {
    __syncthreads();
    const bool reset = lc == 0 && (ND == 12 ? gt_tail::post_a_env<true, false, (ND == 12 ? 12 : 0)>(
                                                  A.tail_p, A.tail_b, gt_anymal_hound{}, e)
                                            : gt_tail::post_a_env<true, false>(A.tail_p, A.tail_b, gt_anymal_hound{}, e));
    const unsigned long long m = __ballot(reset);
    unsigned m16 = 0;
#pragma unroll
    for (int i = 0; i < kTeamsPerBlock; ++i) m16 |= (unsigned)((m >> (LN * i)) & 1ull) << i;
    const int e0 = e - (int)(threadIdx.x / LN);
    const unsigned long long live = __ballot(true);
    if ((int)(threadIdx.x & 63) == __ffsll((long long)live) - 1) {
      uint16_t* slices = reinterpret_cast<uint16_t*>(A.tail_b.reset_masks);
      slices[e0 / kTeamsPerBlock] = (uint16_t)m16;
      if (e0 + kTeamsPerBlock >= N)
        for (int q = e0 / kTeamsPerBlock + 1; q % 4 != 0; ++q) slices[q] = 0;
      gt_tail::publish_count(A.tail_b, (unsigned)__popc(m16), gridDim.x);
    }
  }
  GS_PROF(7)
  GS_PROF_FLUSH
}

}

bool team_fused_tail_available() { return kTeamsPerBlock == 16; }

constexpr int kTeamEpwPlane = 4, kTeamEpwTerr = 16;
static int team_epw(const DevParams& P, bool tail) {
  if (kTeamBlock != GS_WAVE || tail) return 16;
  const int w = P.team_epw > 0 ? P.team_epw : (P.has_terrain ? kTeamEpwTerr : kTeamEpwPlane);
  return w == 8 || w == 4 ? w : 16;
}
#define GS_TEAM_LAUNCH_EPW(K, EPW, ...)                                                                      \
  do {                                                                                                       \
    const dim3 g_((unsigned)blocks), b_((unsigned)WaveForm<EPW>::THREADS);                                   \
    if (P.has_terrain && P.tgs) hipLaunchKernelGGL((K<T, true, true, EPW>), g_, b_, 0, st, __VA_ARGS__);     \
    else if (P.has_terrain) hipLaunchKernelGGL((K<T, true, false, EPW>), g_, b_, 0, st, __VA_ARGS__);        \
    else if (P.tgs) hipLaunchKernelGGL((K<T, false, true, EPW>), g_, b_, 0, st, __VA_ARGS__);                \
    else hipLaunchKernelGGL((K<T, false, false, EPW>), g_, b_, 0, st, __VA_ARGS__);                          \
  } while (0)
#define GS_TEAM_LAUNCH(K, epw, ...)                              \
  do {                                                           \
    if constexpr (kTeamBlock == GS_WAVE) {                       \
      if ((epw) == 8) { GS_TEAM_LAUNCH_EPW(K, 8, __VA_ARGS__); break; }  \
      if ((epw) == 4) { GS_TEAM_LAUNCH_EPW(K, 4, __VA_ARGS__); break; }  \
    }                                                            \
    GS_TEAM_LAUNCH_EPW(K, 16, __VA_ARGS__);                      \
  } while (0)

template <class T>
hipError_t launch_sim_team(const DevModel* M, const DevParams& P, const SimBuffers& B, const float* tau,
                           hipStream_t st) {
  if constexpr (T::HAS_TEAM) {
    static_assert(T::NR == T::NB, "the lane team reports contact forces per body (no kept fixed-joint links)");
    const long lanes = (long)B.N * T::T_LANES;
    const int blocks = (int)((lanes + kTeamBlock - 1) / kTeamBlock);
    GS_TEAM_LAUNCH(k_simulate_team, team_epw(P, false), M, P, B, tau);
    return hipGetLastError();
  } else {
    return hipErrorInvalidConfiguration;
  }
}
template <class T>
hipError_t launch_pd_team(const DevModel* M, const DevParams& P, const SimBuffers& B, const PdDev& A, hipStream_t st) {
  if constexpr (T::HAS_TEAM) {
    const long lanes = (long)B.N * T::T_LANES;
    const int blocks = (int)((lanes + kTeamBlock - 1) / kTeamBlock);
    GS_TEAM_LAUNCH(k_pd_step_team, team_epw(P, A.tail_on != 0), M, P, B, A);
    return hipGetLastError();
  } else {
    return hipErrorInvalidConfiguration;
  }
}

#define GS_TEAM_ENTRY(T, SIG) {SIG, T::HAS_TEAM ? &launch_sim_team<T> : nullptr, T::HAS_TEAM ? &launch_pd_team<T> : nullptr},
TeamEntry g_team_kernels[] = {GS_FOR_EACH_TOPOLOGY(GS_TEAM_ENTRY)};
const int g_num_team_kernels = sizeof(g_team_kernels) / sizeof(g_team_kernels[0]);

extern "C" int gs_debug_phase_cycles(unsigned long long* out, int n, int reset) {
#ifdef GS_PHASE_PROFILE
  if (!out || n <= 0 || n > 64) return -1;
  if (hipDeviceSynchronize() != hipSuccess) return -1;
  if (hipMemcpyFromSymbol(out, HIP_SYMBOL(gs_phase_cycles), sizeof(unsigned long long) * n) != hipSuccess) return -1;
  if (reset) {
    unsigned long long z[64] = {0};
    if (hipMemcpyToSymbol(HIP_SYMBOL(gs_phase_cycles), z, sizeof(z)) != hipSuccess) return -1;
  }
  return 0;
#else
  (void)out; (void)n; (void)reset;
  return -1;
#endif
}
```

isaacgymenv_amd/isaacgym/_lib.py:

```python
from __future__ import annotations

import ctypes as C
import os

_HERE = os.path.dirname(os.path.dirname(os.path.abspath(__file__)))
LIB_PATH = os.path.join(_HERE, "_lib", os.environ.get("GS_LIBGYMSIM", "libgymsim.so"))


class GsModelDesc(C.Structure):
    _fields_ = [("num_bodies", C.c_int32), ("num_dofs", C.c_int32), ("num_candidates", C.c_int32),
                ("num_shapes", C.c_int32), ("fixed_base", C.c_int32)] + [
        (n, C.c_void_p) for n in ("parent", "joint_kind", "body_dof", "joint_origin", "joint_axis", "mass",
                                  "com", "inertia", "cand_body", "cand_point", "cand_radius", "cand_shape",
                                  "dof_effort", "dof_velocity", "dof_armature", "dof_lower", "dof_upper",
                                  "dof_has_limits")] + [
        ("num_links", C.c_int32)] + [(n, C.c_void_p) for n in ("cand_link", "link_body", "link_pose", "link_com")] + [
        (n, C.c_void_p) for n in ("cand_dyn", "shape_kind", "shape_body", "shape_link", "shape_pose", "shape_size",
                                  "shape_margin", "shape_sphere")] + [
        ("num_hull_verts", C.c_int32), ("hull_verts", C.c_void_p), ("shape_hv0", C.c_void_p),
        ("shape_hv1", C.c_void_p), ("num_pairs", C.c_int32), ("pair_a", C.c_void_p), ("pair_b", C.c_void_p),
        ("pair_kind", C.c_void_p), ("pair_pool", C.c_int32), ("num_pair_verts", C.c_int32), ("pair_verts", C.c_void_p),
        ("shape_pv0", C.c_void_p), ("shape_pv1", C.c_void_p)]


class GsSimParams(C.Structure):
    _fields_ = [("dt", C.c_double), ("substeps", C.c_int32), ("gravity", C.c_double * 3),
                ("num_position_iterations", C.c_int32), ("num_velocity_iterations", C.c_int32),
                ("contact_offset", C.c_double), ("rest_offset", C.c_double),
                ("bounce_threshold_velocity", C.c_double), ("max_depenetration_velocity", C.c_double),
                ("contact_collection", C.c_int32), ("kernel_variant", C.c_int32),
                ("joint_limit_margin", C.c_double), ("num_threads", C.c_int32),
                ("solver_type", C.c_int32)]


class GsPdArgs(C.Structure):
    _fields_ = [("actions", C.c_void_p), ("default_pos", C.c_void_p), ("kp", C.c_float), ("kd", C.c_float),
                ("action_scale", C.c_float), ("torque_limit", C.c_float), ("decimation", C.c_int32),
                ("extra_simulates", C.c_int32), ("torques_out", C.c_void_p), ("dof_state_out", C.c_void_p),
                ("root_state_out", C.c_void_p), ("contact_out", C.c_void_p), ("actions_copy_out", C.c_void_p),
                ("tail_params", C.c_void_p), ("tail_buffers", C.c_void_p)]


_lib = None


GS_ABI = 9


def lib():
    global _lib
    if _lib is None:
        if not os.path.exists(LIB_PATH):
            raise RuntimeError(f"{LIB_PATH} is missing: build it with `python -m isaacgymenv_amd.build` "
                               "(hipcc, gfx950). There is no CPU fallback.")
        L = C.CDLL(LIB_PATH)
        L.gs_abi_version.restype = C.c_int
        if L.gs_abi_version() != GS_ABI:
            raise RuntimeError(f"{LIB_PATH} has gymsim ABI {L.gs_abi_version()}, this binding needs {GS_ABI}: "
                               "rebuild it with `python -m isaacgymenv_amd.build`")
        vp, i, f, d = C.c_void_p, C.c_int, C.c_float, C.c_double
        sig = {
            "gs_abi_version": (i, []),
            "gs_last_error": (C.c_char_p, []),
            "gs_topology_supported": (i, [C.POINTER(GsModelDesc)]),
            "gs_sim_create": (vp, [i, C.POINTER(GsSimParams)]),
            "gs_sim_destroy": (None, [vp]),
            "gs_sim_add_ground": (i, [vp, d, d, d]),
            "gs_sim_set_model": (i, [vp, C.POINTER(GsModelDesc)]),
            "gs_sim_prepare": (i, [vp, i, vp, vp, vp]),
            "gs_sim_simulate": (i, [vp, vp, vp]),
            "gs_sim_refresh_root": (i, [vp, vp, vp]),
            "gs_sim_refresh_dof": (i, [vp, vp, vp]),
            "gs_sim_refresh_contact": (i, [vp, vp, vp]),
            "gs_sim_refresh_rigid_body": (i, [vp, vp, vp]),
            "gs_sim_refresh_jacobian": (i, [vp, vp, vp]),
            "gs_sim_refresh_mass_matrix": (i, [vp, vp, vp]),
            "gs_sim_set_root": (i, [vp, vp, vp, i, vp]),
            "gs_sim_set_dof": (i, [vp, vp, vp, i, vp]),
            "gs_sim_pd_step": (i, [vp, C.POINTER(GsPdArgs), vp]),
            "gs_sim_kernel_variant": (i, [vp]),
            "gs_sim_enable_timing": (i, [vp, i]),
            "gs_sim_last_kernel_ms": (f, [vp]),
            "gs_debug_phase_cycles": (i, [vp, i, i]),
            "gs_sim_set_force_sensors": (i, [vp, i, vp]),
            "gs_sim_bind_force_sensors": (i, [vp, vp]),
            "gs_sim_set_dof_drives": (i, [vp, vp, vp, vp]),
            "gs_sim_bind_dof_targets": (i, [vp, vp, vp]),
            "gs_sim_bind_dof_properties_env": (i, [vp, vp, i, i]),
            "gs_sim_pd_tail_supported": (i, [vp]),
            "gs_sim_set_root_and_dof": (i, [vp, vp, vp, vp, i, vp]),
            "gs_sim_set_self_collision": (i, [vp, i]),
            "gs_sim_refresh_force_sensor": (i, [vp, vp, vp]),
            "gs_sim_add_triangle_mesh": (i, [vp, vp, C.c_int64, vp, C.c_int64, vp, d, d, d]),
            "gs_debug_terrain_query": (i, [vp, vp, vp, i, vp, vp]),
            "gs_debug_self_contacts": (i, [vp, i, vp, vp, vp]),
        }
        for name, (res, args) in sig.items():
            fn = getattr(L, name)
            fn.restype = res
            fn.argtypes = args
        _lib = L
    return _lib


def check(rc: int, what: str) -> None:
    if rc != 0:
        raise RuntimeError(f"{what} failed: {lib().gs_last_error().decode()}")


EXPORTED_SYMBOLS = [
    "gs_abi_version", "gs_last_error", "gs_topology_supported", "gs_sim_create", "gs_sim_destroy",
    "gs_sim_add_ground", "gs_sim_set_model", "gs_sim_prepare", "gs_sim_simulate", "gs_sim_refresh_root",
    "gs_sim_refresh_dof", "gs_sim_refresh_contact", "gs_sim_set_root", "gs_sim_set_dof", "gs_sim_pd_step",
    "gs_sim_kernel_variant", "gs_sim_enable_timing", "gs_sim_last_kernel_ms", "gs_debug_phase_cycles",
    "gs_sim_set_force_sensors", "gs_sim_bind_force_sensors", "gs_sim_refresh_force_sensor",
    "gs_sim_add_triangle_mesh", "gs_debug_terrain_query", "gs_sim_refresh_rigid_body", "gs_sim_refresh_jacobian",
    "gs_sim_refresh_mass_matrix", "gs_sim_set_dof_drives", "gs_sim_bind_dof_targets", "gs_sim_set_self_collision",
    "gs_debug_self_contacts", "gs_sim_bind_dof_properties_env", "gs_sim_pd_tail_supported", "gs_sim_set_root_and_dof",
]


def model_desc(flat: dict):
    import numpy as np
    keep = {}
    m = GsModelDesc()
    m.num_bodies, m.num_dofs, m.num_candidates = flat["nb"], flat["nd"], flat["nc"]
    m.num_shapes, m.fixed_base = flat["ns"], flat["fixed_base"]
    pairs = [("parent", "parent", np.int32), ("joint_kind", "jkind", np.int32), ("body_dof", "bdof", np.int32),
             ("joint_origin", "jorigin", np.float64), ("joint_axis", "jaxis", np.float64),
             ("mass", "mass", np.float64), ("com", "com", np.float64), ("inertia", "inertia", np.float64),
             ("cand_body", "cbody", np.int32), ("cand_point", "cpoint", np.float64),
             ("cand_radius", "cradius", np.float64), ("cand_shape", "cshape", np.int32),
             ("dof_effort", "effort", np.float64), ("dof_velocity", "vmax", np.float64),
             ("dof_armature", "armature", np.float64), ("dof_lower", "lower", np.float64),
             ("dof_upper", "upper", np.float64), ("dof_has_limits", "has_limits", np.int32),
             ("cand_link", "clink", np.int32), ("link_body", "lbody", np.int32),
             ("link_pose", "lpose", np.float64), ("link_com", "lcom", np.float64),
             ("cand_dyn", "cdyn", np.int32), ("shape_kind", "shkind", np.int32), ("shape_body", "shbody", np.int32),
             ("shape_link", "shlink", np.int32), ("shape_pose", "shpose", np.float64),
             ("shape_size", "shsize", np.float64), ("shape_margin", "shmargin", np.float64),
             ("shape_sphere", "shsphere", np.float64), ("hull_verts", "hverts", np.float64),
             ("shape_hv0", "shv0", np.int32), ("shape_hv1", "shv1", np.int32), ("pair_a", "pair_a", np.int32),
             ("pair_b", "pair_b", np.int32), ("pair_kind", "pair_kind", np.int32), ("pair_verts", "pverts", np.float64),
             ("shape_pv0", "shp0", np.int32), ("shape_pv1", "shp1", np.int32)]
    m.num_links = flat["nr"]
    m.num_hull_verts = len(flat["hverts"])
    m.num_pairs = int(flat["npair"])
    m.pair_pool = int(flat["npool"])
    m.num_pair_verts = len(flat["pverts"])
    for field, key, dt in pairs:
        a = np.ascontiguousarray(flat[key], dtype=dt)
        if a.size == 0:
            a = np.zeros(1, dtype=dt)
        keep[field] = a
        setattr(m, field, a.ctypes.data)
    return m, keep
```

Before: 32.40 million env-steps/s.

## Spread contact constraint rows across idle wave lanes in 4-env plane form

In the 4-envs-per-wave plane kernel only 16 of 64 lanes did useful work. The new row-lane mode runs each of the three contact-row copies (normal, two tangents) on its own 16-lane group, so each lane builds and factors one row instead of three. The rows are then shared back to every copy through ds_bpermute, and only the first group writes outputs. It also reorders the row slot layout to a 3*s+rr stride. This adds cross-lane permute traffic and redundant replicated work in exchange for cutting per-lane serial row loops, and it is on by default when no terrain is present.

```diff
diff --git a/include/gymsim.h b/include/gymsim.h
--- a/include/gymsim.h
+++ b/include/gymsim.h
@@ -151,6 +151,8 @@
 
 int gs_debug_self_contacts(gs_sim *sim, int mode, float *out, int *count, void *stream);
 
+int gs_debug_team_form(gs_sim *sim, int *envs_per_wave, int *row_lanes);
+
 #ifdef __cplusplus
 }
 #endif
diff --git a/isaacgymenv_amd/csrc/gs_capi.hip b/isaacgymenv_amd/csrc/gs_capi.hip
--- a/isaacgymenv_amd/csrc/gs_capi.hip
+++ b/isaacgymenv_amd/csrc/gs_capi.hip
@@ -150,6 +150,10 @@
     const int w = std::atoi(v);
     s->dp.team_epw = w == 16 || w == 8 || w == 4 ? w : 0;
   }
+  s->dp.team_row_lanes = -1;
+  if (const char* v = std::getenv("GS_TEAM_ROW_LANES")) {
+    if (v[0] == '0' || v[0] == '1') s->dp.team_row_lanes = v[0] - '0';
+  }
   return s;
 }
 
@@ -1008,6 +1012,14 @@
   return e == hipSuccess ? 0 : hip_fail(e, "gs_debug_self_contacts (mode 1 needs a split-form topology)");
 }
 
+int gs_debug_team_form(gs_sim* s, int* envs_per_wave, int* row_lanes) {
+  if (ready(s, "gs_debug_team_form")) return -1;
+  if (!envs_per_wave || !row_lanes) return fail("gs_debug_team_form: bad arguments");
+  if (s->host || s->variant != 2) return fail("gs_debug_team_form: the sim does not run the lane-team kernels");
+  team_launch_form(s->dp, envs_per_wave, row_lanes);
+  return 0;
+}
+
 int gs_sim_kernel_variant(gs_sim* s) { return s ? s->variant : -1; }
 
 int gs_sim_pd_tail_supported(const gs_sim* s) {
diff --git a/isaacgymenv_amd/csrc/gs_internal.h b/isaacgymenv_amd/csrc/gs_internal.h
--- a/isaacgymenv_amd/csrc/gs_internal.h
+++ b/isaacgymenv_amd/csrc/gs_internal.h
@@ -76,6 +76,7 @@
   const struct DevLinks* gen_links;
   int gen_nd, gen_nr;
   int team_epw;
+  int team_row_lanes;
 };
 #define GS_DOFP_FIELDS 6
 
@@ -110,6 +111,7 @@
 };
 
 bool team_fused_tail_available();
+void team_launch_form(const DevParams& P, int* epw, int* row_lanes);
 
 typedef hipError_t (*launch_sim_fn)(const DevModel*, const DevParams&, const SimBuffers&, const float* tau,
                                     hipStream_t);
diff --git a/isaacgymenv_amd/csrc/gs_team.hip b/isaacgymenv_amd/csrc/gs_team.hip
--- a/isaacgymenv_amd/csrc/gs_team.hip
+++ b/isaacgymenv_amd/csrc/gs_team.hip
@@ -123,10 +123,23 @@
   static constexpr int WAVES = kTeamBlock / LANES;
   static constexpr int THREADS = kWhole ? kTeamBlock : GS_WAVE * WAVES;
 };
-template <int EPW>
+template <int EPW, bool ROWL>
+__device__ __forceinline__ int team_wave_lane() {
+  return threadIdx.x & (ROWL ? WaveForm<EPW>::LANES - 1 : GS_WAVE - 1);
+}
+__device__ __forceinline__ int team_row_of_copy() {
+  const int r = (threadIdx.x & (GS_WAVE - 1)) >> 4;
+  return r < 2 ? r : 2;
+}
+__device__ __forceinline__ float from_copy(float x, int q) {
+  return __builtin_bit_cast(float, __builtin_amdgcn_ds_bpermute((int)(((threadIdx.x & 15) | (q << 4)) << 2),
+                                                                __builtin_bit_cast(int, x)));
+}
+__device__ __forceinline__ float sel3(int i, float a, float b, float c) { return i == 0 ? a : (i == 1 ? b : c); }
+template <int EPW, bool ROWL = false>
 __device__ __forceinline__ int team_column() {
   if constexpr (WaveForm<EPW>::kWhole) return threadIdx.x;
-  else return (threadIdx.x / GS_WAVE) * WaveForm<EPW>::LANES + (threadIdx.x & (GS_WAVE - 1));
+  else return (threadIdx.x / GS_WAVE) * WaveForm<EPW>::LANES + team_wave_lane<EPW, ROWL>();
 }
 template <int EPW>
 __device__ __forceinline__ void team_sync() {
@@ -146,7 +159,7 @@
   static constexpr int RZROW = 16;
   static constexpr int CSLOT = 15;
   __device__ static constexpr int zslot(int comp) { return comp < 6 ? 4 * (comp >> 1) + (comp & 1) : 4 * (comp - 6) + 2; }
-  __device__ static constexpr int zs(int rr, int s) { return rr < 2 ? 2 * s + rr : 2 * ZROW + s; }
+  __device__ static constexpr int zs(int rr, int s) { return 3 * s + rr; }
   static constexpr int C_DI = 3 * ZROW, C_G = C_DI + 3, C_TP = C_G + 3, C_TV = C_TP + 1,
                        C_MU = C_TV + 1, C_ACT = C_MU + 1, C_SEP = C_ACT + 1, PER_CONTACT = C_SEP + 1;
   static constexpr int R_DI = 3 * RZROW, R_G = R_DI + 3, R_TP = R_G + 3, R_TV = R_TP + 1,
@@ -351,7 +364,7 @@
 __device__ __forceinline__ float base_jac(const float* xc, int ax, int k) {
   if (k < 3) {
     const float m3[3][3] = {{0.f, xc[2], -xc[1]}, {-xc[2], 0.f, xc[0]}, {xc[1], -xc[0], 0.f}};
-    return m3[ax][k];
+    return sel3(ax, m3[0][k], m3[1][k], m3[2][k]);
   }
   return (ax == k - 3) ? 1.f : 0.f;
 }
@@ -488,7 +501,7 @@
   return ((unsigned long long)(unsigned)hi << 32) | (unsigned)lo;
 }
 
-template <class T, int EPW>
+template <class T, int EPW, bool ROWL>
 __device__ __forceinline__ int team_narrow_replicated(const DevModel* __restrict__ M, const DevParams& P,
                                                    const float* __restrict__ mu_g, int N, int e, int lc,
                                                    const float (&R0)[9], const float (&R)[T::T_CL][9],
@@ -496,7 +509,7 @@
                                                    float* __restrict__ shw_tab, const float* __restrict__ sct,
                                                    float* __restrict__ pool) {
   constexpr int TPW = WaveForm<EPW>::TEAMS;
-  const int team = (threadIdx.x & (GS_WAVE - 1)) >> 2;
+  const int team = team_wave_lane<EPW, ROWL>() >> 2;
   float* tab = shw_tab + team;
   team_sync<EPW>();
 #pragma unroll
@@ -541,7 +554,7 @@
   return cnt;
 }
 
-template <class T, int EPW>
+template <class T, int EPW, bool ROWL>
 __device__ __forceinline__ int team_self_contacts(const DevModel* __restrict__ M, const float* __restrict__ cm,
                                                   const DevParams& P, const float* __restrict__ mu_g, int N, int e,
                                                   int lc, const float (&R0)[9], const float (&R)[T::T_CL][9],
@@ -644,11 +657,11 @@
   const long long np_t0 = clock64();
 #endif
   if constexpr (!team_closed_form<T>()) {
-    return team_narrow_replicated<T, EPW>(M, P, mu_g, N, e, lc, R0, R, X, near, shw_tab, sct, pool);
+    return team_narrow_replicated<T, EPW, ROWL>(M, P, mu_g, N, e, lc, R0, R, X, near, shw_tab, sct, pool);
   } else {
   constexpr int kLC = team_lc<T>(), kSt = kTeamSt;
   constexpr int kNone = 0x7fffffff;
-  const int wl = threadIdx.x & 63;
+  const int wl = team_wave_lane<EPW, ROWL>();
   const int team = wl >> 2;
   float* lslot = shw_tab + wl;
   float* tstg = shw_tab + kLC * kSt * WL + team;
@@ -868,7 +881,7 @@
   return dist;
 }
 
-template <class T, bool TERR, bool TGS, int EPW>
+template <class T, bool TERR, bool TGS, int EPW, bool ROWL>
 __device__ __forceinline__ void substep_team(const DevModel* __restrict__ Min, const float* __restrict__ mdl,
                                              const DevParams& P, TeamState<T>& s, const float* tau,
                                              const float* __restrict__ mu_t, int N, int e, int lc,
@@ -878,6 +891,9 @@
                                              const float* __restrict__ sct, float* __restrict__ stash GS_PROF_PARAM) {
   constexpr int CL = T::T_CL, CC = T::T_CC, RC = T::T_RC, NCH = T::T_NCH, LN = T::T_LANES;
   static_assert(NCH == LN && LN == 4, "lane teams are DPP quads with one chain per lane");
+  static_assert(!ROWL || (!TERR && EPW == 4), "row lanes: the 4-envs-per-wave plane form");
+  constexpr int NROW = ROWL ? 1 : 3;
+  [[maybe_unused]] const int row_own = ROWL ? team_row_of_copy() : 0;
   using C = CM<T>;
   using RS = RowSlots<T>;
   uintptr_t mp = reinterpret_cast<uintptr_t>(Min);
@@ -1096,7 +1112,7 @@
   int npc = 0;
   float* pool = rows_own + RS::POOL * RW;
   if constexpr (T::NPK > 0) {
-    if (P.self_collide) npc = team_self_contacts<T, EPW>(M, cm, P, mu_t, kTeamsPerBlock, 0, lc, R0, R, X, shw_tab, sct, pool);
+    if (P.self_collide) npc = team_self_contacts<T, EPW, ROWL>(M, cm, P, mu_t, kTeamsPerBlock, 0, lc, R0, R, X, shw_tab, sct, pool);
   }
   GS_PROF(11)
 #pragma unroll
@@ -1173,20 +1189,21 @@
         if (act[j]) {
           const float xc[3] = {x[0], x[1], x[2] - r};
 #pragma unroll
-          for (int rr = 0; rr < 3; ++rr) {
+          for (int ri = 0; ri < NROW; ++ri) {
+            const int rr = ROWL ? row_own : ri;
             const int ax3 = (rr == 0) ? 2 : (rr == 1 ? 0 : 1);
-            float* row = rows_own + RS::chain(j) * RW;
-#pragma unroll
-            for (int b = 0; b < 6; ++b) row[RS::zs(rr, RS::zslot(b)) * RW] = base_jac(xc, ax3, b);
+            float* row = rows_own + (RS::chain(j) + RS::zs(rr, 0)) * RW;
+#pragma unroll
+            for (int b = 0; b < 6; ++b) row[RS::zs(0, RS::zslot(b)) * RW] = base_jac(xc, ax3, b);
+            const float xa = sel3(ax3, xc[1], xc[2], xc[0]), xb = sel3(ax3, xc[2], xc[0], xc[1]);
 #pragma unroll
             for (int kk = 0; kk < CL; ++kk) {
               float v = 0.f;
               if (kk <= k) {
-                float tt[3];
-                cross3(S[kk], xc, tt);
-                v = S[kk][3 + ax3] + tt[ax3];
+                const float sa = sel3(ax3, S[kk][1], S[kk][2], S[kk][0]), sb = sel3(ax3, S[kk][2], S[kk][0], S[kk][1]);
+                v = sel3(ax3, S[kk][3], S[kk][4], S[kk][5]) + (sa * xb - sb * xa);
               }
-              row[RS::zs(rr, RS::zslot(6 + kk)) * RW] = v;
+              row[RS::zs(0, RS::zslot(6 + kk)) * RW] = v;
             }
           }
         }
@@ -1357,9 +1374,10 @@
       const int kb = T::T_ccb[j];
       float zr[3][6 + CL], dir[3];
 #pragma unroll
-      for (int rr = 0; rr < 3; ++rr) {
-        float* row = rows_own + RS::chain(j) * RW;
-        auto Z = [&](int sl) -> float& { return row[RS::zs(rr, sl) * RW]; };
+      for (int ri = 0; ri < NROW; ++ri) {
+        const int rr = ROWL ? row_own : ri;
+        float* row = rows_own + (RS::chain(j) + RS::zs(rr, 0)) * RW;
+        auto Z = [&](int sl) -> float& { return row[RS::zs(0, sl) * RW]; };
         float zb[6], zc[CL];
         float cj = 0.f;
 #pragma unroll
@@ -1382,20 +1400,20 @@
 #pragma unroll
           for (int b = 0; b < k; ++b) zb[b] -= Mbb[k][b] * zb[k];
         }
-        float d = 0.f;
+        float d = 0.f, zo[6 + CL];
 #pragma unroll
         for (int b = 0; b < 6; ++b) {
           zb[b] *= sDb[b];
           d += zb[b] * zb[b];
           Z(RS::zslot(b)) = zb[b];
-          zr[rr][b] = zb[b];
+          zo[b] = zb[b];
         }
 #pragma unroll
         for (int k = 0; k < CL; ++k) {
           const float z = k <= kb ? zc[k] * sDc[k] : 0.f;
           d += z * z;
           Z(RS::zslot(6 + k)) = z;
-          zr[rr][6 + k] = z;
+          zo[6 + k] = z;
         }
         Z(3) = 0.f;
         Z(7) = 0.f;
@@ -1404,8 +1422,16 @@
         Z(13) = 0.f;
         Z(14) = 0.f;
         Z(RS::CSLOT) = cj;
-        dir[rr] = d > 0.f ? __builtin_amdgcn_rcpf(d) : 0.f;
-        rec[(RS::C_DI + rr) * RW] = dir[rr];
+        const float di = d > 0.f ? __builtin_amdgcn_rcpf(d) : 0.f;
+        rec[(RS::C_DI + rr) * RW] = di;
+#pragma unroll
+        for (int q = 0; q < 3; ++q) {
+          if (ROWL || q == ri) {
+#pragma unroll
+            for (int f = 0; f < 6 + CL; ++f) zr[q][f] = ROWL ? from_copy(zo[f], q) : zo[f];
+            dir[q] = ROWL ? from_copy(di, q) : di;
+          }
+        }
       }
       float g10 = 0.f, g20 = 0.f, g21 = 0.f;
 #pragma unroll
@@ -1468,15 +1494,15 @@
 #pragma unroll
           for (int b = 0; b < k; ++b) zb[b] -= Mbb[k][b] * zb[k];
         }
+        float* row = rec + RS::zs(rr, 0) * RW;
+        auto Z = [&](int sl) -> float& { return row[RS::zs(0, sl) * RW]; };
         float d = 0.f;
 #pragma unroll
         for (int b = 0; b < 6; ++b) {
           zb[b] *= sDb[b];
           d += zb[b] * zb[b];
-          rec[RS::zs(rr, RS::zslot(b)) * RW] = zb[b];
-          zr[rr][b] = zb[b];
-        }
-        auto Z = [&](int sl) -> float& { return rec[RS::zs(rr, sl) * RW]; };
+          Z(RS::zslot(b)) = zb[b];
+        }
 #pragma unroll
         for (int k = 0; k < 3; ++k) {
           Z(4 * k + 2) = 0.f;
@@ -1486,6 +1512,8 @@
         Z(13) = 0.f;
         Z(14) = 0.f;
         Z(RS::CSLOT) = cj;
+#pragma unroll
+        for (int f = 0; f < 6; ++f) zr[rr][f] = zb[f];
         dir[rr] = d > 0.f ? __builtin_amdgcn_rcpf(d) : 0.f;
         rec[(RS::R_DI + rr) * RW] = dir[rr];
       }
@@ -1515,10 +1543,12 @@
       const int cb = bb > 0 ? (bb - 1) / CL : -1, kb = bb > 0 ? (bb - 1) - cb * CL : -1;
       const float x[3] = {o[kPoolX * RW], o[(kPoolX + 1) * RW], o[(kPoolX + 2) * RW]};
       float zr[3][6], zc3[3][CL], dd[3];
-#pragma unroll
-      for (int rr = 0; rr < 3; ++rr) {
-        const int dofs = rr == 0 ? kPoolN : (rr == 1 ? kPoolT1 : kPoolT2);
-        const float d[3] = {o[dofs * RW], o[(dofs + 1) * RW], o[(dofs + 2) * RW]};
+      static_assert(kPoolT1 == kPoolN + 3 && kPoolT2 == kPoolN + 6, "a pool entry's three directions are one stride apart");
+#pragma unroll
+      for (int ri = 0; ri < NROW; ++ri) {
+        const int rr = ROWL ? row_own : ri;
+        const float* dp = o + (kPoolN + 3 * rr) * RW;
+        const float d[3] = {dp[0], dp[RW], dp[2 * RW]};
         float zc[CL], zbc[6];
         float cpart = 0.f;
 #pragma unroll
@@ -1550,10 +1580,20 @@
         }
         float own = 0.f, db = 0.f;
 #pragma unroll
-        for (int b = 0; b < 6; ++b) { zb[b] *= sDb[b]; db += zb[b] * zb[b]; zr[rr][b] = zb[b]; }
-#pragma unroll
-        for (int k = 0; k < CL; ++k) { zc[k] *= sDc[k]; own += zc[k] * zc[k]; zc3[rr][k] = zc[k]; }
-        dd[rr] = db + quad_sum(own);
+        for (int b = 0; b < 6; ++b) { zb[b] *= sDb[b]; db += zb[b] * zb[b]; }
+#pragma unroll
+        for (int k = 0; k < CL; ++k) { zc[k] *= sDc[k]; own += zc[k] * zc[k]; }
+        const float ddo = db + quad_sum(own);
+#pragma unroll
+        for (int q = 0; q < 3; ++q) {
+          if (ROWL || q == ri) {
+#pragma unroll
+            for (int b = 0; b < 6; ++b) zr[q][b] = ROWL ? from_copy(zb[b], q) : zb[b];
+#pragma unroll
+            for (int k = 0; k < CL; ++k) zc3[q][k] = ROWL ? from_copy(zc[k], q) : zc[k];
+            dd[q] = ROWL ? from_copy(ddo, q) : ddo;
+          }
+        }
         const float cj = quad_sum(cpart);
         float za = 0.f, zbb = 0.f;
 #pragma unroll
@@ -2015,22 +2055,23 @@
 
 struct TeamLane {
   int wave, col, lc, e;
-  bool on;
+  bool on, out;
 };
-template <class T, int EPW>
+template <class T, int EPW, bool ROWL>
 __device__ __forceinline__ TeamLane team_lane(int N) {
   constexpr int LN = T::T_LANES;
   static_assert(WaveForm<EPW>::WAVES == 1 || shw_size<T>() % WaveForm<EPW>::WAVES == 0, "every wave its own slice");
   TeamLane t;
   t.wave = WaveForm<EPW>::kWhole ? 0 : (int)(threadIdx.x / GS_WAVE);
-  t.col = team_column<EPW>();
+  t.col = team_column<EPW, ROWL>();
   t.lc = threadIdx.x & (LN - 1);
-  t.on = WaveForm<EPW>::kWhole || (int)(threadIdx.x & (GS_WAVE - 1)) < WaveForm<EPW>::LANES;
+  t.on = WaveForm<EPW>::kWhole || ROWL || (int)(threadIdx.x & (GS_WAVE - 1)) < WaveForm<EPW>::LANES;
+  t.out = !ROWL || (int)(threadIdx.x & (GS_WAVE - 1)) < WaveForm<EPW>::LANES;
   t.e = t.on ? (xcd_block(blockIdx.x, gridDim.x) * kTeamBlock + t.col) / LN : N;
   return t;
 }
 
-template <class T, bool TERR, bool TGS, int EPW>
+template <class T, bool TERR, bool TGS, int EPW, bool ROWL>
 __global__ __launch_bounds__(WaveForm<EPW>::THREADS, 1) void k_simulate_team(const DevModel* __restrict__ M, DevParams P,
                                                                  SimBuffers B, const float* __restrict__ tau_aos) {
   constexpr int LN = T::T_LANES, CL = T::T_CL, ND = T::ND;
@@ -2042,7 +2083,7 @@
   __shared__ float stash_tab[team_stash_size<T>() * kTeamBlock];
   stage_chain_model<T>(M, mdl);
   stage_shape_consts<T>(M, sct);
-  const TeamLane tl = team_lane<T, EPW>(B.N);
+  const TeamLane tl = team_lane<T, EPW, ROWL>(B.N);
   const int lc = tl.lc, e = tl.e, col = tl.col;
   if (tl.on)
     for (int sh = lc; sh < T::NS; sh += LN)
@@ -2061,14 +2102,14 @@
   const float* team = rows + (col & ~(LN - 1));
   GS_PROF_DECL
   for (int sstep = 0; sstep < P.substeps; ++sstep) {
-    const bool last = (sstep == P.substeps - 1) && P.collect;
-    substep_team<T, TERR, TGS, EPW>(M, mdl, P, s, tau, mu_t, N, e, lc, own, team, B.cf, last, nullptr, shw_wave, sct, stash_tab + col GS_PROF_ARGS);
-  }
-  team_store<T>(B.state, N, opaque_index(e), opaque_index(lc), s);
+    const bool last = (sstep == P.substeps - 1) && P.collect && tl.out;
+    substep_team<T, TERR, TGS, EPW, ROWL>(M, mdl, P, s, tau, mu_t, N, e, lc, own, team, B.cf, last, nullptr, shw_wave, sct, stash_tab + col GS_PROF_ARGS);
+  }
+  if (tl.out) team_store<T>(B.state, N, opaque_index(e), opaque_index(lc), s);
   GS_PROF_FLUSH
 }
 
-template <class T, bool TERR, bool TGS, int EPW>
+template <class T, bool TERR, bool TGS, int EPW, bool ROWL>
 __global__ __launch_bounds__(WaveForm<EPW>::THREADS, 1) void k_pd_step_team(const DevModel* __restrict__ M, DevParams P,
                                                                 SimBuffers B, PdDev A) {
   constexpr int LN = T::T_LANES, CL = T::T_CL, ND = T::ND, NB = T::NB;
@@ -2080,7 +2121,7 @@
   __shared__ float stash_tab[team_stash_size<T>() * kTeamBlock];
   stage_chain_model<T>(M, mdl);
   stage_shape_consts<T>(M, sct);
-  const TeamLane tl = team_lane<T, EPW>(B.N);
+  const TeamLane tl = team_lane<T, EPW, ROWL>(B.N);
   const int lc = tl.lc, e = tl.e, col = tl.col;
   if (tl.on)
     for (int sh = lc; sh < T::NS; sh += LN)
@@ -2112,11 +2153,11 @@
         tau[k] = clampf(A.kp * (A.scale * aj + A.default_pos[lc * CL + k] - qj) - A.kd * qdj, -A.tlim, A.tlim);
       }
     }
-    const bool last = ((it % sub) == sub - 1) && P.collect;
+    const bool last = ((it % sub) == sub - 1) && P.collect && tl.out;
     GS_PROF(6)
     float* cf_aos = (it == total - 1) ? A.cf_out : nullptr;
-    substep_team<T, TERR, TGS, EPW>(M, mdl, P, s, tau, mu_t, N, e, lc, own, team, B.cf, last, cf_aos, shw_wave, sct, stash_tab + col GS_PROF_ARGS);
-    if (it == n_pd - 1 && A.dof_out) {
+    substep_team<T, TERR, TGS, EPW, ROWL>(M, mdl, P, s, tau, mu_t, N, e, lc, own, team, B.cf, last, cf_aos, shw_wave, sct, stash_tab + col GS_PROF_ARGS);
+    if (it == n_pd - 1 && A.dof_out && tl.out) {
       const size_t d0 = dof0();
 #pragma unroll
       for (int k = 0; k < CL; ++k) {
@@ -2125,15 +2166,17 @@
       }
     }
   }
-  team_store<T>(B.state, N, opaque_index(e), opaque_index(lc), s);
-  const size_t d0 = dof0();
-#pragma unroll
-  for (int k = 0; k < CL; ++k) A.torques_out[d0 + k] = tau[k];
-  if (A.actions_copy) {
-#pragma unroll
-    for (int k = 0; k < CL; ++k) A.actions_copy[d0 + k] = A.actions[d0 + k];
-  }
-  if (A.root_out && lc == 0) {
+  if (tl.out) {
+    team_store<T>(B.state, N, opaque_index(e), opaque_index(lc), s);
+    const size_t d0 = dof0();
+#pragma unroll
+    for (int k = 0; k < CL; ++k) A.torques_out[d0 + k] = tau[k];
+    if (A.actions_copy) {
+#pragma unroll
+      for (int k = 0; k < CL; ++k) A.actions_copy[d0 + k] = A.actions[d0 + k];
+    }
+  }
+  if (A.root_out && lc == 0 && tl.out) {
     float* o = A.root_out + (size_t)e * 13;
     o[0] = s.p[0]; o[1] = s.p[1]; o[2] = s.p[2];
     o[3] = s.quat[0]; o[4] = s.quat[1]; o[5] = s.quat[2]; o[6] = s.quat[3];
@@ -2175,18 +2218,34 @@
   const int w = P.team_epw > 0 ? P.team_epw : (P.has_terrain ? kTeamEpwTerr : kTeamEpwPlane);
   return w == 8 || w == 4 ? w : 16;
 }
+constexpr bool kTeamRowLanesPlane = true;
+static bool team_row_lanes(const DevParams& P, int epw) {
+  if (kTeamBlock != GS_WAVE || epw != 4 || P.has_terrain) return false;
+  return P.team_row_lanes >= 0 ? P.team_row_lanes != 0 : kTeamRowLanesPlane;
+}
+void team_launch_form(const DevParams& P, int* epw, int* row_lanes) {
+  *epw = team_epw(P, false);
+  *row_lanes = team_row_lanes(P, *epw) ? 1 : 0;
+}
 #define GS_TEAM_LAUNCH_EPW(K, EPW, ...)                                                                      \
   do {                                                                                                       \
     const dim3 g_((unsigned)blocks), b_((unsigned)WaveForm<EPW>::THREADS);                                   \
-    if (P.has_terrain && P.tgs) hipLaunchKernelGGL((K<T, true, true, EPW>), g_, b_, 0, st, __VA_ARGS__);     \
-    else if (P.has_terrain) hipLaunchKernelGGL((K<T, true, false, EPW>), g_, b_, 0, st, __VA_ARGS__);        \
-    else if (P.tgs) hipLaunchKernelGGL((K<T, false, true, EPW>), g_, b_, 0, st, __VA_ARGS__);                \
-    else hipLaunchKernelGGL((K<T, false, false, EPW>), g_, b_, 0, st, __VA_ARGS__);                          \
+    if (P.has_terrain && P.tgs) hipLaunchKernelGGL((K<T, true, true, EPW, false>), g_, b_, 0, st, __VA_ARGS__);  \
+    else if (P.has_terrain) hipLaunchKernelGGL((K<T, true, false, EPW, false>), g_, b_, 0, st, __VA_ARGS__); \
+    else if (P.tgs) hipLaunchKernelGGL((K<T, false, true, EPW, false>), g_, b_, 0, st, __VA_ARGS__);         \
+    else hipLaunchKernelGGL((K<T, false, false, EPW, false>), g_, b_, 0, st, __VA_ARGS__);                   \
+  } while (0)
+#define GS_TEAM_LAUNCH_ROWL(K, ...)                                                                          \
+  do {                                                                                                       \
+    const dim3 g_((unsigned)blocks), b_((unsigned)WaveForm<4>::THREADS);                                     \
+    if (P.tgs) hipLaunchKernelGGL((K<T, false, true, 4, true>), g_, b_, 0, st, __VA_ARGS__);                 \
+    else hipLaunchKernelGGL((K<T, false, false, 4, true>), g_, b_, 0, st, __VA_ARGS__);                      \
   } while (0)
 #define GS_TEAM_LAUNCH(K, epw, ...)                              \
   do {                                                           \
     if constexpr (kTeamBlock == GS_WAVE) {                       \
       if ((epw) == 8) { GS_TEAM_LAUNCH_EPW(K, 8, __VA_ARGS__); break; }  \
+      if ((epw) == 4 && team_row_lanes(P, 4)) { GS_TEAM_LAUNCH_ROWL(K, __VA_ARGS__); break; }  \
       if ((epw) == 4) { GS_TEAM_LAUNCH_EPW(K, 4, __VA_ARGS__); break; }  \
     }                                                            \
     GS_TEAM_LAUNCH_EPW(K, 16, __VA_ARGS__);                      \
diff --git a/isaacgymenv_amd/isaacgym/_lib.py b/isaacgymenv_amd/isaacgym/_lib.py
--- a/isaacgymenv_amd/isaacgym/_lib.py
+++ b/isaacgymenv_amd/isaacgym/_lib.py
@@ -94,6 +94,7 @@
             "gs_sim_add_triangle_mesh": (i, [vp, vp, C.c_int64, vp, C.c_int64, vp, d, d, d]),
             "gs_debug_terrain_query": (i, [vp, vp, vp, i, vp, vp]),
             "gs_debug_self_contacts": (i, [vp, i, vp, vp, vp]),
+            "gs_debug_team_form": (i, [vp, C.POINTER(C.c_int), C.POINTER(C.c_int)]),
         }
         for name, (res, args) in sig.items():
             fn = getattr(L, name)
@@ -116,7 +117,7 @@
     "gs_sim_set_force_sensors", "gs_sim_bind_force_sensors", "gs_sim_refresh_force_sensor",
     "gs_sim_add_triangle_mesh", "gs_debug_terrain_query", "gs_sim_refresh_rigid_body", "gs_sim_refresh_jacobian",
     "gs_sim_refresh_mass_matrix", "gs_sim_set_dof_drives", "gs_sim_bind_dof_targets", "gs_sim_set_self_collision",
-    "gs_debug_self_contacts", "gs_sim_bind_dof_properties_env", "gs_sim_pd_tail_supported", "gs_sim_set_root_and_dof",
+    "gs_debug_self_contacts", "gs_debug_team_form", "gs_sim_bind_dof_properties_env", "gs_sim_pd_tail_supported", "gs_sim_set_root_and_dof",
 ]
 
 
```

Result: faster. 34.82 million env-steps/s (median of 6 runs) (+7.5%).
